# yjzxkxdn/HubertFA

Measured on NVIDIA B200. Metric: dp_cells_per_s, higher is better.
Workload: dtype f32

## Files before the change

hubertfa_b200/csrc/hfa_api.cu:

```cuda
#include <algorithm>
#include <atomic>
#include <climits>
#include <cstdarg>
#include <cstdio>
#include <cstdlib>
#include <cstring>
#include <mutex>
#include <new>
#include <numeric>
#include <unordered_map>
#include <vector>

#include <cuda.h>

#include "../../include/hfa_align.h"
#include "hfa_common.cuh"

#define HFA_EMIS_ROWS 64

cudaError_t hfa_launch_unpack_emissions(const HfaLaunchCtx &c, int total_row_blocks, float *out);
cudaError_t hfa_launch_dp_warp_any(const HfaLaunchCtx &c, int max_k, int max_pair_k, const int32_t *order, int n,
                                   float *dp_dump);
cudaError_t hfa_launch_dp_cta(const HfaLaunchCtx &c, const int32_t *order, int n, int max_sp, float *dp_dump);
cudaError_t hfa_launch_dp_band(const HfaLaunchCtx &c, int k, int item_begin, int n_items, int32_t *ticket,
                               bool keep_dp, int64_t fused_row_stride, float *dp_dump);
cudaError_t hfa_launch_dp_skew(const HfaLaunchCtx &c, int d, int item_begin, int n_items, int32_t *ticket,
                               bool keep_dp, float *dp_dump);
cudaError_t hfa_launch_emission(const HfaLaunchCtx &c, int total_row_blocks, int max_sp, int dtype,
                                int64_t max_row_stride, int *n_launched);
cudaError_t hfa_launch_edge(const HfaLaunchCtx &c, int total_row_blocks, int dtype);
cudaError_t hfa_launch_pack(const HfaLaunchCtx &c, int total_row_blocks, const float *prob_log,
                            const float *edge_log, const float *not_edge_log,
                            const float *edge_pred);
cudaError_t hfa_launch_backtrace(const HfaLaunchCtx &c, const int32_t *order, int n,
                                 const HfaResultPtrs &res, float *frame_conf, float *dp_path);
cudaError_t hfa_launch_unpack_bp(const HfaLaunchCtx &c, int utt, int8_t *out);
cudaError_t hfa_launch_unpack_dp(const HfaLaunchCtx &c, int utt, float *out);
cudaError_t hfa_launch_ctc_greedy(const void *logits, int dtype, int T, int V, int64_t st_t, int64_t st_v,
                                  int32_t *arg, int32_t *out_ids, int32_t *out_len, cudaStream_t stream);
cudaError_t hfa_launch_jump_tables(const HfaLaunchCtx &c, int n_blocks);
cudaError_t hfa_launch_backtrace_tables(const HfaLaunchCtx &c, const int32_t *order, int n,
                                        const HfaResultPtrs &res, float *frame_conf, float *dp_path);

namespace {

thread_local char g_err[512] = "";
std::atomic<int64_t> g_launches{0};

int fail(int code, const char *fmt, ...)
{
    va_list ap;
    va_start(ap, fmt);
    vsnprintf(g_err, sizeof(g_err), fmt, ap);
    va_end(ap);
    return code;
}
int cuda_fail(cudaError_t e, const char *what)
{
    return fail(HFA_ERR_CUDA, "%s: %s", what, cudaGetErrorString(e));
}

inline int64_t align_up(int64_t v, int64_t a) { return (v + a - 1) / a * a; }

typedef CUresult (*HfaEncodeTiled)(CUtensorMap *, CUtensorMapDataType, cuuint32_t, void *, const cuuint64_t *,
                                   const cuuint64_t *, const cuuint32_t *, const cuuint32_t *, CUtensorMapInterleave,
                                   CUtensorMapSwizzle, CUtensorMapL2promotion, CUtensorMapFloatOOBfill);
HfaEncodeTiled tensor_map_encoder()
{
    if (const char *e = std::getenv("HFA_NO_TENSORMAP"))
        if (e[0] == '1') return nullptr;
    static const HfaEncodeTiled fn = [] {
        void *f = nullptr;
        cudaDriverEntryPointQueryResult q;
        if (cudaGetDriverEntryPoint("cuTensorMapEncodeTiled", &f, cudaEnableDefault, &q) != cudaSuccess ||
            q != cudaDriverEntryPointSuccess)
            return (HfaEncodeTiled) nullptr;
        return reinterpret_cast<HfaEncodeTiled>(f);
    }();
    return fn;
}

struct HfaSideStreams {
    int device = -1;
    cudaStream_t stream[HFA_NUM_CLASSES] = {};
    cudaEvent_t fork = nullptr, join[HFA_NUM_CLASSES] = {};
};
std::vector<HfaSideStreams *> &side_pool()
{
    thread_local std::vector<HfaSideStreams *> pool;
    return pool;
}
HfaSideStreams *side_streams()
{
    std::vector<HfaSideStreams *> &pool = side_pool();
    int dev = 0;
    if (cudaGetDevice(&dev) != cudaSuccess) return nullptr;
    for (HfaSideStreams *s : pool)
        if (s->device == dev) return s;
    HfaSideStreams *s = new (std::nothrow) HfaSideStreams();
    if (!s) return nullptr;
    s->device = dev;
    bool ok = cudaEventCreateWithFlags(&s->fork, cudaEventDisableTiming) == cudaSuccess;
    for (int i = 0; ok && i < HFA_NUM_CLASSES; ++i) {
        ok = cudaStreamCreateWithFlags(&s->stream[i], cudaStreamNonBlocking) == cudaSuccess &&
             cudaEventCreateWithFlags(&s->join[i], cudaEventDisableTiming) == cudaSuccess;
    }
    if (!ok) { delete s; return nullptr; }
    try {
        pool.push_back(s);
    } catch (const std::bad_alloc &) {
        delete s;
        return nullptr;
    }
    return s;
}

int sm_count()
{
    int dev = 0, n = 0;
    if (cudaGetDevice(&dev) != cudaSuccess ||
        cudaDeviceGetAttribute(&n, cudaDevAttrMultiProcessorCount, dev) != cudaSuccess || n < 1)
        return 148;
    return n;
}

}

struct hfa_plan {
    int32_t n_utt = 0, vocab = 0;
    double frame_length = 0.0;
    std::vector<HfaUtt> utt;
    std::vector<int32_t> ids;
    std::vector<int32_t> col_ids;
    std::vector<uint8_t> colmap;
    int32_t n_compact = 0;
    int64_t stored_emis = 0;
    std::vector<int64_t> frame_off, seg_off;
    std::vector<int32_t> order;
    int32_t class_begin[HFA_NUM_CLASSES + 2] = {0};
    int32_t class_count[HFA_NUM_CLASSES + 1] = {0};
    int32_t cta_max_sp = 0, max_sp = 4;
    int32_t warp_all_begin = 0, warp_all_count = 0, warp_max_k = 0;
    int32_t warp_max_pair_k = 0, pair_count = 0;
    std::vector<HfaBandItem> band_items;
    int32_t band_begin[2] = {0, 0}, band_count[2] = {0, 0}, band_k[2] = {2, 4};
    int32_t band_skew[2] = {0, 0};
    int64_t band_xchg_elems = 0, dp_store_elems = 0;
    std::vector<int32_t> jblk_utt, jblk_first;
    int32_t n_valid = 0, n_kept = 0;
    int32_t bt_begin = 0;
    std::vector<int32_t> row_blocks;
    std::vector<int32_t> block_utt;
    int64_t total_frames = 0, total_states = 0, total_cells = 0, padded_cells = 0;
    int64_t total_words = 0, total_edge = 0;
    int64_t o_colids = 0, o_colmap = 0, o_emode = 0;
    int64_t o_utt = 0, o_ids = 0, o_order = 0, o_rowblk = 0, o_blkutt = 0, o_inputs = 0, head_bytes = 0;
    int64_t o_emis = 0, o_edge2 = 0, o_edgep = 0, o_bp = 0, o_path = 0, o_revi = 0, o_revt = 0,
            o_last = 0, o_dpst = 0, o_jump = 0, o_moves = 0, o_rowent = 0, o_band_items = 0, o_jblk_utt = 0, o_jblk_first = 0, o_band_ticket = 0, o_band_xchg = 0, band_bytes = 0, o_tmaps = 0, ws_bytes = 0;
    int32_t n_tmaps = 0;
    std::vector<unsigned char> head;
    HfaResultLayout res{};
    mutable std::mutex layout_mu;
    mutable std::unordered_map<const void *, int64_t> layout_of;
    int64_t row_stride_of(const void *workspace) const
    {
        std::lock_guard<std::mutex> g(layout_mu);
        auto it = layout_of.find(workspace);
        return it == layout_of.end() ? 0 : it->second;
    }
    void set_row_stride(const void *workspace, int64_t v) const
    {
        std::lock_guard<std::mutex> g(layout_mu);
        layout_of[workspace] = v;
    }
};

namespace {

HfaWs make_ws(const hfa_plan *p, void *workspace)
{
    unsigned char *b = static_cast<unsigned char *>(workspace);
    HfaWs w;
    w.utt = reinterpret_cast<const HfaUtt *>(b + p->o_utt);
    w.ids = reinterpret_cast<const int32_t *>(b + p->o_ids);
    w.order = reinterpret_cast<const int32_t *>(b + p->o_order);
    w.row_blocks = reinterpret_cast<const int32_t *>(b + p->o_rowblk);
    w.block_utt = reinterpret_cast<const int32_t *>(b + p->o_blkutt);
    w.inputs = reinterpret_cast<HfaInput *>(b + p->o_inputs);
    w.emis = reinterpret_cast<float *>(b + p->o_emis);
    w.edge2 = reinterpret_cast<float2 *>(b + p->o_edge2);
    w.edge_p = reinterpret_cast<float *>(b + p->o_edgep);
    w.bp = reinterpret_cast<uint32_t *>(b + p->o_bp);
    w.path_state = reinterpret_cast<int32_t *>(b + p->o_path);
    w.rev_idx = reinterpret_cast<int32_t *>(b + p->o_revi);
    w.rev_t = reinterpret_cast<int32_t *>(b + p->o_revt);
    w.dp_last = reinterpret_cast<float *>(b + p->o_last);
    w.dp_store = reinterpret_cast<float *>(b + p->o_dpst);
    w.jump = reinterpret_cast<uint8_t *>(b + p->o_jump);
    w.moves = reinterpret_cast<uint8_t *>(b + p->o_moves);
    w.row_entry = reinterpret_cast<int32_t *>(b + p->o_rowent);
    w.jblk_utt = reinterpret_cast<const int32_t *>(b + p->o_jblk_utt);
    w.jblk_first = reinterpret_cast<const int32_t *>(b + p->o_jblk_first);
    w.tmaps = (p->n_tmaps > 0 && tensor_map_encoder() != nullptr) ? b + p->o_tmaps : nullptr;
    w.col_ids = reinterpret_cast<const int32_t *>(b + p->o_colids);
    w.colmap = reinterpret_cast<const uint8_t *>(b + p->o_colmap);
    w.emis_mode = reinterpret_cast<int32_t *>(b + p->o_emode);
    w.band_items = reinterpret_cast<const HfaBandItem *>(b + p->o_band_items);
    w.band_ticket = reinterpret_cast<int32_t *>(b + p->o_band_ticket);
    w.band_xchg = reinterpret_cast<uint4 *>(b + p->o_band_xchg);
    return w;
}

HfaLaunchCtx make_ctx(const hfa_plan *p, void *workspace, void *stream)
{
    HfaLaunchCtx c;
    c.ws = make_ws(p, workspace);
    c.n_utt = p->n_utt;
    c.vocab = p->vocab;
    c.frame_length = p->frame_length;
    c.stream = static_cast<cudaStream_t>(stream);
    return c;
}

HfaResultPtrs make_res(const hfa_plan *p, void *result)
{
    unsigned char *b = static_cast<unsigned char *>(result);
    HfaResultPtrs r;
    r.status = reinterpret_cast<int32_t *>(b + p->res.status);
    r.n_seg = reinterpret_cast<int32_t *>(b + p->res.n_seg);
    r.end_state = reinterpret_cast<int32_t *>(b + p->res.end_state);
    r.final_score = reinterpret_cast<float *>(b + p->res.final_score);
    r.total_conf = reinterpret_cast<float *>(b + p->res.total_conf);
    r.ph_idx_seq = reinterpret_cast<int32_t *>(b + p->res.ph_idx_seq);
    r.ph_time_int = reinterpret_cast<int32_t *>(b + p->res.ph_time_int);
    r.intervals = reinterpret_cast<double *>(b + p->res.intervals);
    return r;
}

}

extern "C" {

int hfa_abi_version(void) { return HFA_ABI_VERSION; }
const char *hfa_last_error(void) { return g_err; }
int64_t hfa_launch_count(void) { return g_launches.load(); }

int hfa_plan_create(int32_t n_utt, int32_t vocab_size, const int32_t *T, const int32_t *S,
                    const int32_t *ph_ids, double frame_length, hfa_plan **out)
{
    if (out == nullptr) return fail(HFA_ERR_ARG, "hfa_plan_create: out is NULL");
    *out = nullptr;
    if (n_utt < 0 || vocab_size < 1 || (n_utt > 0 && (!T || !S || !ph_ids)))
        return fail(HFA_ERR_ARG, "hfa_plan_create: bad arguments (n_utt=%d, V=%d)", n_utt,
                    vocab_size);
    hfa_plan *p = new (std::nothrow) hfa_plan();
    if (!p) return fail(HFA_ERR_NOMEM, "hfa_plan_create: out of host memory");
    try {
        p->n_utt = n_utt;
        p->vocab = vocab_size;
        p->frame_length = frame_length;
        p->utt.resize((size_t)n_utt);
        p->frame_off.assign((size_t)n_utt + 1, 0);
        p->seg_off.assign((size_t)n_utt + 1, 0);
        p->row_blocks.assign((size_t)n_utt + 1, 0);
        for (int32_t b = 0; b < n_utt; ++b)
            p->seg_off[b + 1] = p->seg_off[b] + std::max<int32_t>(S[b], 0);
        p->total_states = p->seg_off[n_utt];
        p->ids.assign(ph_ids, ph_ids + p->total_states);

        std::vector<int32_t> lists[HFA_NUM_CLASSES + 1], invalid, giant;
        int64_t emis = 0, edge = 0, words = 0, cells = 0, frames = 0;
        for (int32_t b = 0; b < n_utt; ++b) {
            HfaUtt &m = p->utt[b];
            std::memset(&m, 0, sizeof(m));
            const int32_t t = T[b], s = S[b];
            int32_t st = HFA_UTT_OK;
            if (s < 1) st = HFA_UTT_NO_STATES;
            else if (t < 1) st = HFA_UTT_EMPTY;
            else if (s > HFA_MAX_STATES) st = HFA_UTT_TOO_MANY_STATES;
            else {
                const int32_t *id = ph_ids + p->seg_off[b];
                for (int32_t i = 0; i < s; ++i)
                    if (id[i] < 0 || id[i] >= vocab_size) { st = HFA_UTT_BAD_ID; break; }
            }
            m.status = st;
            m.seg_off = p->seg_off[b];
            m.frame_off = frames;
            m.cell_off = cells;
            m.emis_off = emis;
            m.edge_off = edge;
            m.bp_off = words;
            m.dp_off = -1;
            m.tmap = -1;
            p->frame_off[b] = frames;
            if (st == HFA_UTT_OK) {
                m.T = t;
                m.S = s;
                m.Sp = (s + 3) & ~3;
                frames += t;
                cells += (int64_t)t * s;
                emis += (int64_t)t * m.Sp;
                edge += align_up(t, HFA_TILE_T);
                words += (int64_t)((t + 15) / 16) * m.Sp;
                p->row_blocks[b + 1] = p->row_blocks[b] + (t + HFA_EMIS_ROWS - 1) / HFA_EMIS_ROWS;
                p->max_sp = std::max(p->max_sp, m.Sp);
                if (m.Sp <= HFA_WARP_MAX_S) lists[(m.Sp + 31) / 32 - 1].push_back(b);
                else if (s > HFA_CTA_MAX_S) giant.push_back(b);
                else {
                    lists[HFA_NUM_CLASSES].push_back(b);
                    p->cta_max_sp = std::max(p->cta_max_sp, m.Sp);
                }
            } else {
                p->row_blocks[b + 1] = p->row_blocks[b];
                invalid.push_back(b);
            }
        }
        p->frame_off[n_utt] = frames;
        p->total_frames = frames;
        p->total_cells = cells;
        p->padded_cells = emis;
        p->total_words = words;
        p->total_edge = edge;

        auto by_len = [&](int32_t a, int32_t b) {
            return p->utt[a].T != p->utt[b].T ? p->utt[a].T > p->utt[b].T : a < b;
        };
        std::vector<int32_t> all;
        for (int c = 0; c <= HFA_NUM_CLASSES; ++c) {
            std::sort(lists[c].begin(), lists[c].end(), by_len);
            p->class_begin[c] = (int32_t)p->order.size();
            p->class_count[c] = (int32_t)lists[c].size();
            p->order.insert(p->order.end(), lists[c].begin(), lists[c].end());
            all.insert(all.end(), lists[c].begin(), lists[c].end());
        }
        all.insert(all.end(), giant.begin(), giant.end());
        int skew_d = 2;
        if (const char *e = std::getenv("HFA_SKEW_D")) skew_d = (std::atoi(e) == 3) ? 3 : 2;
        if (const char *e = std::getenv("HFA_LAT_KERNEL")) { if (e[0] == 'b') skew_d = 0; }
        if (tensor_map_encoder() == nullptr) skew_d = 0;
        auto n_bands = [&](int32_t b, int k) {
            if (k == 1) return hfa_skew_strips(p->utt[b].Sp);
            const int w = 32 * k, own = w - 32, sp = p->utt[b].Sp;
            return sp <= w ? 1 : (sp - 32 + own - 1) / own;
        };
        int64_t band_max = 3072;
        if (const char *e = std::getenv("HFA_BAND_MAX")) band_max = std::atoll(e);
        int lat_mode = -1;
        if (const char *e = std::getenv("HFA_LATENCY_MODE")) lat_mode = e[0] - '0';
        std::vector<int32_t> lat_band;
        bool hybrid = false;
        if (lat_mode != 0) {
            int64_t nb = 0;
            for (int c = 0; c < HFA_NUM_CLASSES; ++c)
                for (int32_t b : lists[c]) nb += n_bands(b, skew_d > 0 ? 1 : 2);
            if (skew_d > 0) {
                p->band_k[0] = 1;
                p->band_skew[0] = skew_d;
            }
            if (lat_mode == 2 || (nb > 0 && nb <= band_max)) {
                for (int c = 0; c < HFA_NUM_CLASSES; ++c) {
                    lat_band.insert(lat_band.end(), lists[c].begin(), lists[c].end());
                    lists[c].clear();
                    p->class_count[c] = 0;
                }
                std::sort(lat_band.begin(), lat_band.end(), by_len);
            } else if (skew_d > 0 && nb > 0) {
                double alpha = 0.0;
                if (const char *e = std::getenv("HFA_HYBRID")) alpha = std::atof(e);
                auto ucost = [&](int32_t b) { return (int64_t)p->utt[b].T * ((p->utt[b].Sp + 31) / 32); };
                int64_t sum_cost = 0;
                for (int c = 0; c < HFA_NUM_CLASSES; ++c)
                    for (int32_t b : lists[c]) sum_cost += ucost(b);
                const double thresh = alpha * (double)sum_cost / (4.0 * sm_count());
                if (alpha > 0.0) {
                    int64_t strips = 0;
                    for (int c = 1; c < HFA_NUM_CLASSES; ++c) {
                        std::vector<int32_t> keep;
                        for (int32_t b : lists[c]) {
                            if ((double)ucost(b) >= thresh && strips + n_bands(b, 1) <= 8 * band_max) {
                                lat_band.push_back(b);
                                strips += n_bands(b, 1);
                            } else {
                                keep.push_back(b);
                            }
                        }
                        lists[c].swap(keep);
                        p->class_count[c] = (int32_t)lists[c].size();
                    }
                    std::sort(lat_band.begin(), lat_band.end(), by_len);
                    hybrid = !lat_band.empty();
                }
            }
        }
        std::vector<int32_t> big_band;
        {
            int big_mode = -1;
            if (const char *e = std::getenv("HFA_BIG_KERNEL")) big_mode = (e[0] == 'b');
            auto count = [&](int k) {
                int64_t nb = 0;
                for (int32_t b : lists[HFA_NUM_CLASSES]) nb += n_bands(b, k);
                return nb;
            };
            int big_k = 0;
            if (const char *e = std::getenv("HFA_BIG_K")) big_k = std::atoi(e);
            if (big_k != 2 && big_k != 4 && big_k != 8) {
                big_k = 8;
                for (int k : {2, 4, 8})
                    if (count(k) <= band_max) { big_k = k; break; }
                if (skew_d > 0 && count(1) <= band_max) big_k = 1;
            }
            p->band_k[1] = big_k;
            if (big_k == 1) p->band_skew[1] = skew_d;
            if (big_mode == 1 || (big_mode == -1 && count(big_k) <= band_max)) {
                big_band = lists[HFA_NUM_CLASSES];
                lists[HFA_NUM_CLASSES].clear();
                p->class_count[HFA_NUM_CLASSES] = 0;
            }
            if (!giant.empty()) {
                if (big_band.empty()) {
                    p->band_k[1] = skew_d > 0 ? 1 : 2;
                    p->band_skew[1] = skew_d;
                }
                big_band.insert(big_band.end(), giant.begin(), giant.end());
                std::sort(big_band.begin(), big_band.end(), by_len);
            }
        }
        bool keep_dp = true;
        if (const char *e = std::getenv("HFA_KEEP_DP")) keep_dp = (e[0] != '0');
        auto add_bands = [&](const std::vector<int32_t> &utts, int which) {
            const int k = p->band_k[which];
            const int sd = p->band_skew[which];
            p->band_begin[which] = (int32_t)p->band_items.size();
            for (int32_t b : utts) {
                const int nb = n_bands(b, k);
                const int64_t tiles = (p->utt[b].T + 15) / 16;
                p->utt[b].skew_d = sd;
                p->utt[b].band_k = k;
                p->utt[b].tmap = p->n_tmaps++;
                if (keep_dp && !(hybrid && which == 0)) {
                    p->utt[b].dp_off = p->dp_store_elems;
                    p->dp_store_elems += sd > 0 ? (int64_t)nb * hfa_skew_blocks(sd, p->utt[b].T) * HFA_SKEW_BLK * 32
                                                : (int64_t)nb * p->utt[b].T * 32 * k;
                }
                for (int j = 0; j < nb; ++j) {
                    const bool has_right = j + 1 < nb;
                    p->band_items.push_back(HfaBandItem{b, j, has_right ? p->band_xchg_elems : 0});
                    if (has_right) p->band_xchg_elems += sd > 0 ? (tiles + 1) / 2 * 32 : tiles * 64;
                }
            }
            p->band_count[which] = (int32_t)p->band_items.size() - p->band_begin[which];
        };
        add_bands(lat_band, 0);
        add_bands(big_band, 1);
        p->n_valid = (int32_t)all.size();
        for (const HfaUtt &m : p->utt) p->n_kept += (m.status == 0 && m.dp_off >= 0);
        p->jblk_first.assign((size_t)n_utt + 1, 0);
        for (int32_t b = 0; b < n_utt; ++b) {
            const HfaUtt &m = p->utt[b];
            const int64_t w = (m.status == 0 && m.dp_off >= 0) ? (int64_t)((m.T + 15) / 16) * m.Sp : 0;
            const int32_t nblk = (int32_t)((w + 255) / 256);
            p->jblk_first[b + 1] = p->jblk_first[b] + nblk;
            p->jblk_utt.insert(p->jblk_utt.end(), (size_t)nblk, b);
        }
        int pair_mode = 1;
        if (const char *e = std::getenv("HFA_PAIR")) pair_mode = std::atoi(e);
        std::vector<int32_t> warp_all;
        std::vector<std::pair<int32_t, int>> pairable;
        int64_t sum_pair = 0, sum_plain = 0;
        for (int c = 0; c < HFA_NUM_CLASSES; ++c) {
            warp_all.insert(warp_all.end(), lists[c].begin(), lists[c].end());
            for (int32_t b : lists[c]) {
                const HfaUtt &m = p->utt[b];
                const int32_t *id = ph_ids + m.seg_off;
                int phon = 0;
                bool ok = pair_mode > 0;
                for (int32_t i = 0; i < m.S && ok; ++i) {
                    phon += id[i] != 0;
                    if (i > 0 && id[i] == 0 && id[i - 1] == 0) ok = false;
                }
                const int kp = (phon + (id[m.S - 1] == 0) + 31) / 32;
                if (ok && kp <= HFA_PAIR_MAX_K) {
                    pairable.push_back({b, kp});
                    sum_pair += (int64_t)m.T * (17 + 25 * kp);
                    sum_plain += (int64_t)m.T * (16 + 21 * (c + 1));
                }
                p->warp_max_k = std::max(p->warp_max_k, c + 1);
            }
        }
        bool compact = vocab_size <= 255;
        if (const char *e = std::getenv("HFA_COMPACT")) compact = compact && e[0] != '0';
        p->col_ids.assign((size_t)(p->total_states + 4 * (int64_t)n_utt), vocab_size);
        p->colmap.assign((size_t)p->total_states, 0);
        if (pair_mode >= 2 || sum_pair < sum_plain)
            for (const auto &bk : pairable) {
                HfaUtt &m = p->utt[bk.first];
                m.pair_k = bk.second;
                p->warp_max_pair_k = std::max(p->warp_max_pair_k, bk.second);
                p->pair_count += 1;
                if (!compact) continue;
                const int32_t *id = ph_ids + m.seg_off;
                int col_of[256];
                std::fill(col_of, col_of + 256, -1);
                for (int32_t i = 0; i < m.S; ++i) col_of[id[i]] = 0;
                int d = 0;
                for (int v = 0; v < vocab_size; ++v)
                    if (col_of[v] == 0) col_of[v] = d++;
                const int dp = (d + 3) & ~3;
                if (dp >= m.Sp) continue;
                m.Dp = dp;
                p->n_compact += 1;
                int32_t *ci = p->col_ids.data() + m.seg_off + 4 * (int64_t)bk.first;
                for (int v = 0; v < vocab_size; ++v)
                    if (col_of[v] >= 0) ci[col_of[v]] = v;
                for (int32_t i = 0; i < m.S; ++i) p->colmap[(size_t)(m.seg_off + i)] = (uint8_t)col_of[id[i]];
            }
        for (const HfaUtt &m : p->utt)
            if (m.status == 0) p->stored_emis += (int64_t)m.T * (m.Dp > 0 ? m.Dp : m.Sp);
        const bool old_order = p->pair_count == 0;
        auto cost = [&](int32_t b) {
            const HfaUtt &m = p->utt[b];
            if (old_order) return (int64_t)m.T * (2 + (m.Sp + 31) / 32);
            return (int64_t)m.T * (m.pair_k > 0 ? 17 + 25 * m.pair_k : 16 + 21 * ((m.Sp + 31) / 32));
        };
        std::sort(warp_all.begin(), warp_all.end(),
                  [&](int32_t a, int32_t b) { return cost(a) != cost(b) ? cost(a) > cost(b) : a < b; });
        p->warp_all_begin = (int32_t)p->order.size();
        p->warp_all_count = (int32_t)warp_all.size();
        p->order.insert(p->order.end(), warp_all.begin(), warp_all.end());
        std::sort(all.begin(), all.end(), by_len);
        p->bt_begin = (int32_t)p->order.size();
        p->order.insert(p->order.end(), all.begin(), all.end());
        p->order.insert(p->order.end(), invalid.begin(), invalid.end());

        int64_t o = 0;
        auto region = [&](int64_t bytes) { const int64_t at = o; o = align_up(o + bytes, 256); return at; };
        p->o_utt = region((int64_t)n_utt * sizeof(HfaUtt));
        p->o_ids = region(p->total_states * 4);
        p->o_order = region((int64_t)p->order.size() * 4);
        p->o_rowblk = region((int64_t)(n_utt + 1) * 4);
        p->block_utt.reserve((size_t)p->row_blocks[n_utt]);
        for (int32_t b = 0; b < n_utt; ++b)
            p->block_utt.insert(p->block_utt.end(), (size_t)(p->row_blocks[b + 1] - p->row_blocks[b]), b);
        p->o_blkutt = region((int64_t)p->block_utt.size() * 4);
        p->o_band_items = region((int64_t)p->band_items.size() * sizeof(HfaBandItem));
        p->o_jblk_utt = region((int64_t)p->jblk_utt.size() * 4);
        p->o_jblk_first = region((int64_t)p->jblk_first.size() * 4);
        p->o_colids = region(p->n_compact > 0 ? (int64_t)p->col_ids.size() * 4 : 0);
        p->o_colmap = region(p->n_compact > 0 ? (int64_t)p->colmap.size() : 0);
        p->head_bytes = o;
        p->o_inputs = region((int64_t)n_utt * sizeof(HfaInput));
        p->o_emis = region(emis * 4);
        p->o_edge2 = region(edge * 8);
        p->o_edgep = region(edge * 4 + 4);
        p->o_bp = region(words * 4);
        p->o_path = region(frames * 4);
        p->o_revi = region(p->total_states * 4);
        p->o_revt = region(p->total_states * 4);
        p->o_last = region((int64_t)n_utt * 8);
        p->o_emode = region(p->n_compact > 0 ? (int64_t)n_utt * 4 : 0);
        p->o_dpst = region(p->dp_store_elems * 4);
        const bool jump_tables = p->dp_store_elems > 0;
        p->o_jump = region(jump_tables ? words : 0);
        p->o_moves = region(jump_tables ? words : 0);
        p->o_rowent = region(jump_tables ? edge / 16 * 4 : 0);

        p->o_tmaps = region((int64_t)p->n_tmaps * 128);
        p->o_band_ticket = region(p->band_items.empty() ? 0 : 8);
        p->o_band_xchg = region(p->band_xchg_elems * 16);
        p->band_bytes = o - p->o_band_ticket;
        p->ws_bytes = std::max<int64_t>(o, 256);

        p->head.assign((size_t)p->head_bytes, 0);
        if (n_utt > 0) {
            std::memcpy(p->head.data() + p->o_utt, p->utt.data(), (size_t)n_utt * sizeof(HfaUtt));
            if (p->total_states)
                std::memcpy(p->head.data() + p->o_ids, p->ids.data(), (size_t)p->total_states * 4);
            std::memcpy(p->head.data() + p->o_order, p->order.data(), p->order.size() * 4);
        }
        if (!p->band_items.empty())
            std::memcpy(p->head.data() + p->o_band_items, p->band_items.data(),
                        p->band_items.size() * sizeof(HfaBandItem));
        if (!p->jblk_utt.empty())
            std::memcpy(p->head.data() + p->o_jblk_utt, p->jblk_utt.data(), p->jblk_utt.size() * 4);
        std::memcpy(p->head.data() + p->o_jblk_first, p->jblk_first.data(), p->jblk_first.size() * 4);
        if (p->n_compact > 0) {
            std::memcpy(p->head.data() + p->o_colids, p->col_ids.data(), p->col_ids.size() * 4);
            if (!p->colmap.empty()) std::memcpy(p->head.data() + p->o_colmap, p->colmap.data(), p->colmap.size());
        }
        std::memcpy(p->head.data() + p->o_rowblk, p->row_blocks.data(), (size_t)(n_utt + 1) * 4);
        if (!p->block_utt.empty())
            std::memcpy(p->head.data() + p->o_blkutt, p->block_utt.data(), p->block_utt.size() * 4);

        int64_t r = 0;
        auto rreg = [&](int64_t bytes) { const int64_t at = r; r = align_up(r + bytes, 16); return at; };
        p->res.status = rreg((int64_t)n_utt * 4);
        p->res.n_seg = rreg((int64_t)n_utt * 4);
        p->res.end_state = rreg((int64_t)n_utt * 4);
        p->res.final_score = rreg((int64_t)n_utt * 4);
        p->res.total_conf = rreg((int64_t)n_utt * 4);
        p->res.ph_idx_seq = rreg(p->total_states * 4);
        p->res.ph_time_int = rreg(p->total_states * 4);
        p->res.intervals = rreg(p->total_states * 16);
        p->res.total_bytes = std::max<int64_t>(r, 16);
    } catch (const std::bad_alloc &) {
        delete p;
        return fail(HFA_ERR_NOMEM, "hfa_plan_create: out of host memory");
    }
    *out = p;
    return HFA_OK;
}

void hfa_plan_destroy(hfa_plan *plan) { delete plan; }

int64_t hfa_plan_workspace_bytes(const hfa_plan *p) { return p ? p->ws_bytes : 0; }
int64_t hfa_plan_total_frames(const hfa_plan *p) { return p ? p->total_frames : 0; }
int64_t hfa_plan_total_states(const hfa_plan *p) { return p ? p->total_states : 0; }
int64_t hfa_plan_total_cells(const hfa_plan *p) { return p ? p->total_cells : 0; }
const int64_t *hfa_plan_frame_offsets(const hfa_plan *p) { return p ? p->frame_off.data() : nullptr; }
const int64_t *hfa_plan_seg_offsets(const hfa_plan *p) { return p ? p->seg_off.data() : nullptr; }

int hfa_plan_result_layout(const hfa_plan *p, HfaResultLayout *out)
{
    if (!p || !out) return fail(HFA_ERR_ARG, "hfa_plan_result_layout: NULL argument");
    *out = p->res;
    return HFA_OK;
}

int hfa_plan_algorithmic_bytes(const hfa_plan *p, int32_t dtype, int64_t out[3])
{
    if (!p || !out) return fail(HFA_ERR_ARG, "hfa_plan_algorithmic_bytes: NULL argument");
    const int64_t in_b = (dtype == HFA_DTYPE_F32) ? 4 : 2;
    int64_t words = 0, kept_cells = 0, kept_frames = 0;
    for (const HfaUtt &m : p->utt)
        if (m.status == 0) {
            words += (int64_t)((m.T + 15) / 16) * m.S;
            if (m.dp_off >= 0) {
                kept_cells += (int64_t)m.T * m.S;
                kept_frames += m.T;
            }
        }
    out[0] = p->total_frames * ((int64_t)p->vocab * in_b + in_b) + p->total_cells * 4 +
             p->total_frames * 12;
    out[1] = p->total_cells * 4 + p->total_frames * 8 + words * 4 + kept_cells * 4;
    out[2] = (p->total_frames - kept_frames) * (8 + 8) + kept_frames * (8 + 4) + p->total_states * 24;
    return HFA_OK;
}

int hfa_plan_routing(const hfa_plan *p, int32_t out[8])
{
    if (!p || !out) return fail(HFA_ERR_ARG, "hfa_plan_routing: NULL argument");
    out[0] = p->warp_all_count;
    out[1] = p->band_count[0];
    out[2] = p->band_k[0];
    out[3] = p->band_count[1];
    out[4] = p->band_k[1];
    out[5] = p->class_count[HFA_NUM_CLASSES];
    out[6] = p->dp_store_elems > 0;
    out[7] = std::max(p->band_skew[0], p->band_skew[1]);
    return HFA_OK;
}

int32_t hfa_plan_pair_utterances(const hfa_plan *p) { return p ? p->pair_count : 0; }
int64_t hfa_plan_stored_emission_bytes(const hfa_plan *p) { return p ? p->stored_emis * 4 : 0; }

int64_t hfa_plan_debug_region(const hfa_plan *p, int32_t which, int64_t *n_bytes)
{
    if (!p) return -1;
    int64_t off = -1, n = 0;
    switch (which) {
        case 0: off = p->o_emis; n = p->padded_cells * 4; break;
        case 1: off = p->o_edge2; n = p->total_edge * 8; break;
        case 2: off = p->o_edgep; n = p->total_edge * 4; break;
        case 3: off = p->o_bp; n = p->total_words * 4; break;
        default: break;
    }
    if (n_bytes) *n_bytes = n;
    return off;
}

int hfa_plan_upload(const hfa_plan *p, void *workspace, void *stream)
{
    if (!p || !workspace) return fail(HFA_ERR_ARG, "hfa_plan_upload: NULL argument");
    if (p->head_bytes == 0) return HFA_OK;
    cudaError_t e = cudaMemcpyAsync(workspace, p->head.data(), (size_t)p->head_bytes,
                                    cudaMemcpyHostToDevice, static_cast<cudaStream_t>(stream));
    if (e != cudaSuccess) return cuda_fail(e, "hfa_plan_upload");
    if (p->n_tmaps > 0 && tensor_map_encoder() != nullptr) try {
        std::vector<CUtensorMap> maps((size_t)p->n_tmaps);
        for (const HfaUtt &m : p->utt) {
            if (m.status != 0 || m.tmap < 0) continue;
            const cuuint64_t dims[2] = {(cuuint64_t)m.Sp, (cuuint64_t)m.T};
            const cuuint64_t pitch[1] = {(cuuint64_t)m.Sp * 4};
            const cuuint32_t box[2] = {(cuuint32_t)(m.skew_d > 0 ? HFA_SKEW_BOX : 32 * m.band_k),
                                       (cuuint32_t)(m.skew_d > 0 ? HFA_SKEW_BLK : HFA_TILE_T)};
            const cuuint32_t estr[2] = {1, 1};
            void *base = static_cast<unsigned char *>(workspace) + p->o_emis + m.emis_off * 4;
            const CUresult r = tensor_map_encoder()(&maps[(size_t)m.tmap], CU_TENSOR_MAP_DATA_TYPE_FLOAT32, 2, base,
                                                    dims, pitch, box, estr, CU_TENSOR_MAP_INTERLEAVE_NONE,
                                                    CU_TENSOR_MAP_SWIZZLE_NONE, CU_TENSOR_MAP_L2_PROMOTION_NONE,
                                                    CU_TENSOR_MAP_FLOAT_OOB_FILL_NONE);
            if (r != CUDA_SUCCESS) return fail(HFA_ERR_CUDA, "hfa_plan_upload: cuTensorMapEncodeTiled failed (%d)", (int)r);
        }
        e = cudaMemcpyAsync(static_cast<unsigned char *>(workspace) + p->o_tmaps, maps.data(), maps.size() * 128,
                            cudaMemcpyHostToDevice, static_cast<cudaStream_t>(stream));
        if (e != cudaSuccess) return cuda_fail(e, "hfa_plan_upload: tensor maps");
    } catch (const std::bad_alloc &) {
        return fail(HFA_ERR_NOMEM, "hfa_plan_upload: out of host memory");
    }
    if (p->n_compact > 0) {
        e = cudaMemsetAsync(static_cast<unsigned char *>(workspace) + p->o_emode, 0, (size_t)p->n_utt * 4,
                            static_cast<cudaStream_t>(stream));
        if (e != cudaSuccess) return cuda_fail(e, "hfa_plan_upload: emission mode reset");
    }
    if (p->band_bytes > 0) {
        e = cudaMemsetAsync(static_cast<unsigned char *>(workspace) + p->o_band_ticket, 0,
                            (size_t)p->band_bytes, static_cast<cudaStream_t>(stream));
        if (e != cudaSuccess) return cuda_fail(e, "hfa_plan_upload: band table reset");
    }
    return HFA_OK;
}

int hfa_set_inputs(const hfa_plan *p, void *workspace, const void *const *frame_ptrs,
                   const int64_t *frame_stride_t, const int64_t *frame_stride_v,
                   const void *const *edge_ptrs, const int64_t *edge_stride, void *stream)
{
    if (!p || !workspace) return fail(HFA_ERR_ARG, "hfa_set_inputs: NULL plan/workspace");
    if (p->n_utt == 0) return HFA_OK;
    if (!frame_ptrs || !frame_stride_t || !frame_stride_v || !edge_ptrs || !edge_stride)
        return fail(HFA_ERR_ARG, "hfa_set_inputs: NULL input table");
    try {
        std::vector<HfaInput> in((size_t)p->n_utt);
        int64_t row_stride = 0;
        bool contiguous = true;
        for (int32_t b = 0; b < p->n_utt; ++b) {
            if (p->utt[b].status == 0 && (!frame_ptrs[b] || !edge_ptrs[b]))
                return fail(HFA_ERR_ARG, "hfa_set_inputs: NULL logits pointer for utterance %d", b);
            if (p->utt[b].status == 0) {
                if (frame_stride_v[b] != 1 || frame_stride_t[b] < p->vocab ||
                    (reinterpret_cast<uintptr_t>(frame_ptrs[b]) & 3u))
                    contiguous = false;
                row_stride = std::max(row_stride, frame_stride_t[b]);
            }
            in[b].frame = frame_ptrs[b];
            in[b].edge = edge_ptrs[b];
            in[b].frame_st = frame_stride_t[b];
            in[b].frame_sv = frame_stride_v[b];
            in[b].edge_st = edge_stride[b];
        }
        HfaLaunchCtx c = make_ctx(p, workspace, stream);
        cudaError_t e = cudaMemcpyAsync(c.ws.inputs, in.data(), in.size() * sizeof(HfaInput),
                                        cudaMemcpyHostToDevice, c.stream);
        if (e != cudaSuccess) return cuda_fail(e, "hfa_set_inputs: input table upload");
        p->set_row_stride(workspace, contiguous ? row_stride : 0);
    } catch (const std::bad_alloc &) {
        return fail(HFA_ERR_NOMEM, "hfa_set_inputs: out of host memory");
    }
    return HFA_OK;
}

static_assert(sizeof(HfaInputDesc) == sizeof(HfaInput), "the public descriptor is the kernels' own");

int hfa_set_inputs_device(const hfa_plan *p, void *workspace, const HfaInputDesc *table, int64_t max_row_stride,
                          void *stream)
{
    if (!p || !workspace) return fail(HFA_ERR_ARG, "hfa_set_inputs_device: NULL plan/workspace");
    if (p->n_utt == 0) return HFA_OK;
    if (!table) return fail(HFA_ERR_ARG, "hfa_set_inputs_device: NULL table");
    if (max_row_stride < 0) return fail(HFA_ERR_ARG, "hfa_set_inputs_device: negative row stride");
    HfaLaunchCtx c = make_ctx(p, workspace, stream);
    cudaError_t e = cudaMemcpyAsync(c.ws.inputs, table, (size_t)p->n_utt * sizeof(HfaInput),
                                    cudaMemcpyDeviceToDevice, c.stream);
    if (e != cudaSuccess) return cuda_fail(e, "hfa_set_inputs_device: table copy");
    try {
        p->set_row_stride(workspace, max_row_stride);
    } catch (const std::bad_alloc &) {
        return fail(HFA_ERR_NOMEM, "hfa_set_inputs_device: out of host memory");
    }
    return HFA_OK;
}

void hfa_release_thread_resources(void)
{
    for (HfaSideStreams *s : side_pool()) {
        for (int i = 0; i < HFA_NUM_CLASSES; ++i) {
            if (s->stream[i]) cudaStreamDestroy(s->stream[i]);
            if (s->join[i]) cudaEventDestroy(s->join[i]);
        }
        if (s->fork) cudaEventDestroy(s->fork);
        delete s;
    }
    side_pool().clear();
}

int hfa_emission(const hfa_plan *p, void *workspace, int32_t dtype, void *stream)
{
    if (!p || !workspace) return fail(HFA_ERR_ARG, "hfa_emission: NULL plan/workspace");
    if (p->n_utt == 0 || p->total_frames == 0) return HFA_OK;
    if (dtype < 0 || dtype > 2) return fail(HFA_ERR_ARG, "hfa_emission: bad dtype %d", dtype);
    HfaLaunchCtx c = make_ctx(p, workspace, stream);
    static const bool no_tma = [] { const char *v = std::getenv("HFA_EMISSION_NO_TMA"); return v && v[0] == '1'; }();
    const int64_t row_stride = no_tma ? 0 : p->row_stride_of(workspace);
    HfaSideStreams *ss = nullptr;
    cudaError_t e = cudaSuccess;
    if (row_stride > 0) {
        ss = side_streams();
        if (!ss) return fail(HFA_ERR_CUDA, "hfa_emission: cannot create side streams");
        e = cudaEventRecord(ss->fork, c.stream);
        if (e != cudaSuccess) return cuda_fail(e, "hfa_emission: fork");
    }
    int n_launched = 0;
    e = hfa_launch_emission(c, p->row_blocks[p->n_utt], p->max_sp, dtype, row_stride, &n_launched);
    if (e != cudaSuccess) return cuda_fail(e, "hfa_emission: launch");
    if (n_launched == 2) {
        HfaLaunchCtx cs = c;
        cs.stream = ss->stream[HFA_NUM_CLASSES - 1];
        e = cudaStreamWaitEvent(cs.stream, ss->fork, 0);
        if (e == cudaSuccess) e = hfa_launch_edge(cs, p->row_blocks[p->n_utt], dtype);
        if (e == cudaSuccess) e = cudaEventRecord(ss->join[HFA_NUM_CLASSES - 1], cs.stream);
        if (e == cudaSuccess) e = cudaStreamWaitEvent(c.stream, ss->join[HFA_NUM_CLASSES - 1], 0);
        if (e != cudaSuccess) return cuda_fail(e, "hfa_emission: edge kernel");
    }
    g_launches += n_launched;
    return HFA_OK;
}

int hfa_pack_emissions(const hfa_plan *p, void *workspace, const float *prob_log,
                       const float *edge_log, const float *not_edge_log, const float *edge_pred,
                       void *stream)
{
    if (!p || !workspace) return fail(HFA_ERR_ARG, "hfa_pack_emissions: NULL plan/workspace");
    if (p->n_utt == 0 || p->total_frames == 0) return HFA_OK;
    if (!prob_log || !edge_log || !not_edge_log)
        return fail(HFA_ERR_ARG, "hfa_pack_emissions: NULL input");
    HfaLaunchCtx c = make_ctx(p, workspace, stream);
    cudaError_t e = hfa_launch_pack(c, p->row_blocks[p->n_utt], prob_log, edge_log, not_edge_log,
                                    edge_pred);
    if (e != cudaSuccess) return cuda_fail(e, "hfa_pack_emissions: launch");
    g_launches += 1;
    return HFA_OK;
}

static int viterbi_forward_impl(const hfa_plan *p, void *workspace, float *dp_dump, void *stream,
                                int64_t fused_row_stride)
{
    if (!p || !workspace) return fail(HFA_ERR_ARG, "hfa_viterbi_forward: NULL plan/workspace");
    HfaLaunchCtx c = make_ctx(p, workspace, stream);
    const int n_cta = p->class_count[HFA_NUM_CLASSES];
    struct Item { int k; const int32_t *order; int n; };
    Item items[4];
    int n_items = 0;
    if (p->warp_all_count > 0) items[n_items++] = {0, c.ws.order + p->warp_all_begin, p->warp_all_count};
    if (p->band_count[0] > 0) items[n_items++] = {-3, nullptr, 0};
    if (p->band_count[1] > 0) items[n_items++] = {-4, nullptr, 1};
    if (n_cta > 0) items[n_items++] = {-1, c.ws.order + p->class_begin[HFA_NUM_CLASSES], n_cta};
    if (n_items == 0) return HFA_OK;

    const bool fork = n_items > 1;
    HfaSideStreams *ss = nullptr;
    if (fork) {
        ss = side_streams();
        if (!ss) return fail(HFA_ERR_CUDA, "hfa_viterbi_forward: cannot create side streams");
        cudaError_t e = cudaEventRecord(ss->fork, c.stream);
        if (e != cudaSuccess) return cuda_fail(e, "hfa_viterbi_forward: fork record");
    }
    const cudaStream_t user = c.stream;
    for (int it = 0; it < n_items; ++it) {
        cudaError_t e;
        const bool side = fork && it > 0;
        c.stream = side ? ss->stream[it - 1] : user;
        if (side) {
            e = cudaStreamWaitEvent(c.stream, ss->fork, 0);
            if (e != cudaSuccess) return cuda_fail(e, "hfa_viterbi_forward: fork wait");
        }
        if (items[it].k == 0)
            e = hfa_launch_dp_warp_any(c, p->warp_max_k, p->warp_max_pair_k, items[it].order, items[it].n, dp_dump);
        else if (items[it].k == -3 || items[it].k == -4) {
            const int wh = items[it].k == -3 ? 0 : 1;
            if (p->band_skew[wh] > 0)
                e = hfa_launch_dp_skew(c, p->band_skew[wh], p->band_begin[wh], p->band_count[wh],
                                       c.ws.band_ticket + wh, p->dp_store_elems > 0, dp_dump);
            else
                e = hfa_launch_dp_band(c, p->band_k[wh], p->band_begin[wh], p->band_count[wh],
                                       c.ws.band_ticket + wh, p->dp_store_elems > 0, fused_row_stride, dp_dump);
        }
        else
            e = hfa_launch_dp_cta(c, items[it].order, items[it].n, p->cta_max_sp, dp_dump);
        if (e != cudaSuccess) return cuda_fail(e, "hfa_viterbi_forward: kernel launch");
        g_launches += 1;
        if (side) {
            e = cudaEventRecord(ss->join[it - 1], c.stream);
            if (e == cudaSuccess) e = cudaStreamWaitEvent(user, ss->join[it - 1], 0);
            if (e != cudaSuccess) return cuda_fail(e, "hfa_viterbi_forward: join");
        }
    }
    return HFA_OK;
}

int hfa_viterbi_forward(const hfa_plan *p, void *workspace, float *dp_dump, void *stream)
{
    return viterbi_forward_impl(p, workspace, dp_dump, stream, 0);
}

int hfa_backtrace(const hfa_plan *p, void *workspace, void *result, float *frame_conf,
                  float *dp_path, void *stream)
{
    if (!p || !workspace || !result) return fail(HFA_ERR_ARG, "hfa_backtrace: NULL argument");
    if (p->n_utt == 0) return HFA_OK;
    HfaLaunchCtx c = make_ctx(p, workspace, stream);
    const HfaResultPtrs r = make_res(p, result);
    if (!p->jblk_utt.empty()) {
        cudaError_t ej = hfa_launch_jump_tables(c, (int)p->jblk_utt.size());
        if (ej == cudaSuccess)
            ej = hfa_launch_backtrace_tables(c, c.ws.order + p->bt_begin, p->n_valid, r, frame_conf, dp_path);
        if (ej != cudaSuccess) return cuda_fail(ej, "hfa_backtrace: table kernels");
        g_launches += 2;
        if (p->n_kept == p->n_utt) return HFA_OK;
    }
    cudaError_t e = hfa_launch_backtrace(c, c.ws.order + p->bt_begin, p->n_utt, r, frame_conf,
                                         dp_path);
    if (e != cudaSuccess) return cuda_fail(e, "hfa_backtrace: launch");
    g_launches += 1;
    return HFA_OK;
}

static bool fused_ok(const hfa_plan *p, const void *workspace, int32_t dtype)
{
    const int64_t max_row_stride = p->row_stride_of(workspace);
    const bool all_banded = p->warp_all_count == 0 &&
                            p->class_count[HFA_NUM_CLASSES] == 0 && !p->band_items.empty();
    const bool skewed = p->band_skew[0] > 0 || p->band_skew[1] > 0;
    return all_banded && !skewed && p->max_sp <= HFA_CTA_MAX_S && p->dp_store_elems > 0 && dtype == HFA_DTYPE_F32 &&
           max_row_stride > 0 &&
           p->vocab <= 256 && max_row_stride * 4 * HFA_TILE_T <= 48 * 1024;
}

int hfa_forward_fused(const hfa_plan *p, void *workspace, int32_t dtype, void *stream)
{
    if (!p || !workspace) return fail(HFA_ERR_ARG, "hfa_forward_fused: NULL plan/workspace");
    if (!fused_ok(p, workspace, dtype))
        return fail(HFA_ERR_UNSUPPORTED, "hfa_forward_fused: needs an all-banded plan that keeps dp, f32 logits "
                                         "with contiguous rows (set by hfa_set_inputs) and V <= 256");
    HfaLaunchCtx c = make_ctx(p, workspace, stream);
    cudaError_t e = hfa_launch_edge(c, p->row_blocks[p->n_utt], dtype);
    if (e != cudaSuccess) return cuda_fail(e, "hfa_forward_fused: edge kernel");
    g_launches += 1;
    return viterbi_forward_impl(p, workspace, nullptr, stream, p->row_stride_of(workspace));
}

int64_t hfa_plan_algorithmic_bytes_fused(const hfa_plan *p, int32_t dtype)
{
    if (!p) return 0;
    const int64_t in_b = (dtype == HFA_DTYPE_F32) ? 4 : 2;
    int64_t words = 0;
    for (const HfaUtt &m : p->utt)
        if (m.status == 0) words += (int64_t)((m.T + 15) / 16) * m.S;
    return p->total_frames * ((int64_t)p->vocab * in_b + in_b) + p->total_frames * 12 + words * 4 +
           p->total_cells * 4;
}

int hfa_align_batch(const hfa_plan *p, void *workspace, int32_t dtype, void *result,
                    float *frame_conf, void *stream)
{
    if (!p || !workspace) return fail(HFA_ERR_ARG, "hfa_align_batch: NULL plan/workspace");
    static const int fused_mode = [] { const char *v = std::getenv("HFA_FUSED"); return v ? (v[0] == '1' ? 1 : 0) : -1; }();
    int64_t n_valid = 0;
    for (const HfaUtt &m : p->utt) n_valid += (m.status == 0);
    const bool unsplit = (int64_t)p->band_items.size() == n_valid;
    int rc;
    if ((fused_mode == 1 || (fused_mode == -1 && unsplit)) && fused_ok(p, workspace, dtype)) {
        rc = hfa_forward_fused(p, workspace, dtype, stream);
    } else {
        rc = hfa_emission(p, workspace, dtype, stream);
        if (rc != HFA_OK) return rc;
        rc = viterbi_forward_impl(p, workspace, nullptr, stream, 0);
    }
    if (rc != HFA_OK) return rc;
    return hfa_backtrace(p, workspace, result, frame_conf, nullptr, stream);
}

int hfa_ctc_greedy(const void *logits, int32_t dtype, int64_t T, int64_t V, int64_t stride_t,
                   int64_t stride_v, int32_t *scratch, int32_t *out_ids, int32_t *out_len, void *stream)
{
    if (!logits || !scratch || !out_ids || !out_len) return fail(HFA_ERR_ARG, "hfa_ctc_greedy: NULL argument");
    if (T < 0 || V < 1 || T > INT32_MAX || V > INT32_MAX || dtype < 0 || dtype > 2)
        return fail(HFA_ERR_ARG, "hfa_ctc_greedy: bad shape / dtype (T=%lld, V=%lld)", (long long)T, (long long)V);
    cudaError_t e = hfa_launch_ctc_greedy(logits, dtype, (int)T, (int)V, stride_t, stride_v, scratch, out_ids,
                                          out_len, static_cast<cudaStream_t>(stream));
    if (e != cudaSuccess) return cuda_fail(e, "hfa_ctc_greedy: launch");
    g_launches += 1;
    return HFA_OK;
}

int hfa_debug_unpack_backptr(const hfa_plan *p, const void *workspace, int32_t utt, int8_t *out,
                             void *stream)
{
    if (!p || !workspace || !out) return fail(HFA_ERR_ARG, "hfa_debug_unpack_backptr: NULL argument");
    if (utt < 0 || utt >= p->n_utt || p->utt[utt].status != 0)
        return fail(HFA_ERR_ARG, "hfa_debug_unpack_backptr: bad utterance %d", utt);
    HfaLaunchCtx c = make_ctx(p, const_cast<void *>(workspace), stream);
    cudaError_t e = hfa_launch_unpack_bp(c, utt, out);
    if (e != cudaSuccess) return cuda_fail(e, "hfa_debug_unpack_backptr: launch");
    g_launches += 1;
    return HFA_OK;
}

int hfa_debug_unpack_dp(const hfa_plan *p, const void *workspace, int32_t utt, float *out, void *stream)
{
    if (!p || !workspace || !out) return fail(HFA_ERR_ARG, "hfa_debug_unpack_dp: NULL argument");
    if (utt < 0 || utt >= p->n_utt || p->utt[utt].status != 0)
        return fail(HFA_ERR_ARG, "hfa_debug_unpack_dp: bad utterance %d", utt);
    if (p->utt[utt].dp_off < 0)
        return fail(HFA_ERR_UNSUPPORTED, "hfa_debug_unpack_dp: the forward pass keeps no dp for utterance %d", utt);
    HfaLaunchCtx c = make_ctx(p, const_cast<void *>(workspace), stream);
    cudaError_t e = hfa_launch_unpack_dp(c, utt, out);
    if (e != cudaSuccess) return cuda_fail(e, "hfa_debug_unpack_dp: launch");
    g_launches += 1;
    return HFA_OK;
}

int hfa_debug_unpack_emissions(const hfa_plan *p, const void *workspace, float *out, void *stream)
{
    if (!p || !workspace || !out) return fail(HFA_ERR_ARG, "hfa_debug_unpack_emissions: NULL argument");
    HfaLaunchCtx c = make_ctx(p, const_cast<void *>(workspace), stream);
    cudaError_t e = hfa_launch_unpack_emissions(c, p->n_utt > 0 ? p->row_blocks[p->n_utt] : 0, out);
    if (e != cudaSuccess) return cuda_fail(e, "hfa_debug_unpack_emissions: launch");
    g_launches += 1;
    return HFA_OK;
}

}
```

hubertfa_b200/csrc/hfa_backtrace.cu:

```cuda
#include "hfa_common.cuh"

#define HFA_BT_WARPS 4

namespace {

__device__ __forceinline__ double seg_time(const float *p, int t, int T, double frame_length)
{
    double d = (t + 1 < T) ? (double)__fsub_rn(p[t + 1], p[t]) : 0.0;
    d = fmin(fmax(__dmul_rn(d, 0.5), -0.5), 0.5);
    return __dmul_rn(frame_length, __dadd_rn((double)(float)t, d));
}

template <typename FMove, typename FSpan>
__device__ __forceinline__ int hfa_walk_row(const uint32_t *__restrict__ row_words, int cur, int tt, bool row0,
                                            FMove on_move, FSpan on_span)
{
    while (tt >= 0) {
        const uint32_t wc = row_words[cur];
        uint32_t nz = (wc | (wc >> 16)) & 0xffffu & ((2u << tt) - 1u);
        if (row0) nz |= 1u;
        if (nz == 0u) {
            on_span(cur, 0, tt);
            break;
        }
        const int tp = 31 - __clz(nz);
        on_span(cur, tp, tt);
        on_move(cur, tp);
        if (row0 && tp == 0) break;
        cur -= ((wc >> (16 + tp)) & 1u) ? 2 : 1;
        tt = tp - 1;
    }
    return cur;
}

__global__ void __launch_bounds__(256)
hfa_jump_table_kernel(HfaWs ws)
{
    const int u = ws.jblk_utt[blockIdx.x];
    const HfaUtt m = ws.utt[u];
    const int n_rows = (m.T + 15) >> 4;
    const int64_t idx = (int64_t)(blockIdx.x - ws.jblk_first[u]) * blockDim.x + threadIdx.x;
    if (idx >= (int64_t)n_rows * m.Sp) return;
    const int w = (int)(idx / m.Sp), s = (int)(idx - (int64_t)w * m.Sp);
    const int tt = (w == n_rows - 1) ? ((m.T - 1) & 15) : 15;
    int n_moves = 0;
    const int from = hfa_walk_row(ws.bp + m.bp_off + (int64_t)w * m.Sp, s, tt, false,
                                  [&](int, int) { ++n_moves; }, [](int, int, int) {});
    ws.jump[m.bp_off + idx] = (uint8_t)(s - from);
    ws.moves[m.bp_off + idx] = (uint8_t)n_moves;
}

__global__ void __launch_bounds__(HFA_BT_WARPS * 32)
hfa_backtrace_kernel(HfaWs ws, const int32_t *__restrict__ order, int n, HfaResultPtrs res,
                     float *__restrict__ frame_conf, float *__restrict__ dp_path,
                     double frame_length)
{
    __shared__ float4 stage_sm[HFA_BT_WARPS][32];
    __shared__ float dpath_sm[HFA_BT_WARPS][32];
    const int lane = threadIdx.x & 31, warp = threadIdx.x >> 5;
    const int item = blockIdx.x * HFA_BT_WARPS + warp;
    if (item >= n) return;
    const int u = order[item];
    const HfaUtt m = ws.utt[u];
    if (m.status != 0) {
        if (lane == 0) {
            res.status[u] = m.status;
            res.n_seg[u] = 0;
            res.end_state[u] = -1;
            res.final_score[u] = HFA_NEG_INF;
            res.total_conf[u] = __uint_as_float(0x7fc00000u);
        }
        return;
    }
    if (m.dp_off >= 0) return;
    const int T = m.T, S = m.S, Sp = m.Sp;
    const int32_t *ids = ws.ids + m.seg_off;
    const uint32_t *bp = ws.bp + m.bp_off;
    int32_t *rev_idx = ws.rev_idx + m.seg_off;
    int32_t *rev_t = ws.rev_t + m.seg_off;
    int32_t *path_state = ws.path_state + m.frame_off;

    const float last1 = ws.dp_last[2 * u];
    const float last2 = (S >= 2) ? ws.dp_last[2 * u + 1] : HFA_NEG_INF;
    int s = S - 1;
    float final_score = last1;
    if (S >= 2 && last2 > last1 && ids[S - 1] == 0) {
        s = S - 2;
        final_score = last2;
    }
    const int s_end = s;

    constexpr int LEAD = 4;
    const int n_rows = (T + 15) >> 4;
    int n_seg = 0;
    int s_hi = s;
    uint32_t q[LEAD][2];
    int qref[LEAD];
    auto fetch = [&](int row, int ref, uint32_t (&w2)[2]) {
        w2[0] = w2[1] = 0u;
        if (row >= 0) {
            const uint32_t *r = bp + (int64_t)row * Sp;
            if (ref - lane >= 0) w2[0] = r[ref - lane];
            if (ref - lane - 32 >= 0) w2[1] = r[ref - lane - 32];
        }
    };
    uint32_t W = (s_hi - lane >= 0) ? bp[(int64_t)(n_rows - 1) * Sp + (s_hi - lane)] : 0u;
#pragma unroll
    for (int dd = 0; dd < LEAD; ++dd) {
        fetch(n_rows - 2 - dd, s_hi, q[dd]);
        qref[dd] = s_hi;
    }
    for (int w = n_rows - 1; w >= 0; --w) {
        uint32_t f[2];
        fetch(w - 1 - LEAD, s_hi, f);
        const int fref = s_hi;
        int tt = (w == n_rows - 1) ? ((T - 1) & 15) : 15;
        int my_state = 0;
        while (tt >= 0) {
            const uint32_t wc = __shfl_sync(0xffffffffu, W, (s_hi - s) & 31);
            uint32_t nz = (wc | (wc >> 16)) & 0xffffu & ((2u << tt) - 1u);
            if (w == 0) nz |= 1u;
            if (nz == 0u) {
                if (lane <= tt) my_state = s;
                break;
            }
            const int tp = 31 - __clz(nz);
            if (lane <= tt && lane >= tp) my_state = s;
            if (lane == 0 && n_seg < S) {
                rev_idx[n_seg] = s;
                rev_t[n_seg] = 16 * w + tp;
            }
            ++n_seg;
            if (w == 0 && tp == 0) break;
            s -= ((wc >> (16 + tp)) & 1u) ? 2 : 1;
            tt = tp - 1;
        }
        if (lane < 16 && 16 * w + lane < T) path_state[16 * w + lane] = my_state;
        if (w > 0) {
            const int o = (qref[0] - s) + lane;
            if (qref[0] - s + 31 < 64) {
                const uint32_t x0 = __shfl_sync(0xffffffffu, q[0][0], o & 31);
                const uint32_t x1 = __shfl_sync(0xffffffffu, q[0][1], o & 31);
                W = (o < 32) ? x0 : x1;
            } else {
                W = (s - lane >= 0) ? bp[(int64_t)(w - 1) * Sp + (s - lane)] : 0u;
            }
            s_hi = s;
#pragma unroll
            for (int dd = 0; dd + 1 < LEAD; ++dd) {
                q[dd][0] = q[dd + 1][0];
                q[dd][1] = q[dd + 1][1];
                qref[dd] = qref[dd + 1];
            }
            q[LEAD - 1][0] = f[0];
            q[LEAD - 1][1] = f[1];
            qref[LEAD - 1] = fref;
        }
    }
    if (n_seg > S) n_seg = S;
    __syncwarp();

    double log_sum = 0.0;
    {
    const float *emis = ws.emis + m.emis_off;
    const float2 *edge2 = ws.edge2 + m.edge_off;
    const double ratio = __ddiv_rn((double)T, (double)S);
    const bool lead_sp = (ids[0] == 0) && (S > 1);
    const bool compact = m.Dp > 0 && ws.emis_mode[u] != 0;
    const int Ep = compact ? m.Dp : Sp;
    const uint8_t *cmap = ws.colmap + m.seg_off;
    float4 *stage = stage_sm[warp];
    float *dpath = dpath_sm[warp];
    float d = 0.0f, cu = 0.0f, carry_d = 0.0f;
    const int n_rounds = (T + 31) >> 5;
    auto load_state = [&](int round) {
        const int t = round * 32 + lane;
        return (round < n_rounds && t < T) ? path_state[t] : 0;
    };
    struct Raw { float x, y; float2 ed; int id, st, sprev; };
    auto gather = [&](int round, int st, int sprev) {
        const int t = min(round * 32 + lane, T - 1);
        const float *row = emis + (int64_t)t * Ep;
        Raw g;
        g.x = hfa_ldg_f32_64B(row + (compact ? (int)cmap[st] : st));
        g.y = hfa_ldg_f32_64B(row + (compact ? (int)cmap[sprev] : sprev));
        g.ed = edge2[t];
        g.id = ids[st];
        g.st = st;
        g.sprev = sprev;
        return g;
    };
    auto finish = [&](int round, const Raw &g) {
        const int t = round * 32 + lane;
        float4 v = make_float4(0.f, 0.f, 0.f, __int_as_float(4));
        if (t < T) {
            const bool moved = (t > 0) && (g.sprev != g.st);
            v.x = g.x;
            v.y = g.y;
            v.z = moved ? g.ed.x : g.ed.y;
            int fl = (moved ? 1 : 0) | ((g.id == 0) ? 2 : 0);
            if (t == 0) {
                const bool seeded = (g.st == 0) || (g.st == 1 && lead_sp);
                v.x = seeded ? v.x : HFA_NEG_INF;
                fl = 8;
            }
            v.w = __int_as_float(fl);
        }
        return v;
    };
    int st_a = load_state(0), st_b = load_state(1), st_c = load_state(2);
    Raw g_cur = gather(0, st_a, __shfl_up_sync(0xffffffffu, st_a, 1));
    Raw g_nxt;
    {
        int sp1 = __shfl_up_sync(0xffffffffu, st_b, 1);
        const int last0 = __shfl_sync(0xffffffffu, st_a, 31);
        if (lane == 0) sp1 = last0;
        g_nxt = gather(1, st_b, sp1);
    }
    for (int r = 0; r < n_rounds; ++r) {
        const int st_d = load_state(r + 3);
        int sp2 = __shfl_up_sync(0xffffffffu, st_c, 1);
        const int last1 = __shfl_sync(0xffffffffu, st_b, 31);
        if (lane == 0) sp2 = last1;
        const Raw g_nn = gather(r + 2, st_c, sp2);
        const float4 v_cur = finish(r, g_cur);

        stage[lane] = v_cur;
        const uint32_t special = __ballot_sync(0xffffffffu, (__float_as_int(v_cur.w) & 13) != 0);
        __syncwarp();
        int j = 0;
        while (j < 32) {
            if ((special >> j) & 1u) {
                const float4 q = stage[j];
                const int fl = __float_as_int(q.w);
                if (fl & 1) {
                    d = hfa_advance(__fadd_rn(__fadd_rn(d, q.y), q.z), cu, ratio);
                    cu = (fl & 2) ? 0.0f : q.x;
                } else if (fl & 8) {
                    d = q.x;
                    cu = d;
                }
                if (lane == 0) dpath[j] = d;
                ++j;
                continue;
            }
            const uint32_t rest = special >> j;
            const int run = rest ? (__ffs(rest) - 1) : (32 - j);
            const bool sp_state = (__float_as_int(stage[j].w) & 2) != 0;
            int k = 0;
            for (; k + 4 <= run; k += 4) {
                const float4 q0 = stage[j + k], q1 = stage[j + k + 1], q2 = stage[j + k + 2],
                             q3 = stage[j + k + 3];
                const float d0 = __fadd_rn(__fadd_rn(d, q0.x), q0.z);
                const float d1 = __fadd_rn(__fadd_rn(d0, q1.x), q1.z);
                const float d2 = __fadd_rn(__fadd_rn(d1, q2.x), q2.z);
                d = __fadd_rn(__fadd_rn(d2, q3.x), q3.z);
                cu = fmaxf(fmaxf(cu, q0.x), fmaxf(fmaxf(q1.x, q2.x), q3.x));
                if (lane == 0) {
                    dpath[j + k] = d0; dpath[j + k + 1] = d1; dpath[j + k + 2] = d2; dpath[j + k + 3] = d;
                }
            }
            for (; k < run; ++k) {
                const float4 q = stage[j + k];
                d = __fadd_rn(__fadd_rn(d, q.x), q.z);
                cu = fmaxf(cu, q.x);
                if (lane == 0) dpath[j + k] = d;
            }
            if (sp_state) cu = 0.0f;
            j += run;
        }
        __syncwarp();
        const int t = r * 32 + lane;
        if (t < T) {
            const float cur = dpath[lane];
            const float prev = (lane == 0) ? carry_d : dpath[lane - 1];
            const float fc = expf(__fsub_rn(cur, prev));
            if (frame_conf != nullptr) frame_conf[m.frame_off + t] = fc;
            if (dp_path != nullptr) dp_path[m.frame_off + t] = cur;
            log_sum += (double)logf(__fadd_rn(fc, 1e-6f));
        }
        carry_d = d;
        __syncwarp();
        st_b = st_c;
        st_c = st_d;
        g_cur = g_nxt;
        g_nxt = g_nn;
    }
    }
#pragma unroll
    for (int o = 16; o > 0; o >>= 1) log_sum += __shfl_xor_sync(0xffffffffu, log_sum, o);
    const float mean = (float)(log_sum / (double)T);
    const float total = expf(__fdiv_rn(mean, 3.0f));

    const float *p = ws.edge_p + m.edge_off;
    int32_t *out_idx = res.ph_idx_seq + m.seg_off;
    int32_t *out_t = res.ph_time_int + m.seg_off;
    double *out_iv = res.intervals + 2 * m.seg_off;
    for (int k = lane; k < n_seg; k += 32) {
        const int tk = rev_t[n_seg - 1 - k];
        out_idx[k] = rev_idx[n_seg - 1 - k];
        out_t[k] = tk;
        out_iv[2 * k] = seg_time(p, tk, T, frame_length);
        out_iv[2 * k + 1] = (k + 1 < n_seg) ? seg_time(p, rev_t[n_seg - 2 - k], T, frame_length)
                                            : __dmul_rn(frame_length, (double)T);
    }
    if (lane == 0) {
        res.status[u] = (final_score == HFA_NEG_INF) ? 4 : 0;
        res.n_seg[u] = n_seg;
        res.end_state[u] = s_end;
        res.final_score[u] = final_score;
        res.total_conf[u] = total;
    }
}

#define HFA_BTT_THREADS 256

__global__ void __launch_bounds__(HFA_BTT_THREADS)
hfa_backtrace_tables_kernel(HfaWs ws, const int32_t *__restrict__ order, int n, HfaResultPtrs res,
                            float *__restrict__ frame_conf, float *__restrict__ dp_path, double frame_length)
{
    constexpr int NW = HFA_BTT_THREADS / 32;
    __shared__ int warp_sum[NW];
    __shared__ double warp_log[NW];
    __shared__ int carry_sm;
    const int tid = threadIdx.x, lane = tid & 31, warp = tid >> 5;
    const int u = order[blockIdx.x];
    const HfaUtt m = ws.utt[u];
    if (m.status != 0 || m.dp_off < 0) return;
    const int T = m.T, S = m.S, Sp = m.Sp;
    const int32_t *ids = ws.ids + m.seg_off;
    const uint32_t *bp = ws.bp + m.bp_off;
    int32_t *path_state = ws.path_state + m.frame_off;
    int32_t *out_idx = res.ph_idx_seq + m.seg_off;
    int32_t *out_t = res.ph_time_int + m.seg_off;
    const int n_rows = (T + 15) >> 4;
    int32_t *entry = ws.row_entry + m.edge_off / HFA_TILE_T;

    const float last1 = ws.dp_last[2 * u];
    const float last2 = (S >= 2) ? ws.dp_last[2 * u + 1] : HFA_NEG_INF;
    int s_end = S - 1;
    float final_score = last1;
    if (S >= 2 && last2 > last1 && ids[S - 1] == 0) {
        s_end = S - 2;
        final_score = last2;
    }

    if (warp == 0) {
        const uint8_t *J = ws.jump + m.bp_off;
        int sr = s_end;
        int w = n_rows - 1;
        while (w >= 0) {
            uint32_t c0[16], c1[16];
#pragma unroll
            for (int r = 0; r < 16; ++r) {
                const bool row_ok = w - r >= 1;
                c0[r] = (row_ok && sr - lane >= 0) ? J[(int64_t)(w - r) * Sp + (sr - lane)] : 0u;
                c1[r] = (row_ok && sr - lane - 32 >= 0) ? J[(int64_t)(w - r) * Sp + (sr - lane - 32)] : 0u;
            }
            const int s_ref = sr;
            int done = 0;
#pragma unroll
            for (int r = 0; r < 16; ++r) {
                const int d = s_ref - sr;
                if (w - r < 0 || d >= 64) break;
                if (lane == 0) entry[w - r] = sr;
                const uint32_t x0 = __shfl_sync(0xffffffffu, c0[r], d & 31);
                const uint32_t x1 = __shfl_sync(0xffffffffu, c1[r], d & 31);
                sr -= (int)(d < 32 ? x0 : x1);
                ++done;
            }
            w -= done;
        }
    }
    if (tid == 0) carry_sm = 0;
    __syncthreads();

    const uint8_t *M = ws.moves + m.bp_off;
    const float *dps = ws.dp_store + m.dp_off;
    for (int base = 0; base < n_rows; base += HFA_BTT_THREADS) {
        const int wr = base + tid;
        int e = 0, c = 0;
        if (wr < n_rows) {
            e = entry[wr];
            c = (int)M[(int64_t)wr * Sp + e] + (wr == 0 ? 1 : 0);
        }
        int incl = c;
#pragma unroll
        for (int o = 1; o < 32; o <<= 1) {
            const int v = __shfl_up_sync(0xffffffffu, incl, o);
            if (lane >= o) incl += v;
        }
        if (lane == 31) warp_sum[warp] = incl;
        __syncthreads();
        int pos = carry_sm + incl;
        for (int q = 0; q < warp; ++q) pos += warp_sum[q];
        __syncthreads();
        if (tid == HFA_BTT_THREADS - 1) carry_sm = pos;
        if (wr < n_rows) {
            const int tt = (wr == n_rows - 1) ? ((T - 1) & 15) : 15;
            hfa_walk_row(bp + (int64_t)wr * Sp, e, tt, wr == 0,
                         [&](int st, int f) {
                             --pos;
                             if (pos < S) {
                                 out_idx[pos] = st;
                                 out_t[pos] = 16 * wr + f;
                             }
                         },
                         [&](int st, int f_lo, int f_hi) {
                             for (int f = f_lo; f <= f_hi; ++f) path_state[16 * wr + f] = st;
                         });
            float dv[16];
#pragma unroll
            for (int f = 0; f < 16; ++f) {
                const int t = min(16 * wr + f, T - 1);
                dv[f] = hfa_ldg_f32_64B(dps + (m.skew_d > 0 ? hfa_skew_dp_index(m.skew_d, T, t, path_state[t])
                                                            : hfa_dp_store_index(m.band_k, T, t, path_state[t])));
            }
#pragma unroll
            for (int f = 0; f < 16; ++f)
                if (16 * wr + f < T) path_state[16 * wr + f] = __float_as_int(dv[f]);
        }
        __syncthreads();
    }
    const int n_seg = min(carry_sm, S);

    double log_sum = 0.0;
    for (int t = tid; t < T; t += HFA_BTT_THREADS) {
        const float cur = __int_as_float(path_state[t]);
        const float prev = (t > 0) ? __int_as_float(path_state[t - 1]) : 0.0f;
        const float fc = expf(__fsub_rn(cur, prev));
        if (frame_conf != nullptr) frame_conf[m.frame_off + t] = fc;
        if (dp_path != nullptr) dp_path[m.frame_off + t] = cur;
        log_sum += (double)logf(__fadd_rn(fc, 1e-6f));
    }
#pragma unroll
    for (int o = 16; o > 0; o >>= 1) log_sum += __shfl_xor_sync(0xffffffffu, log_sum, o);
    if (lane == 0) warp_log[warp] = log_sum;

    const float *p = ws.edge_p + m.edge_off;
    double *out_iv = res.intervals + 2 * m.seg_off;
    for (int k = tid; k < n_seg; k += HFA_BTT_THREADS) {
        out_iv[2 * k] = seg_time(p, out_t[k], T, frame_length);
        out_iv[2 * k + 1] = (k + 1 < n_seg) ? seg_time(p, out_t[k + 1], T, frame_length)
                                            : __dmul_rn(frame_length, (double)T);
    }
    __syncthreads();
    if (tid == 0) {
        double tot = 0.0;
        for (int q = 0; q < NW; ++q) tot += warp_log[q];
        const float mean = (float)(tot / (double)T);
        res.status[u] = (final_score == HFA_NEG_INF) ? 4 : 0;
        res.n_seg[u] = n_seg;
        res.end_state[u] = s_end;
        res.final_score[u] = final_score;
        res.total_conf[u] = expf(__fdiv_rn(mean, 3.0f));
    }
}

__global__ void hfa_unpack_bp_kernel(HfaWs ws, int u, int8_t *__restrict__ out)
{
    const HfaUtt m = ws.utt[u];
    const int64_t n = (int64_t)m.T * m.S;
    for (int64_t i = blockIdx.x * (int64_t)blockDim.x + threadIdx.x; i < n;
         i += (int64_t)gridDim.x * blockDim.x) {
        const int t = (int)(i / m.S), s = (int)(i - (int64_t)t * m.S);
        const uint32_t w = ws.bp[m.bp_off + (int64_t)(t >> 4) * m.Sp + s];
        const int b = t & 15;
        const int code = ((w >> (16 + b)) & 1u) ? 2 : (int)((w >> b) & 1u);
        out[i] = (int8_t)((t == 0) ? -1 : code);
    }
}

__global__ void hfa_unpack_dp_kernel(HfaWs ws, int u, float *__restrict__ out)
{
    const HfaUtt m = ws.utt[u];
    const float *dps = ws.dp_store + m.dp_off;
    const int64_t n = (int64_t)m.T * m.S;
    for (int64_t i = blockIdx.x * (int64_t)blockDim.x + threadIdx.x; i < n;
         i += (int64_t)gridDim.x * blockDim.x) {
        const int t = (int)(i / m.S), s = (int)(i - (int64_t)t * m.S);
        out[i] = dps[m.skew_d > 0 ? hfa_skew_dp_index(m.skew_d, m.T, t, s) : hfa_dp_store_index(m.band_k, m.T, t, s)];
    }
}

}

cudaError_t hfa_launch_unpack_dp(const HfaLaunchCtx &c, int utt, float *out)
{
    hfa_unpack_dp_kernel<<<148, 256, 0, c.stream>>>(c.ws, utt, out);
    return cudaGetLastError();
}

cudaError_t hfa_launch_backtrace(const HfaLaunchCtx &c, const int32_t *order, int n,
                                 const HfaResultPtrs &res, float *frame_conf, float *dp_path)
{
    if (n <= 0) return cudaSuccess;
    const int blocks = (n + HFA_BT_WARPS - 1) / HFA_BT_WARPS;
    hfa_backtrace_kernel<<<blocks, HFA_BT_WARPS * 32, 0, c.stream>>>(c.ws, order, n, res, frame_conf,
                                                                    dp_path, c.frame_length);
    return cudaGetLastError();
}

cudaError_t hfa_launch_jump_tables(const HfaLaunchCtx &c, int n_blocks)
{
    if (n_blocks <= 0) return cudaSuccess;
    hfa_jump_table_kernel<<<n_blocks, 256, 0, c.stream>>>(c.ws);
    return cudaGetLastError();
}

cudaError_t hfa_launch_backtrace_tables(const HfaLaunchCtx &c, const int32_t *order, int n,
                                        const HfaResultPtrs &res, float *frame_conf, float *dp_path)
{
    if (n <= 0) return cudaSuccess;
    hfa_backtrace_tables_kernel<<<n, HFA_BTT_THREADS, 0, c.stream>>>(c.ws, order, n, res, frame_conf, dp_path,
                                                                    c.frame_length);
    return cudaGetLastError();
}

cudaError_t hfa_launch_unpack_bp(const HfaLaunchCtx &c, int utt, int8_t *out)
{
    hfa_unpack_bp_kernel<<<148, 256, 0, c.stream>>>(c.ws, utt, out);
    return cudaGetLastError();
}
```

hubertfa_b200/csrc/hfa_common.cuh:

```cuda
#pragma once
#include <cuda_runtime.h>
#include <cuda_fp16.h>
#include <cuda_bf16.h>
#include <stdint.h>

#define HFA_TILE_T 16
#define HFA_WARP_MAX_K 8
#define HFA_WARP_MAX_S (32 * HFA_WARP_MAX_K)
#define HFA_CTA_K 8
#define HFA_PAIR_MAX_K 4
#define HFA_NUM_CLASSES 8

struct HfaUtt {
    int32_t T, S, Sp, status;
    int64_t seg_off;
    int64_t emis_off;
    int64_t edge_off;
    int64_t bp_off;
    int64_t frame_off;
    int64_t cell_off;
    int64_t dp_off;
    int32_t band_k;
    int32_t tmap;
    int32_t skew_d;
    int32_t pair_k;
    int32_t Dp;
    int32_t pad_;
};
static_assert(sizeof(HfaUtt) == 96, "HfaUtt is 96 bytes (16-byte multiple)");

struct HfaInput {
    const void *frame;
    const void *edge;
    int64_t frame_st, frame_sv, edge_st;
};

struct HfaBandItem {
    int32_t utt, band;
    int64_t xoff;
};

struct HfaWs {
    const HfaUtt *utt;
    const int32_t *ids;
    const int32_t *order;
    const int32_t *row_blocks;
    const int32_t *block_utt;
    HfaInput *inputs;
    float *emis;
    float2 *edge2;
    float *edge_p;
    uint32_t *bp;
    int32_t *path_state;
    int32_t *rev_idx;
    int32_t *rev_t;
    float *dp_last;
    float *dp_store;
    uint8_t *jump;
    uint8_t *moves;
    int32_t *row_entry;
    const int32_t *jblk_utt;
    const int32_t *jblk_first;
    const void *tmaps;
    const int32_t *col_ids;
    const uint8_t *colmap;
    int32_t *emis_mode;
    const HfaBandItem *band_items;
    int32_t *band_ticket;
    uint4 *band_xchg;
};

#define HFA_NEG_INF __uint_as_float(0xff800000u)

__host__ __device__ __forceinline__ int64_t hfa_dp_store_index(int K, int T, int t, int s)
{
    const int W = 32 * K, OWN = W - 32;
    const int b = (s < W) ? 0 : 1 + (s - W) / OWN;
    return ((int64_t)b * T + t) * W + (s - b * OWN);
}

#define HFA_SKEW_OWN 30
#define HFA_SKEW_BOX 36
#define HFA_SKEW_BLK 32
__host__ __device__ __forceinline__ int hfa_skew_strips(int Sp)
{
    return Sp <= 32 ? 1 : 1 + (Sp - 32 + HFA_SKEW_OWN - 1) / HFA_SKEW_OWN;
}
__host__ __device__ __forceinline__ int hfa_skew_blocks(int D, int T)
{
    return (T + 31 * D + HFA_SKEW_BLK - 1) / HFA_SKEW_BLK;
}
__host__ __device__ __forceinline__ int64_t hfa_skew_dp_index(int D, int T, int t, int s)
{
    const int w = (s < 32) ? 0 : 1 + (s - 32) / HFA_SKEW_OWN;
    const int p = s - HFA_SKEW_OWN * w;
    return ((int64_t)w * hfa_skew_blocks(D, T) * HFA_SKEW_BLK + t + p * D) * 32 + p;
}

__device__ __forceinline__ uint32_t hfa_smem_u32(const void *p)
{
    return static_cast<uint32_t>(__cvta_generic_to_shared(p));
}
__device__ __forceinline__ void hfa_mbar_init(uint64_t *bar, uint32_t count)
{
    asm volatile("mbarrier.init.shared::cta.b64 [%0], %1;" ::"r"(hfa_smem_u32(bar)), "r"(count)
                 : "memory");
}
__device__ __forceinline__ void hfa_fence_mbar_init()
{
    asm volatile("fence.mbarrier_init.release.cluster;" ::: "memory");
    asm volatile("fence.proxy.async.shared::cta;" ::: "memory");
}
__device__ __forceinline__ void hfa_mbar_expect_tx(uint64_t *bar, uint32_t bytes)
{
    asm volatile("mbarrier.arrive.expect_tx.shared::cta.b64 _, [%0], %1;" ::"r"(hfa_smem_u32(bar)),
                 "r"(bytes)
                 : "memory");
}
__device__ __forceinline__ void hfa_bulk_load(void *dst_smem, const void *src_gmem, uint32_t bytes,
                                              uint64_t *bar)
{
    asm volatile(
        "cp.async.bulk.shared::cluster.global.mbarrier::complete_tx::bytes [%0], [%1], %2, [%3];" ::
            "r"(hfa_smem_u32(dst_smem)),
        "l"(src_gmem), "r"(bytes), "r"(hfa_smem_u32(bar))
        : "memory");
}
__device__ __forceinline__ void hfa_bulk_store(void *dst_gmem, const void *src_smem, uint32_t bytes)
{
    asm volatile("cp.async.bulk.global.shared::cta.bulk_group [%0], [%1], %2;" ::"l"(dst_gmem),
                 "r"(hfa_smem_u32(src_smem)), "r"(bytes)
                 : "memory");
}
__device__ __forceinline__ void hfa_bulk_commit() { asm volatile("cp.async.bulk.commit_group;" ::: "memory"); }
__device__ __forceinline__ void hfa_bulk_wait_read() { asm volatile("cp.async.bulk.wait_group.read 0;" ::: "memory"); }
__device__ __forceinline__ void hfa_bulk_wait_all() { asm volatile("cp.async.bulk.wait_group 0;" ::: "memory"); }
__device__ __forceinline__ void hfa_fence_async_smem() { asm volatile("fence.proxy.async.shared::cta;" ::: "memory"); }
__device__ __forceinline__ void hfa_tensor_load_2d(void *dst_smem, const void *tmap, int x, int y, uint64_t *bar)
{
    asm volatile(
        "cp.async.bulk.tensor.2d.shared::cluster.global.tile.mbarrier::complete_tx::bytes [%0], [%1, {%2, %3}], [%4];"
        ::"r"(hfa_smem_u32(dst_smem)), "l"(tmap), "r"(x), "r"(y), "r"(hfa_smem_u32(bar))
        : "memory");
}
__device__ __forceinline__ bool hfa_elect_one()
{
    uint32_t pred;
    asm volatile(
        "{\n"
        ".reg .pred p;\n"
        "elect.sync _|p, 0xffffffff;\n"
        "selp.u32 %0, 1, 0, p;\n"
        "}\n"
        : "=r"(pred));
    return pred != 0;
}
__device__ __forceinline__ bool hfa_mbar_try_wait(uint64_t *bar, uint32_t parity)
{
    uint32_t ok;
    asm volatile(
        "{\n"
        ".reg .pred p;\n"
        "mbarrier.try_wait.parity.shared::cta.b64 p, [%1], %2;\n"
        "selp.u32 %0, 1, 0, p;\n"
        "}\n"
        : "=r"(ok)
        : "r"(hfa_smem_u32(bar)), "r"(parity)
        : "memory");
    return ok != 0;
}
__device__ __forceinline__ bool hfa_mbar_test_wait(uint64_t *bar, uint32_t parity)
{
    uint32_t ok;
    asm volatile(
        "{\n"
        ".reg .pred p;\n"
        "mbarrier.test_wait.parity.shared::cta.b64 p, [%1], %2;\n"
        "selp.u32 %0, 1, 0, p;\n"
        "}\n"
        : "=r"(ok)
        : "r"(hfa_smem_u32(bar)), "r"(parity)
        : "memory");
    return ok != 0;
}
__device__ __forceinline__ void hfa_mbar_arrive(uint64_t *bar)
{
    asm volatile("mbarrier.arrive.shared::cta.b64 _, [%0];" ::"r"(hfa_smem_u32(bar)) : "memory");
}
__device__ __forceinline__ void hfa_mbar_wait(uint64_t *bar, uint32_t parity)
{
    uint32_t spins = 0;
    while (!hfa_mbar_try_wait(bar, parity)) {
        if (++spins > (1u << 24)) __trap();
    }
}

__device__ __forceinline__ float hfa_ldg_f32_64B(const float *p)
{
    float v;
    asm volatile("ld.global.L2::64B.f32 %0, [%1];" : "=f"(v) : "l"(p));
    return v;
}

__device__ __forceinline__ float hfa_advance(float a, float curr, double ratio)
{
    return __double2float_rn(__dadd_rn((double)a, __dmul_rn((double)curr, ratio)));
}

__device__ __forceinline__ float hfa_exp_neg(float x)
{
#ifndef HFA_FAST_EXP
    return expf(x);
#else
    float y;
    asm("ex2.approx.ftz.f32 %0, %1;" : "=f"(y) : "f"(__fmul_rn(x, 1.4426950408889634f)));
    return y;
#endif
}

template <typename T> __device__ __forceinline__ float hfa_to_float(T v);
template <> __device__ __forceinline__ float hfa_to_float<float>(float v) { return v; }
template <> __device__ __forceinline__ float hfa_to_float<__half>(__half v) { return __half2float(v); }
template <> __device__ __forceinline__ float hfa_to_float<__nv_bfloat16>(__nv_bfloat16 v)
{
    return __bfloat162float(v);
}

struct HfaResultPtrs {
    int32_t *status, *n_seg, *end_state;
    float *final_score, *total_conf;
    int32_t *ph_idx_seq, *ph_time_int;
    double *intervals;
};

struct HfaLaunchCtx {
    HfaWs ws;
    int32_t n_utt;
    int32_t vocab;
    double frame_length;
    cudaStream_t stream;
};
```

hubertfa_b200/csrc/hfa_dp_skew.cu:

```cuda
#include <cstdlib>

#include "hfa_common.cuh"

namespace {

__device__ __forceinline__ float sk_lds_f32(uint32_t addr)
{
    float v;
    asm volatile("ld.shared.f32 %0, [%1];" : "=f"(v) : "r"(addr));
    return v;
}
__device__ __forceinline__ float2 sk_lds_f2(uint32_t addr)
{
    float2 v;
    asm volatile("ld.shared.v2.f32 {%0, %1}, [%2];" : "=f"(v.x), "=f"(v.y) : "r"(addr));
    return v;
}
__device__ __forceinline__ void sk_sts_f32(uint32_t addr, float v)
{
    asm volatile("st.shared.f32 [%0], %1;" ::"r"(addr), "f"(v) : "memory");
}
__device__ __forceinline__ int sk_lds_i32(uint32_t addr)
{
    int v;
    asm volatile("ld.shared.s32 %0, [%1];" : "=r"(v) : "r"(addr) : "memory");
    return v;
}
__device__ __forceinline__ void sk_sts_i32(uint32_t addr, int v)
{
    asm volatile("st.shared.s32 [%0], %1;" ::"r"(addr), "r"(v) : "memory");
}
__device__ __forceinline__ void sk_mbar_init(uint32_t bar, uint32_t count)
{
    asm volatile("mbarrier.init.shared::cta.b64 [%0], %1;" ::"r"(bar), "r"(count) : "memory");
}
__device__ __forceinline__ void sk_mbar_expect_tx(uint32_t bar, uint32_t bytes)
{
    asm volatile("mbarrier.arrive.expect_tx.shared::cta.b64 _, [%0], %1;" ::"r"(bar), "r"(bytes) : "memory");
}
__device__ __forceinline__ void sk_mbar_arrive(uint32_t bar)
{
    asm volatile("mbarrier.arrive.shared::cta.b64 _, [%0];" ::"r"(bar) : "memory");
}
__device__ __forceinline__ void sk_mbar_wait(uint32_t bar, uint32_t parity, uint32_t limit)
{
    uint32_t spins = 0;
    for (;;) {
        uint32_t ok;
        asm volatile(
            "{\n"
            ".reg .pred p;\n"
            "mbarrier.try_wait.parity.shared::cta.b64 p, [%1], %2;\n"
            "selp.u32 %0, 1, 0, p;\n"
            "}\n"
            : "=r"(ok)
            : "r"(bar), "r"(parity)
            : "memory");
        if (ok) return;
        if (++spins > limit) __trap();
    }
}
__device__ __forceinline__ bool sk_mbar_test(uint32_t bar, uint32_t parity)
{
    uint32_t ok;
    asm volatile(
        "{\n"
        ".reg .pred p;\n"
        "mbarrier.test_wait.parity.shared::cta.b64 p, [%1], %2;\n"
        "selp.u32 %0, 1, 0, p;\n"
        "}\n"
        : "=r"(ok)
        : "r"(bar), "r"(parity)
        : "memory");
    return ok != 0;
}
__device__ __forceinline__ void sk_bulk_load(uint32_t dst, const void *src, uint32_t bytes, uint32_t bar)
{
    asm volatile("cp.async.bulk.shared::cta.global.mbarrier::complete_tx::bytes [%0], [%1], %2, [%3];" ::"r"(dst),
                 "l"(src), "r"(bytes), "r"(bar)
                 : "memory");
}
__device__ __forceinline__ void sk_tensor_load_2d(uint32_t dst, const void *tmap, int x, int y, uint32_t bar)
{
    asm volatile(
        "cp.async.bulk.tensor.2d.shared::cta.global.tile.mbarrier::complete_tx::bytes [%0], [%1, {%2, %3}], [%4];" ::"r"(dst),
        "l"(tmap), "r"(x), "r"(y), "r"(bar)
        : "memory");
}
__device__ __forceinline__ void sk_bulk_store(void *dst, uint32_t src, uint32_t bytes)
{
    asm volatile("cp.async.bulk.global.shared::cta.bulk_group [%0], [%1], %2;" ::"l"(dst), "r"(src), "r"(bytes) : "memory");
}
__device__ __forceinline__ bool sk_elect_one()
{
    uint32_t pred;
    asm volatile(
        "{\n"
        ".reg .pred p;\n"
        "elect.sync _|p, 0xffffffff;\n"
        "selp.u32 %0, 1, 0, p;\n"
        "}\n"
        : "=r"(pred));
    return pred != 0;
}
__device__ __forceinline__ void sk_bulk_wait_read_1() { asm volatile("cp.async.bulk.wait_group.read 1;" ::: "memory"); }
__device__ __forceinline__ void sk_bulk_wait_read_0() { asm volatile("cp.async.bulk.wait_group.read 0;" ::: "memory"); }

__device__ __forceinline__ ulonglong2 sk_ld_slot(const ulonglong2 *p)
{
    ulonglong2 v;
    asm volatile("ld.relaxed.gpu.global.v2.u64 {%0, %1}, [%2];" : "=l"(v.x), "=l"(v.y) : "l"(p) : "memory");
    return v;
}
__device__ __forceinline__ void sk_st_slot(ulonglong2 *p, unsigned long long a, unsigned long long b)
{
    asm volatile("st.relaxed.gpu.global.v2.u64 [%0], {%1, %2};" ::"l"(p), "l"(a), "l"(b) : "memory");
}
__device__ __forceinline__ void sk_st_word(unsigned long long *p, unsigned long long a)
{
    asm volatile("st.relaxed.gpu.global.u64 [%0], %1;" ::"l"(p), "l"(a) : "memory");
}
__device__ __forceinline__ unsigned long long sk_pack(float v, uint32_t tag)
{
    return (unsigned long long)__float_as_uint(v) | ((unsigned long long)tag << 32);
}

__device__ __forceinline__ void sk_select(float up1, float stay, float up2, double pe, uint32_t sp_hi, uint32_t mr,
                                          float &dp, double &P, uint32_t &acc)
{
    asm("{\n\t"
        ".reg .pred q1, q2, q3;\n\t"
        ".reg .f32 m;\n\t"
        ".reg .f64 pn;\n\t"
        ".reg .b32 lo, hi;\n\t"
        "setp.gt.f32 q1, %3, %4;\n\t"
        "max.f32 m, %4, %3;\n\t"
        "setp.gt.f32 q2, %5, m;\n\t"
        "max.f32 %0, m, %5;\n\t"
        "@q1 lop3.b32 %2, %2, %8, 0x0000ffff, 0xf8;\n\t"
        "@q2 lop3.b32 %2, %2, %8, 0xffff0000, 0xf8;\n\t"
        "or.pred q3, q1, q2;\n\t"
        "setp.gt.or.f64 q3, %6, %1, q3;\n\t"
        "selp.f64 pn, %6, %1, q3;\n\t"
        "mov.b64 {lo, hi}, pn;\n\t"
        "and.b32 hi, hi, %7;\n\t"
        "mov.b64 %1, {lo, hi};\n\t"
        "}"
        : "=&f"(dp), "+d"(P), "+r"(acc)
        : "f"(up1), "f"(stay), "f"(up2), "d"(pe), "r"(sp_hi), "r"(mr));
}
__device__ __forceinline__ void sk_select_guarded(float up1, float stay, float up2, double pe, uint32_t sp_hi,
                                                  uint32_t mr, int live, float &dp, double &P, uint32_t &acc)
{
    asm("{\n\t"
        ".reg .pred pl, q1, q2, q3;\n\t"
        ".reg .f32 m, dn;\n\t"
        ".reg .f64 pn;\n\t"
        ".reg .b32 lo, hi, msk;\n\t"
        "setp.ne.b32 pl, %9, 0;\n\t"
        "setp.gt.and.f32 q1, %3, %4, pl;\n\t"
        "max.f32 m, %4, %3;\n\t"
        "setp.gt.and.f32 q2, %5, m, pl;\n\t"
        "max.f32 dn, m, %5;\n\t"
        "selp.f32 %0, dn, %0, pl;\n\t"
        "@q1 lop3.b32 %2, %2, %8, 0x0000ffff, 0xf8;\n\t"
        "@q2 lop3.b32 %2, %2, %8, 0xffff0000, 0xf8;\n\t"
        "or.pred q3, q1, q2;\n\t"
        "setp.gt.or.f64 q3, %6, %1, q3;\n\t"
        "and.pred q3, q3, pl;\n\t"
        "selp.f64 pn, %6, %1, q3;\n\t"
        "mov.b64 {lo, hi}, pn;\n\t"
        "selp.b32 msk, %7, 0xffffffff, pl;\n\t"
        "and.b32 hi, hi, msk;\n\t"
        "mov.b64 %1, {lo, hi};\n\t"
        "}"
        : "+f"(dp), "+d"(P), "+r"(acc)
        : "f"(up1), "f"(stay), "f"(up2), "d"(pe), "r"(sp_hi), "r"(mr), "r"(live));
}

constexpr int SK_BOXW = HFA_SKEW_BOX;
constexpr int BLK = HFA_SKEW_BLK;
constexpr uint32_t SK_ROW_B = SK_BOXW * 4u;
constexpr uint32_t SK_STG_B = BLK * SK_ROW_B;
constexpr uint32_t SK_EDGE_B = BLK * 8u;
constexpr uint32_t SK_DPST_B = BLK * 128u;
constexpr uint32_t SK_PUB_B = (2 * BLK + BLK + 32) * 4u;
constexpr int SK_LOOK = 3;
constexpr int SK_NBUF = 3;
static_assert(BLK == 16 || BLK == 32, "a block is one or two backpointer words long");

template <int NSTG> struct SkSmem {
    static constexpr uint32_t TILE = 0;
    static constexpr uint32_t EDGE = TILE + (NSTG + 1) * SK_STG_B;
    static constexpr uint32_t DPST = EDGE + (NSTG + 1) * SK_EDGE_B;
    static constexpr uint32_t PUB = DPST + SK_NBUF * SK_DPST_B;
    static constexpr uint32_t FULL = PUB + SK_NBUF * SK_PUB_B;
    static constexpr uint32_t READY = FULL + NSTG * 8;
    static constexpr uint32_t DONE = READY + NSTG * 8;
    static constexpr uint32_t SLOT = DONE + NSTG * 8;
    static constexpr uint32_t BYTES = SLOT + 16;
};

template <int D, int NSTG, bool KEEP, bool DUMP>
__global__ void __launch_bounds__(64)
hfa_dp_skew_kernel(HfaWs ws, int item_begin, int32_t *ticket, float *__restrict__ dp_dump, int force_slow)
{
    using SM = SkSmem<NSTG>;
    constexpr int R = NSTG * BLK;
    constexpr int Q = (31 * D + BLK - 1) / BLK;
    constexpr int PF = NSTG - 1 - Q;
    static_assert(D >= 2, "advance scores must be at least two iterations old when they are consumed");
    static_assert(PF >= 1, "ring too small for this skew");
    extern __shared__ __align__(128) unsigned char smem_raw[];
    uint32_t sm0;
    {
        const uint32_t a = hfa_smem_u32(smem_raw);
        asm volatile("mov.u32 %0, %1;" : "=r"(sm0) : "r"(a));
    }

    if (threadIdx.x == 0) {
        unsigned hw_slot;
        asm volatile("mov.u32 %0, %%warpid;" : "=r"(hw_slot));
        sk_sts_i32(sm0 + SM::SLOT + 4u, (int)((hw_slot >> 2) & 1u));
        sk_sts_i32(sm0 + SM::SLOT, (int)atomicInc(reinterpret_cast<unsigned int *>(ticket), gridDim.x - 1));
#pragma unroll
        for (int s = 0; s < NSTG; ++s) {
            sk_mbar_init(sm0 + SM::FULL + 8u * s, 1);
            sk_mbar_init(sm0 + SM::READY + 8u * s, 32);
            sk_mbar_init(sm0 + SM::DONE + 8u * s, 32);
        }
        hfa_fence_mbar_init();
    }
    __syncthreads();
    const int lane = threadIdx.x & 31;
    const bool producer =
        __shfl_sync(0xffffffffu, (threadIdx.x >> 5) ^ (unsigned)sk_lds_i32(sm0 + SM::SLOT + 4u), 0) != 0;
    const int item = item_begin + sk_lds_i32(sm0 + SM::SLOT);
    const HfaBandItem bi = ws.band_items[item];
    const int u = bi.utt, w = bi.band;
    const HfaUtt m = ws.utt[u];
    const int T = m.T, S = m.S, Sp = m.Sp;
    const bool has_left = w > 0, has_right = w + 1 < hfa_skew_strips(Sp);
    const int c0 = HFA_SKEW_OWN * w;
    const int NB = hfa_skew_blocks(D, T);

    if (producer) {
        const float2 *g_edge = ws.edge2 + m.edge_off;
        const unsigned char *tmap = static_cast<const unsigned char *>(ws.tmaps) + (size_t)m.tmap * 128;
        float *g_dp = (KEEP && m.dp_off >= 0) ? ws.dp_store + m.dp_off + (int64_t)w * NB * (BLK * 32) : nullptr;
        const int edge_len = (T + 15) & ~15;
        auto issue = [&](int i, int st) {
            const int t0 = i * BLK;
            const uint32_t bar = sm0 + SM::FULL + 8u * (uint32_t)st;
            if (t0 >= T) {
                sk_mbar_arrive(bar);
                return;
            }
            const uint32_t ebytes = (uint32_t)min(BLK, edge_len - t0) * 8u;
            const uint32_t bytes = SK_STG_B + ebytes;
            sk_mbar_expect_tx(bar, st == 0 ? 2u * bytes : bytes);
            sk_tensor_load_2d(sm0 + SM::TILE + (uint32_t)st * SK_STG_B, tmap, c0 & ~3, t0, bar);
            sk_bulk_load(sm0 + SM::EDGE + (uint32_t)st * SK_EDGE_B, g_edge + t0, ebytes, bar);
            if (st == 0) {
                sk_tensor_load_2d(sm0 + SM::TILE + (uint32_t)NSTG * SK_STG_B, tmap, c0 & ~3, t0, bar);
                sk_bulk_load(sm0 + SM::EDGE + (uint32_t)NSTG * SK_EDGE_B, g_edge + t0, ebytes, bar);
            }
        };
        static_assert(PF + 1 <= NSTG, "prologue fills distinct stages");
        if (sk_elect_one())
            for (int i = 0; i <= PF && i < NB; ++i) issue(i, i);

        const ulonglong2 *left_x = reinterpret_cast<const ulonglong2 *>(ws.band_xchg) +
                                   (has_left ? ws.band_items[item - 1].xoff : 0);
        ulonglong2 *my_x = reinterpret_cast<ulonglong2 *>(ws.band_xchg) + bi.xoff;
        auto slot_needed = [&](int jj) { const int t = BLK * jj + lane; return has_left && lane < BLK && t >= 1 && t < T; };
        ulonglong2 xv = make_ulonglong2(0ull, 0ull);
        if (slot_needed(0)) xv = sk_ld_slot(left_x + lane);

        int a = 0, st_a = 0, buf_b = 0;
        uint32_t par_a = 0;
        int b = 0, st_b = 0;
        uint32_t par_b = 0;
        int st_issue = (PF + 1) % NSTG;
        uint32_t spins = 0;
        while (b < NB) {
            if (b < a && __all_sync(0xffffffffu, sk_mbar_test(sm0 + SM::DONE + 8u * (uint32_t)st_b, par_b))) {
                if (has_right) {
#pragma unroll
                    for (int q = lane; q < 2 * BLK; q += 32) {
                        const int half = q / BLK, i = q % BLK;
                        const int t = BLK * b + i - (31 - half) * D;
                        if (t >= 1 && t < T)
                            sk_st_word(reinterpret_cast<unsigned long long *>(my_x + t) + half,
                                       sk_pack(sk_lds_f32(sm0 + SM::PUB + (uint32_t)buf_b * SK_PUB_B + 4u * (uint32_t)q),
                                               (uint32_t)t + 1u));
                    }
                }
                if (sk_elect_one()) {
                    if (KEEP && g_dp != nullptr) {
                        sk_bulk_store(g_dp + (int64_t)b * (BLK * 32), sm0 + SM::DPST + (uint32_t)buf_b * SK_DPST_B,
                                      SK_DPST_B);
                        hfa_bulk_commit();
                    }
                    if (b + PF + 1 < NB) issue(b + PF + 1, st_issue);
                }
                if (++st_issue == NSTG) st_issue = 0;
                if (++st_b == NSTG) {
                    st_b = 0;
                    par_b ^= 1u;
                }
                if (++buf_b == SK_NBUF) buf_b = 0;
                ++b;
                spins = 0;
                continue;
            }
            if (a < NB && a <= b + SK_NBUF - 1 &&
                __all_sync(0xffffffffu, sk_mbar_test(sm0 + SM::FULL + 8u * (uint32_t)st_a, par_a))) {
                bool go = true;
                if (has_left) {
                    const int t = BLK * a + lane;
                    const bool need = slot_needed(a);
                    ulonglong2 *src = const_cast<ulonglong2 *>(left_x) + t;
                    const uint32_t tag = (uint32_t)t + 1u;
                    const bool ok = !need || ((uint32_t)(xv.x >> 32) == tag && (uint32_t)(xv.y >> 32) == tag);
                    go = __all_sync(0xffffffffu, ok);
                    if (!go) {
                        if (!ok) xv = sk_ld_slot(src);
                    } else {
                        const ulonglong2 v = xv;
                        xv = slot_needed(a + 1) ? sk_ld_slot(src + BLK) : make_ulonglong2(0ull, 0ull);
                        if (lane < BLK) {
                            const float a30 = need ? __uint_as_float((uint32_t)v.y) : 0.0f;
                            const float a31 = need ? __uint_as_float((uint32_t)v.x) : 0.0f;
                            const uint32_t row_sa = sm0 + SM::TILE + (uint32_t)st_a * SK_STG_B + (uint32_t)lane * SK_ROW_B +
                                                    4u * (uint32_t)(c0 & 3);
                            sk_sts_f32(row_sa, a30);
                            sk_sts_f32(row_sa + 4u, a31);
                            if (st_a == 0) {
                                sk_sts_f32(row_sa + (uint32_t)NSTG * SK_STG_B, a30);
                                sk_sts_f32(row_sa + (uint32_t)NSTG * SK_STG_B + 4u, a31);
                            }
                            if (need) sk_st_slot(src, 0ull, 0ull);
                        }
                        hfa_fence_async_smem();
                    }
                }
                if (go) {
                    if (KEEP && a >= SK_NBUF && sk_elect_one()) {
                        if (a == b + SK_NBUF - 1) sk_bulk_wait_read_0();
                        else sk_bulk_wait_read_1();
                    }
                    sk_mbar_arrive(sm0 + SM::READY + 8u * (uint32_t)st_a);
                    if (++st_a == NSTG) {
                        st_a = 0;
                        par_a ^= 1u;
                    }
                    ++a;
                    spins = 0;
                    continue;
                }
            }
            if (++spins > (1u << 26)) __trap();
        }
        if (KEEP && sk_elect_one()) hfa_bulk_wait_all();
        return;
    }

    const int s = c0 + lane;
    const bool ghost = has_left && lane < 2;
    const bool real = !ghost && s < Sp;
    const int n_rows = (T + 15) >> 4;
    uint32_t *g_bp = ws.bp + m.bp_off;
    const double ratio = __ddiv_rn((double)T, (double)S);
    const float NEG = HFA_NEG_INF, POS = __uint_as_float(0x7f800000u);

    const int32_t *ids = ws.ids + m.seg_off;
    uint32_t sp_hi = 0xffffffffu;
    float jcap = NEG;
    if (s < S) {
        if (ids[s] == 0) sp_hi = 0u;
        if (s >= 2 && ids[s - 1] == 0) jcap = POS;
    }
    const bool lead_sp = (ids[0] == 0) && (S > 1);
    const bool seeded = !ghost && (s == 0 || (s == 1 && lead_sp));
    const float cap1 = (s == 0) ? NEG : POS;

    int st_wait = 0;
    uint32_t par_wait = 0;
    int buf = 0;

    float dp = NEG;
    double P = __longlong_as_double(0xfff0000000000000ll);
    uint32_t bits = 0;
    float q1[D], q2[2 * D];
#pragma unroll
    for (int i = 0; i < D; ++i) q1[i] = NEG;
#pragma unroll
    for (int i = 0; i < 2 * D; ++i) q2[i] = NEG;

    int u_row = ((-lane * D) % R + R) % R;
    const uint32_t tile_sa = sm0 + SM::TILE + 4u * (uint32_t)(lane + (c0 & 3));
    const uint32_t edge_sa = sm0 + SM::EDGE;
    const uint32_t dpst_sa = sm0 + SM::DPST + 4u * (uint32_t)lane;
    const int o_res = (lane * D) & 15;
    const int q_rows = (lane * D + 15) >> 4;
    const uint32_t m16 = o_res ? ((0xffffu << (16 - o_res)) & 0xffffu) : 0xffffu;
    const uint32_t hi_mask = m16 | (m16 << 16);
    const uint32_t mrot0 = 0x00010001u << ((16 - o_res) & 15);
    const uint32_t pub_sa = sm0 + SM::PUB +
                            ((has_right && lane == 31) ? 0u : (has_right && lane == 30) ? 4u * BLK
                                                                                        : 8u * BLK + 4u * (uint32_t)lane);
    uint32_t *bp_ptr = g_bp + (int64_t)(-q_rows) * Sp + s;
    int bp_row = -q_rows;

    auto flush_bits = [&](uint32_t acc, bool all_valid) {
        if (real && (all_valid || (bp_row >= 0 && bp_row < n_rows))) *bp_ptr = bits | (acc & hi_mask);
        bits = acc & ~hi_mask;
        bp_ptr += Sp;
        ++bp_row;
    };

    for (int j = 0; j < NB; ++j) {
        sk_mbar_wait(sm0 + SM::READY + 8u * (uint32_t)st_wait, par_wait, 1u << 26);
        const int st_cur = st_wait;
        if (++st_wait == NSTG) {
            st_wait = 0;
            par_wait ^= 1u;
        }

        const uint32_t e_sa = tile_sa + (uint32_t)u_row * SK_ROW_B;
        const uint32_t d_sa = edge_sa + (uint32_t)u_row * 8u;
        const uint32_t k_sa = dpst_sa + (uint32_t)buf * SK_DPST_B;
        const uint32_t p_sa = pub_sa + (uint32_t)buf * SK_PUB_B;
        const bool steady = (BLK * j - 31 * D >= 1) && (BLK * j + BLK - 1 <= T - 1);

        if ((j == 0 && !has_left) || force_slow) {
            uint32_t acc = 0;
#pragma unroll 1
            for (int k = 0; k < BLK; ++k) {
                const int t = BLK * j + k - lane * D;
                const bool live = (t >= 1) && (t < T);
                const float e = sk_lds_f32(e_sa + SK_ROW_B * k);
                const float2 ed = sk_lds_f2(d_sa + 8u * k);
                const float base = __fadd_rn(dp, e);
                const float stay = __fadd_rn(base, ed.y);
                const float adv = __double2float_rn(__dadd_rn((double)__fadd_rn(base, ed.x), P));
                const float advx = ghost ? e : adv;
                const float n1 = fminf(__shfl_up_sync(0xffffffffu, advx, 1), cap1);
                const float n2 = fminf(__shfl_up_sync(0xffffffffu, advx, 2), jcap);
                const float up1 = q1[0], up2 = q2[0];
#pragma unroll
                for (int i = 0; i + 1 < D; ++i) q1[i] = q1[i + 1];
                q1[D - 1] = n1;
#pragma unroll
                for (int i = 0; i + 1 < 2 * D; ++i) q2[i] = q2[i + 1];
                q2[2 * D - 1] = n2;
                sk_sts_f32(p_sa + 4u * k, advx);
                const float mm = fmaxf(stay, up1);
                const bool b1 = up1 > stay, b2 = up2 > mm;
                const double pe = __dmul_rn((double)e, ratio);
                if (live) {
                    dp = fmaxf(mm, up2);
                    if (b1) acc |= 1u << (t & 15);
                    if (b2) acc |= 0x10000u << (t & 15);
                    const double pn = (b1 || b2 || pe > P) ? pe : P;
                    P = __hiloint2double(__double2hiint(pn) & (int)sp_hi, __double2loint(pn));
                }
                if (t == 0 && seeded) {
                    dp = e;
                    P = pe;
                }
                if (KEEP) sk_sts_f32(k_sa + 128u * k, dp);
                if (DUMP) {
                    if (!ghost && s < S && t >= 0 && t < T) dp_dump[m.cell_off + (int64_t)t * S + s] = dp;
                }
                if ((k & 15) == 15) {
                    flush_bits(acc, false);
                    acc = 0;
                }
            }
        } else {
            float ev[BLK];
            float2 dv[BLK];
#pragma unroll
            for (int k = 0; k < SK_LOOK; ++k) {
                ev[k] = sk_lds_f32(e_sa + SK_ROW_B * k);
                dv[k] = sk_lds_f2(d_sa + 8u * k);
            }
            float r1[BLK + D], r2[BLK + 2 * D];
#pragma unroll
            for (int i = 0; i < D; ++i) r1[i] = q1[i];
#pragma unroll
            for (int i = 0; i < 2 * D; ++i) r2[i] = q2[i];
            uint32_t mr = mrot0, acc = 0;
            if (!DUMP && steady) {
#pragma unroll
                for (int k = 0; k < BLK; ++k) {
                    if (k + SK_LOOK < BLK) {
                        ev[k + SK_LOOK] = sk_lds_f32(e_sa + SK_ROW_B * (k + SK_LOOK));
                        dv[k + SK_LOOK] = sk_lds_f2(d_sa + 8u * (k + SK_LOOK));
                    }
                    const float e = ev[k];
                    const float base = __fadd_rn(dp, e);
                    const float stay = __fadd_rn(base, dv[k].y);
                    const float adv = __double2float_rn(__dadd_rn((double)__fadd_rn(base, dv[k].x), P));
                    const float advx = ghost ? e : adv;
                    r1[k + D] = fminf(__shfl_up_sync(0xffffffffu, advx, 1), cap1);
                    r2[k + 2 * D] = fminf(__shfl_up_sync(0xffffffffu, advx, 2), jcap);
                    sk_sts_f32(p_sa + 4u * k, advx);
                    const double pe = __dmul_rn((double)e, ratio);
                    sk_select(r1[k], stay, r2[k], pe, sp_hi, mr, dp, P, acc);
                    mr = __funnelshift_l(mr, mr, 1);
                    if (KEEP) sk_sts_f32(k_sa + 128u * k, dp);
                    if ((k & 15) == 15) {
                        flush_bits(acc, true);
                        acc = 0;
                    }
                }
            } else {
                const int tb = BLK * j - lane * D - 1;
#pragma unroll
                for (int k = 0; k < BLK; ++k) {
                    if (k + SK_LOOK < BLK) {
                        ev[k + SK_LOOK] = sk_lds_f32(e_sa + SK_ROW_B * (k + SK_LOOK));
                        dv[k + SK_LOOK] = sk_lds_f2(d_sa + 8u * (k + SK_LOOK));
                    }
                    const int live = (unsigned)(tb + k) < (unsigned)(T - 1);
                    const float e = ev[k];
                    const float base = __fadd_rn(dp, e);
                    const float stay = __fadd_rn(base, dv[k].y);
                    const float adv = __double2float_rn(__dadd_rn((double)__fadd_rn(base, dv[k].x), P));
                    const float advx = ghost ? e : adv;
                    r1[k + D] = fminf(__shfl_up_sync(0xffffffffu, advx, 1), cap1);
                    r2[k + 2 * D] = fminf(__shfl_up_sync(0xffffffffu, advx, 2), jcap);
                    sk_sts_f32(p_sa + 4u * k, advx);
                    const double pe = __dmul_rn((double)e, ratio);
                    sk_select_guarded(r1[k], stay, r2[k], pe, sp_hi, mr, live, dp, P, acc);
                    mr = __funnelshift_l(mr, mr, 1);
                    if (KEEP) sk_sts_f32(k_sa + 128u * k, dp);
                    if (DUMP) {
                        const int t = tb + 1 + k;
                        if (!ghost && s < S && t >= 0 && t < T) dp_dump[m.cell_off + (int64_t)t * S + s] = dp;
                    }
                    if ((k & 15) == 15) {
                        flush_bits(acc, false);
                        acc = 0;
                    }
                }
            }
#pragma unroll
            for (int i = 0; i < D; ++i) q1[i] = r1[BLK + i];
#pragma unroll
            for (int i = 0; i < 2 * D; ++i) q2[i] = r2[BLK + i];
        }
        if (KEEP) hfa_fence_async_smem();
        sk_mbar_arrive(sm0 + SM::DONE + 8u * (uint32_t)st_cur);
        if (++buf == SK_NBUF) buf = 0;
        u_row += BLK;
        if (u_row >= R) u_row -= R;
    }
    if (real && o_res != 0 && bp_row >= 0 && bp_row < n_rows) *bp_ptr = bits;
    if (!ghost) {
        if (s == S - 1) ws.dp_last[2 * u] = dp;
        if (s == S - 2) ws.dp_last[2 * u + 1] = dp;
    }
}

template <int D, int NSTG, bool KEEP, bool DUMP>
cudaError_t launch_skew(const HfaLaunchCtx &c, int item_begin, int n_items, int32_t *ticket, float *dp_dump,
                        int force_slow)
{
    const size_t smem = SkSmem<NSTG>::BYTES;
    cudaError_t e = cudaFuncSetAttribute(hfa_dp_skew_kernel<D, NSTG, KEEP, DUMP>,
                                         cudaFuncAttributeMaxDynamicSharedMemorySize, (int)smem);
    if (e != cudaSuccess) return e;
    hfa_dp_skew_kernel<D, NSTG, KEEP, DUMP><<<n_items, 64, smem, c.stream>>>(c.ws, item_begin, ticket, dp_dump,
                                                                            force_slow);
    return cudaGetLastError();
}

template <int D, int NSTG>
cudaError_t launch_skew_d(const HfaLaunchCtx &c, int item_begin, int n_items, int32_t *ticket, bool keep_dp,
                          float *dp_dump, int force_slow)
{
    if (dp_dump != nullptr)
        return keep_dp ? launch_skew<D, NSTG, true, true>(c, item_begin, n_items, ticket, dp_dump, force_slow)
                       : launch_skew<D, NSTG, false, true>(c, item_begin, n_items, ticket, dp_dump, force_slow);
    return keep_dp ? launch_skew<D, NSTG, true, false>(c, item_begin, n_items, ticket, dp_dump, force_slow)
                   : launch_skew<D, NSTG, false, false>(c, item_begin, n_items, ticket, dp_dump, force_slow);
}

}

cudaError_t hfa_launch_dp_skew(const HfaLaunchCtx &c, int d, int item_begin, int n_items, int32_t *ticket,
                               bool keep_dp, float *dp_dump)
{
    if (n_items <= 0) return cudaSuccess;
    if (c.ws.tmaps == nullptr) return cudaErrorNotSupported;
    const char *sl = getenv("HFA_SKEW_SLOW");
    const int force_slow = (sl && sl[0] == '1') ? 1 : 0;
    constexpr int NS = HFA_SKEW_BLK == 32 ? 5 : 12;
    if (d == 2) return launch_skew_d<2, NS>(c, item_begin, n_items, ticket, keep_dp, dp_dump, force_slow);
    if (d == 3) return launch_skew_d<3, NS>(c, item_begin, n_items, ticket, keep_dp, dp_dump, force_slow);
    return cudaErrorInvalidValue;
}
```

hubertfa_b200/csrc/hfa_emission.cu:

```cuda
#include "hfa_common.cuh"

#define HFA_EMIS_ROWS 64
#define HFA_EMIS_WARPS 8

namespace {

__device__ __forceinline__ float warp_max(float v)
{
#pragma unroll
    for (int o = 16; o > 0; o >>= 1) v = fmaxf(v, __shfl_xor_sync(0xffffffffu, v, o));
    return v;
}
__device__ __forceinline__ float warp_sum(float v)
{
#pragma unroll
    for (int o = 16; o > 0; o >>= 1) v = __fadd_rn(v, __shfl_xor_sync(0xffffffffu, v, o));
    return v;
}

__device__ __forceinline__ float edge_pred(float x)
{
    const float sg = __fdiv_rn(1.0f, __fadd_rn(1.0f, expf(-x)));
    const float v = __fdiv_rn(__fsub_rn(sg, 0.1f), 0.8f);
    return fminf(fmaxf(v, 0.0f), 1.0f);
}

__device__ __forceinline__ void edge_logs(float p, float p_prev, float2 &out)
{
    double ep = __dadd_rn((double)p, (double)p_prev);
    ep = fmin(fmax(ep, 0.0), 1.0);
    out.x = (float)log(__dadd_rn(ep, 1e-6));
    out.y = (float)log(__dadd_rn(__dsub_rn(1.0, ep), 1e-6));
}

__device__ __forceinline__ float lds_f32(uint32_t addr)
{
    float v;
    asm volatile("ld.shared.f32 %0, [%1];" : "=f"(v) : "r"(addr));
    return v;
}

#define HFA_EMIS_ID_CAP 8192

__device__ __forceinline__ int4 hfa_ids4(const int32_t *ids, int S, int V, int s4)
{
    return make_int4(s4 < S ? __ldg(ids + s4) : V, s4 + 1 < S ? __ldg(ids + s4 + 1) : V,
                     s4 + 2 < S ? __ldg(ids + s4 + 2) : V, s4 + 3 < S ? __ldg(ids + s4 + 3) : V);
}

template <typename TIn> __device__ __forceinline__ float hfa_ld_edge(const TIn *p);
template <> __device__ __forceinline__ float hfa_ld_edge<float>(const float *p)
{
    float v;
    asm volatile("ld.global.L2::64B.f32 %0, [%1];" : "=f"(v) : "l"(p));
    return v;
}
template <> __device__ __forceinline__ float hfa_ld_edge<__half>(const __half *p)
{
    unsigned short v;
    asm volatile("ld.global.L2::64B.u16 %0, [%1];" : "=h"(v) : "l"(p));
    return __half2float(__ushort_as_half(v));
}
template <> __device__ __forceinline__ float hfa_ld_edge<__nv_bfloat16>(const __nv_bfloat16 *p)
{
    unsigned short v;
    asm volatile("ld.global.L2::64B.u16 %0, [%1];" : "=h"(v) : "l"(p));
    return __bfloat162float(__ushort_as_bfloat16(v));
}

template <typename TIn>
__device__ __forceinline__ void edge_block(const HfaWs &ws, const HfaUtt &m, const HfaInput &in,
                                           int t_base, int tid)
{
    if (tid < HFA_EMIS_ROWS) {
        const int t = t_base + tid;
        if (t < m.T) {
            const TIn *edge = reinterpret_cast<const TIn *>(in.edge);
            const float p = edge_pred(hfa_ld_edge<TIn>(edge + (int64_t)t * in.edge_st));
            const float pp = (t > 0) ? edge_pred(hfa_ld_edge<TIn>(edge + (int64_t)(t - 1) * in.edge_st)) : 0.0f;
            float2 lg;
            edge_logs(p, pp, lg);
            ws.edge2[m.edge_off + t] = lg;
            ws.edge_p[m.edge_off + t] = p;
        }
    }
}

#define HFA_EMIS_BLOCK_MAX_V 255

template <typename TIn>
__global__ void __launch_bounds__(HFA_EMIS_WARPS * 32, 5)
hfa_emission_block_kernel(HfaWs ws, int n_utt, int V, int sp_cap)
{
    constexpr int RPW = HFA_EMIS_ROWS / HFA_EMIS_WARPS;
    extern __shared__ __align__(16) unsigned char smem_raw[];
    const int VP = (V + 1) | 1;
    const int mask_words = (V + 31) >> 5;
    int32_t *ids_sm = reinterpret_cast<int32_t *>(smem_raw);
    uint32_t *mask_sm = reinterpret_cast<uint32_t *>(ids_sm + sp_cap);
    int32_t *kept_sm = reinterpret_cast<int32_t *>(mask_sm + 8);
    float2 *stat_sm = reinterpret_cast<float2 *>(kept_sm + 256);
    float *xs = reinterpret_cast<float *>(stat_sm + HFA_EMIS_ROWS);

    const int tid = threadIdx.x, lane = tid & 31, warp = tid >> 5;
    const int u = ws.block_utt[blockIdx.x];
    const HfaUtt m = ws.utt[u];
    const HfaInput in = ws.inputs[u];
    const bool compact = m.Dp > 0;
    const int T = m.T, S = compact ? m.Dp : m.S, Sp = compact ? m.Dp : m.Sp;
    const int t_base = (blockIdx.x - ws.row_blocks[u]) * HFA_EMIS_ROWS;
    const TIn *frame = reinterpret_cast<const TIn *>(in.frame);
    if (compact && t_base == 0 && threadIdx.x == 0) ws.emis_mode[u] = 1;

    {
        const TIn *rowp[RPW];
#pragma unroll
        for (int r = 0; r < RPW; ++r)
            rowp[r] = frame + (int64_t)min(t_base + warp + HFA_EMIS_WARPS * r, T - 1) * in.frame_st +
                      (int64_t)lane * in.frame_sv;
        const int64_t vstep = 32 * in.frame_sv;
        float *xw = xs + warp * VP + lane;
        for (int v = lane; v < V; v += 32) {
            float xv[RPW];
#pragma unroll
            for (int r = 0; r < RPW; ++r) {
                xv[r] = hfa_to_float<TIn>(*rowp[r]);
                rowp[r] += vstep;
            }
#pragma unroll
            for (int r = 0; r < RPW; ++r) xw[r * HFA_EMIS_WARPS * VP] = xv[r];
            xw += 32;
        }
    }
    if (lane < RPW) xs[(warp + HFA_EMIS_WARPS * lane) * VP + V] = HFA_NEG_INF;

    if (tid < 8) mask_sm[tid] = (tid == 0) ? 1u : 0u;
    __syncthreads();
    const int32_t *ids = compact ? ws.col_ids + m.seg_off + 4 * (int64_t)u : ws.ids + m.seg_off;
    for (int s = tid; s < Sp; s += blockDim.x) {
        const int id = (s < S) ? ids[s] : V;
        if (s < sp_cap) ids_sm[s] = id;
        if (id < V) atomicOr(&mask_sm[id >> 5], 1u << (id & 31));
    }
    __syncthreads();
    int n_kept = 0;
#pragma unroll
    for (int w = 0; w < 8; ++w) n_kept += (w < mask_words) ? __popc(mask_sm[w]) : 0;
    if (tid < V && ((mask_sm[tid >> 5] >> (tid & 31)) & 1u)) {
        int pos = __popc(mask_sm[tid >> 5] & ((1u << (tid & 31)) - 1u));
        for (int w = 0; w < (tid >> 5); ++w) pos += __popc(mask_sm[w]);
        kept_sm[pos] = tid;
    }
    __syncthreads();

    {
        const float *row = xs + (tid >> 2) * VP;
        const int part = tid & 3;
        float mx = HFA_NEG_INF;
        for (int k = part; k < n_kept; k += 4) mx = fmaxf(mx, row[kept_sm[k]]);
        mx = fmaxf(mx, __shfl_xor_sync(0xffffffffu, mx, 1));
        mx = fmaxf(mx, __shfl_xor_sync(0xffffffffu, mx, 2));
        float sum = 0.0f;
        for (int k = part; k < n_kept; k += 4) sum = __fadd_rn(sum, hfa_exp_neg(__fsub_rn(row[kept_sm[k]], mx)));
        sum = __fadd_rn(sum, __shfl_xor_sync(0xffffffffu, sum, 1));
        sum = __fadd_rn(sum, __shfl_xor_sync(0xffffffffu, sum, 2));
        if (part == 0) stat_sm[tid >> 2] = make_float2(mx, logf(sum));
    }
    __syncthreads();

    {
        uint32_t goff[2][4];
#pragma unroll
        for (int it = 0; it < 2; ++it) {
            const int s4 = min(lane * 4 + 128 * it, Sp - 4);
            const int4 id4 = *reinterpret_cast<const int4 *>(ids_sm + s4);
            goff[it][0] = (uint32_t)id4.x * 4u; goff[it][1] = (uint32_t)id4.y * 4u;
            goff[it][2] = (uint32_t)id4.z * 4u; goff[it][3] = (uint32_t)id4.w * 4u;
        }
        const uint32_t xs_sa = hfa_smem_u32(xs);
        const int rows_here = min(RPW, (T - t_base - warp + HFA_EMIS_WARPS - 1) / HFA_EMIS_WARPS);
        float *dst = ws.emis + m.emis_off + (int64_t)(t_base + warp) * Sp + lane * 4;
        const int dst_step = HFA_EMIS_WARPS * Sp;
        const bool st0 = lane * 4 < Sp, st1 = lane * 4 + 128 < Sp;
#pragma unroll
        for (int r = 0; r < RPW; ++r) {
            if (r >= rows_here) break;
            const int rr = warp + HFA_EMIS_WARPS * r;
            const float2 st = stat_sm[rr];
            const uint32_t rb = xs_sa + (uint32_t)(rr * VP) * 4u;
            float4 o;
            o.x = __fsub_rn(__fsub_rn(lds_f32(rb + goff[0][0]), st.x), st.y);
            o.y = __fsub_rn(__fsub_rn(lds_f32(rb + goff[0][1]), st.x), st.y);
            o.z = __fsub_rn(__fsub_rn(lds_f32(rb + goff[0][2]), st.x), st.y);
            o.w = __fsub_rn(__fsub_rn(lds_f32(rb + goff[0][3]), st.x), st.y);
            if (st0) *reinterpret_cast<float4 *>(dst + r * dst_step) = o;
            if (Sp > 128) {
                o.x = __fsub_rn(__fsub_rn(lds_f32(rb + goff[1][0]), st.x), st.y);
                o.y = __fsub_rn(__fsub_rn(lds_f32(rb + goff[1][1]), st.x), st.y);
                o.z = __fsub_rn(__fsub_rn(lds_f32(rb + goff[1][2]), st.x), st.y);
                o.w = __fsub_rn(__fsub_rn(lds_f32(rb + goff[1][3]), st.x), st.y);
                if (st1) *reinterpret_cast<float4 *>(dst + r * dst_step + 128) = o;
            }
        }
        if (Sp > 256) {
            const int s_sm = min(Sp, sp_cap);
            for (int r = 0; r < rows_here; ++r) {
                const int rr = warp + HFA_EMIS_WARPS * r;
                const float2 st = stat_sm[rr];
                for (int s4 = lane * 4 + 256; s4 < s_sm; s4 += 128) {
                    const int4 id4 = *reinterpret_cast<const int4 *>(ids_sm + s4);
                    float4 o;
                    o.x = __fsub_rn(__fsub_rn(xs[rr * VP + id4.x], st.x), st.y);
                    o.y = __fsub_rn(__fsub_rn(xs[rr * VP + id4.y], st.x), st.y);
                    o.z = __fsub_rn(__fsub_rn(xs[rr * VP + id4.z], st.x), st.y);
                    o.w = __fsub_rn(__fsub_rn(xs[rr * VP + id4.w], st.x), st.y);
                    *reinterpret_cast<float4 *>(dst + r * dst_step + (s4 - lane * 4)) = o;
                }
                for (int s4 = lane * 4 + s_sm; s4 < Sp; s4 += 128) {
                    const int4 id4 = hfa_ids4(ids, S, V, s4);
                    float4 o;
                    o.x = __fsub_rn(__fsub_rn(xs[rr * VP + id4.x], st.x), st.y);
                    o.y = __fsub_rn(__fsub_rn(xs[rr * VP + id4.y], st.x), st.y);
                    o.z = __fsub_rn(__fsub_rn(xs[rr * VP + id4.z], st.x), st.y);
                    o.w = __fsub_rn(__fsub_rn(xs[rr * VP + id4.w], st.x), st.y);
                    *reinterpret_cast<float4 *>(dst + r * dst_step + (s4 - lane * 4)) = o;
                }
            }
        }
    }
    edge_block<TIn>(ws, m, in, t_base, tid);
}

template <typename TIn>
__global__ void __launch_bounds__(HFA_EMIS_ROWS)
hfa_edge_kernel(HfaWs ws)
{
    const int u = ws.block_utt[blockIdx.x];
    const HfaUtt m = ws.utt[u];
    const HfaInput in = ws.inputs[u];
    edge_block<TIn>(ws, m, in, (blockIdx.x - ws.row_blocks[u]) * HFA_EMIS_ROWS, threadIdx.x);
}

template <int NJ, typename TIn>
__device__ __forceinline__ void hfa_row_stats(const TIn *row, const int (&kreg)[16], int part, int n_kept,
                                              float &mx, float &sum)
{
    float xv[NJ];
#pragma unroll
    for (int j = 0; j < NJ; ++j) {
        const float x = hfa_to_float<TIn>(row[kreg[j]]);
        xv[j] = (part + 4 * j < n_kept) ? x : HFA_NEG_INF;
    }
#pragma unroll
    for (int j = 0; j < NJ; ++j) mx = fmaxf(mx, xv[j]);
    mx = fmaxf(mx, __shfl_xor_sync(0xffffffffu, mx, 1));
    mx = fmaxf(mx, __shfl_xor_sync(0xffffffffu, mx, 2));
#pragma unroll
    for (int j = 0; j < NJ; ++j)
        sum = __fadd_rn(sum, hfa_exp_neg(__fsub_rn(xv[j], mx)));
}

template <typename TIn>
__global__ void __launch_bounds__(HFA_EMIS_WARPS * 32)
hfa_emission_stream_kernel(HfaWs ws, int n_blocks, int V, int sp_cap, int stage_bytes)
{
    constexpr int RPW = HFA_EMIS_ROWS / HFA_EMIS_WARPS;
    extern __shared__ __align__(128) unsigned char smem_raw[];
    unsigned char *stage0 = smem_raw;
    int32_t *ids_sm = reinterpret_cast<int32_t *>(smem_raw + 2 * stage_bytes);
    uint32_t *mask_sm = reinterpret_cast<uint32_t *>(ids_sm + sp_cap);
    int32_t *kept_sm = reinterpret_cast<int32_t *>(mask_sm + 8);
    float2 *stat_sm = reinterpret_cast<float2 *>(kept_sm + 256);
    uint64_t *bar = reinterpret_cast<uint64_t *>(stat_sm + HFA_EMIS_ROWS);
    int32_t *shift_sm = reinterpret_cast<int32_t *>(bar + 2);

    const int tid = threadIdx.x, lane = tid & 31, warp = tid >> 5;
    const int blk0 = (int)(((int64_t)blockIdx.x * n_blocks) / gridDim.x);
    const int blk1 = (int)(((int64_t)(blockIdx.x + 1) * n_blocks) / gridDim.x);
    if (blk0 >= blk1) return;

    auto issue = [&](int blk, int s) {
        const int u = ws.block_utt[blk];
        const HfaUtt m = ws.utt[u];
        const HfaInput in = ws.inputs[u];
        const int t_base = (blk - ws.row_blocks[u]) * HFA_EMIS_ROWS;
        const int rows = min(HFA_EMIS_ROWS, m.T - t_base);
        const unsigned char *src = reinterpret_cast<const unsigned char *>(in.frame) +
                                   (int64_t)t_base * in.frame_st * (int64_t)sizeof(TIn);
        const uint32_t shift = (uint32_t)(reinterpret_cast<uintptr_t>(src) & 15u);
        const uint32_t bytes =
            (shift + (uint32_t)(((int64_t)(rows - 1) * in.frame_st + V) * (int64_t)sizeof(TIn)) + 15u) & ~15u;
        shift_sm[s] = (int32_t)shift;
        hfa_mbar_expect_tx(&bar[s], bytes);
        hfa_bulk_load(stage0 + (size_t)s * stage_bytes, src - shift, bytes, &bar[s]);
    };
    if (tid == 0) {
        hfa_mbar_init(&bar[0], 1);
        hfa_mbar_init(&bar[1], 1);
        hfa_fence_mbar_init();
        issue(blk0, 0);
    }
    __syncthreads();

    int cur_u = -1;
    int S = 0, Sp = 4, T = 0, n_kept = 0;
    uint32_t goff[2][4] = {{0, 0, 0, 0}, {0, 0, 0, 0}};
    int lpr = 32;
    int kreg[16];
#pragma unroll
    for (int j = 0; j < 16; ++j) kreg[j] = 0;
    HfaUtt m;
    HfaInput in;
    for (int blk = blk0; blk < blk1; ++blk) {
        const int s = (blk - blk0) & 1;
        if (tid == 0 && blk + 1 < blk1) issue(blk + 1, s ^ 1);
        const int u = ws.block_utt[blk];
        if (u != cur_u) {
            cur_u = u;
            m = ws.utt[u];
            in = ws.inputs[u];
            const bool compact = m.Dp > 0;
            S = compact ? m.Dp : m.S; Sp = compact ? m.Dp : m.Sp; T = m.T;
            const int mask_words = (V + 31) >> 5;
            if (tid < 8) mask_sm[tid] = (tid == 0) ? 1u : 0u;
            __syncthreads();
            const int32_t *ids = compact ? ws.col_ids + m.seg_off + 4 * (int64_t)u : ws.ids + m.seg_off;
            for (int q = tid; q < Sp; q += blockDim.x) {
                const int id = (q < S) ? ids[q] : V;
                if (q < sp_cap) ids_sm[q] = id;
                if (id < V) atomicOr(&mask_sm[id >> 5], 1u << (id & 31));
            }
            if (compact && tid == 0 && blk == ws.row_blocks[u]) ws.emis_mode[u] = 1;
            __syncthreads();
            n_kept = 0;
#pragma unroll
            for (int w = 0; w < 8; ++w) n_kept += (w < mask_words) ? __popc(mask_sm[w]) : 0;
            if (tid < V && ((mask_sm[tid >> 5] >> (tid & 31)) & 1u)) {
                int pos = __popc(mask_sm[tid >> 5] & ((1u << (tid & 31)) - 1u));
                for (int w = 0; w < (tid >> 5); ++w) pos += __popc(mask_sm[w]);
                kept_sm[pos] = tid;
            }
            lpr = (Sp <= 32) ? 8 : (Sp <= 64) ? 16 : 32;
#pragma unroll
            for (int it = 0; it < 2; ++it) {
                const int s4 = min((lane & (lpr - 1)) * 4 + 128 * it, Sp - 4);
                const int4 id4 = *reinterpret_cast<const int4 *>(ids_sm + s4);
                goff[it][0] = (uint32_t)id4.x; goff[it][1] = (uint32_t)id4.y;
                goff[it][2] = (uint32_t)id4.z; goff[it][3] = (uint32_t)id4.w;
            }
            __syncthreads();
#pragma unroll
            for (int j = 0; j < 16; ++j) {
                const int k = (lane & 3) + 4 * j;
                kreg[j] = (k < n_kept && k < 256) ? kept_sm[k] : 0;
            }
        }
        const int t_base = (blk - ws.row_blocks[u]) * HFA_EMIS_ROWS;
        const int row_st = (int)in.frame_st;

        hfa_mbar_wait(&bar[s], (uint32_t)(((blk - blk0) >> 1) & 1));
        const TIn *xs = reinterpret_cast<const TIn *>(stage0 + (size_t)s * stage_bytes + shift_sm[s]);

        {
            const int rr = RPW * warp + (lane >> 2);
            const TIn *row = xs + rr * row_st;
            const int part = lane & 3;
            float mx = HFA_NEG_INF, sum = 0.0f;
            if (n_kept <= 64) {
                const int nj = (n_kept + 3) >> 2;
                if (nj <= 8) hfa_row_stats<8, TIn>(row, kreg, part, n_kept, mx, sum);
                else if (nj <= 10) hfa_row_stats<10, TIn>(row, kreg, part, n_kept, mx, sum);
                else if (nj <= 12) hfa_row_stats<12, TIn>(row, kreg, part, n_kept, mx, sum);
                else if (nj <= 14) hfa_row_stats<14, TIn>(row, kreg, part, n_kept, mx, sum);
                else hfa_row_stats<16, TIn>(row, kreg, part, n_kept, mx, sum);
            } else {
                for (int k = part; k < n_kept; k += 4) mx = fmaxf(mx, hfa_to_float<TIn>(row[kept_sm[k]]));
                mx = fmaxf(mx, __shfl_xor_sync(0xffffffffu, mx, 1));
                mx = fmaxf(mx, __shfl_xor_sync(0xffffffffu, mx, 2));
                for (int k = part; k < n_kept; k += 4)
                    sum = __fadd_rn(sum, hfa_exp_neg(__fsub_rn(hfa_to_float<TIn>(row[kept_sm[k]]), mx)));
            }
            sum = __fadd_rn(sum, __shfl_xor_sync(0xffffffffu, sum, 1));
            sum = __fadd_rn(sum, __shfl_xor_sync(0xffffffffu, sum, 2));
            if (part == 0) stat_sm[rr] = make_float2(mx, logf(sum));
        }
        __syncwarp();

        {
            const int rows_here = max(0, min(RPW, T - t_base - RPW * warp));
            float *dst = ws.emis + m.emis_off + (int64_t)(t_base + RPW * warp) * Sp + lane * 4;
            const int dst_step = Sp;
            const bool st0 = lane * 4 < Sp, st1 = lane * 4 + 128 < Sp;
            auto val = [&](const TIn *row, uint32_t id, const float2 st) {
                const float x = (id < (uint32_t)V) ? hfa_to_float<TIn>(row[id]) : HFA_NEG_INF;
                return __fsub_rn(__fsub_rn(x, st.x), st.y);
            };
            if (lpr < 32) {
                const int sub = (lpr == 8) ? (lane >> 3) : (lane >> 4);
                const int col = (lane & (lpr - 1)) * 4;
                const int rpp = 32 / lpr;
                const bool stc = col < Sp;
                float *dst_n = ws.emis + m.emis_off + (int64_t)(t_base + RPW * warp) * Sp + col;
#pragma unroll
                for (int r0 = 0; r0 < RPW; r0 += 2) {
                    if (r0 >= rows_here) break;
                    if (rpp == 4 && (r0 & 2)) continue;
                    const int r = r0 + sub;
                    const int rr = RPW * warp + r;
                    const float2 st = stat_sm[rr];
                    const TIn *row = xs + rr * row_st;
                    float4 o;
                    o.x = val(row, goff[0][0], st); o.y = val(row, goff[0][1], st);
                    o.z = val(row, goff[0][2], st); o.w = val(row, goff[0][3], st);
                    if (stc && r < rows_here) *reinterpret_cast<float4 *>(dst_n + r * dst_step) = o;
                }
            } else {
#pragma unroll
            for (int r = 0; r < RPW; ++r) {
                if (r >= rows_here) break;
                const int rr = RPW * warp + r;
                const float2 st = stat_sm[rr];
                const TIn *row = xs + rr * row_st;
                float4 o;
                o.x = val(row, goff[0][0], st); o.y = val(row, goff[0][1], st);
                o.z = val(row, goff[0][2], st); o.w = val(row, goff[0][3], st);
                if (st0) *reinterpret_cast<float4 *>(dst + r * dst_step) = o;
                if (Sp > 128) {
                    o.x = val(row, goff[1][0], st); o.y = val(row, goff[1][1], st);
                    o.z = val(row, goff[1][2], st); o.w = val(row, goff[1][3], st);
                    if (st1) *reinterpret_cast<float4 *>(dst + r * dst_step + 128) = o;
                }
            }
            }
            if (Sp > 256) {
                const int s_sm = min(Sp, sp_cap);
                for (int r = 0; r < rows_here; ++r) {
                    const int rr = RPW * warp + r;
                    const float2 st = stat_sm[rr];
                    const TIn *row = xs + rr * row_st;
                    for (int s4 = lane * 4 + 256; s4 < s_sm; s4 += 128) {
                        const int4 id4 = *reinterpret_cast<const int4 *>(ids_sm + s4);
                        float4 o;
                        o.x = val(row, (uint32_t)id4.x, st); o.y = val(row, (uint32_t)id4.y, st);
                        o.z = val(row, (uint32_t)id4.z, st); o.w = val(row, (uint32_t)id4.w, st);
                        *reinterpret_cast<float4 *>(dst + r * dst_step + (s4 - lane * 4)) = o;
                    }
                    if (Sp > s_sm) {
                        const int32_t *ids = m.Dp > 0 ? ws.col_ids + m.seg_off + 4 * (int64_t)cur_u
                                                      : ws.ids + m.seg_off;
                        for (int s4 = lane * 4 + s_sm; s4 < Sp; s4 += 128) {
                            const int4 id4 = hfa_ids4(ids, S, V, s4);
                            float4 o;
                            o.x = val(row, (uint32_t)id4.x, st); o.y = val(row, (uint32_t)id4.y, st);
                            o.z = val(row, (uint32_t)id4.z, st); o.w = val(row, (uint32_t)id4.w, st);
                            *reinterpret_cast<float4 *>(dst + r * dst_step + (s4 - lane * 4)) = o;
                        }
                    }
                }
            }
        }
        __syncthreads();
    }
}

template <typename TIn>
__global__ void __launch_bounds__(HFA_EMIS_WARPS * 32)
hfa_emission_wide_kernel(HfaWs ws, int n_utt, int V, int sp_cap)
{
    constexpr int RPW = HFA_EMIS_ROWS / HFA_EMIS_WARPS;
    extern __shared__ __align__(16) unsigned char smem_raw[];
    int32_t *ids_sm = reinterpret_cast<int32_t *>(smem_raw);
    uint32_t *mask_sm = reinterpret_cast<uint32_t *>(ids_sm + sp_cap);
    const int mask_words = (V + 31) >> 5;
    float *rows_sm = reinterpret_cast<float *>(mask_sm + ((mask_words + 3) & ~3));
    const int VS = V + 1;

    const int tid = threadIdx.x, lane = tid & 31, warp = tid >> 5;
    const int u = ws.block_utt[blockIdx.x];
    const HfaUtt m = ws.utt[u];
    const HfaInput in = ws.inputs[u];
    const bool compact = m.Dp > 0;
    const int T = m.T, S = compact ? m.Dp : m.S, Sp = compact ? m.Dp : m.Sp;
    const int t_base = (blockIdx.x - ws.row_blocks[u]) * HFA_EMIS_ROWS;
    const TIn *frame = reinterpret_cast<const TIn *>(in.frame);
    float *g_out = ws.emis + m.emis_off;
    if (compact && t_base == 0 && threadIdx.x == 0) ws.emis_mode[u] = 1;

    for (int w = tid; w < mask_words; w += blockDim.x) mask_sm[w] = (w == 0) ? 1u : 0u;
    __syncthreads();
    const int32_t *ids = compact ? ws.col_ids + m.seg_off + 4 * (int64_t)u : ws.ids + m.seg_off;
    for (int s = tid; s < Sp; s += blockDim.x) {
        const int id = (s < S) ? ids[s] : V;
        if (s < sp_cap) ids_sm[s] = id;
        if (id < V) atomicOr(&mask_sm[id >> 5], 1u << (id & 31));
    }
    __syncthreads();

    float *rowbuf = rows_sm + (size_t)warp * VS;
    if (lane == 0) rowbuf[V] = HFA_NEG_INF;
    __syncwarp();
    for (int j = 0; j < RPW; ++j) {
        const int t = t_base + warp + HFA_EMIS_WARPS * j;
        if (t >= T) continue;
        const TIn *src = frame + (int64_t)t * in.frame_st;
        float mr = HFA_NEG_INF;
        for (int v = lane; v < V; v += 32) {
            float xv = hfa_to_float<TIn>(src[(int64_t)v * in.frame_sv]);
            if (!((mask_sm[v >> 5] >> (v & 31)) & 1u)) xv = __fsub_rn(xv, 1e9f);
            rowbuf[v] = xv;
            mr = fmaxf(mr, xv);
        }
        mr = warp_max(mr);
        float sum = 0.0f;
        for (int v = lane; v < V; v += 32) sum = __fadd_rn(sum, hfa_exp_neg(__fsub_rn(rowbuf[v], mr)));
        const float l = logf(warp_sum(sum));
        __syncwarp();
        float *dst = g_out + (int64_t)t * Sp;
        for (int s4 = lane * 4; s4 < Sp; s4 += 128) {
            const int4 id4 = s4 < sp_cap ? *reinterpret_cast<const int4 *>(ids_sm + s4)
                                         : hfa_ids4(ids, S, V, s4);
            float4 o;
            o.x = __fsub_rn(__fsub_rn(rowbuf[id4.x], mr), l);
            o.y = __fsub_rn(__fsub_rn(rowbuf[id4.y], mr), l);
            o.z = __fsub_rn(__fsub_rn(rowbuf[id4.z], mr), l);
            o.w = __fsub_rn(__fsub_rn(rowbuf[id4.w], mr), l);
            *reinterpret_cast<float4 *>(dst + s4) = o;
        }
        __syncwarp();
    }
    edge_block<TIn>(ws, m, in, t_base, tid);
}

__global__ void __launch_bounds__(256)
hfa_pack_kernel(HfaWs ws, int n_utt, const float *__restrict__ prob_log,
                const float *__restrict__ edge_log, const float *__restrict__ not_edge_log,
                const float *__restrict__ edge_pred_in)
{
    const int tid = threadIdx.x;
    const int u = ws.block_utt[blockIdx.x];
    const HfaUtt m = ws.utt[u];
    const int T = m.T, S = m.S, Sp = m.Sp;
    const int t_base = (blockIdx.x - ws.row_blocks[u]) * HFA_EMIS_ROWS;
    const int rows = min(HFA_EMIS_ROWS, T - t_base);
    const float *src = prob_log + m.cell_off + (int64_t)t_base * S;
    float *dst = ws.emis + m.emis_off + (int64_t)t_base * Sp;
    if (m.Dp > 0 && t_base == 0 && tid == 0) ws.emis_mode[u] = 0;
    for (int64_t i = tid; i < (int64_t)rows * Sp; i += blockDim.x) {
        const int r = (int)(i / Sp), s = (int)(i - (int64_t)r * Sp);
        dst[i] = (s < S) ? src[(int64_t)r * S + s] : HFA_NEG_INF;
    }
    if (tid < rows) {
        const int t = t_base + tid;
        ws.edge2[m.edge_off + t] = make_float2(edge_log[m.frame_off + t], not_edge_log[m.frame_off + t]);
        ws.edge_p[m.edge_off + t] = edge_pred_in ? edge_pred_in[m.frame_off + t] : 0.0f;
    }
}

__global__ void __launch_bounds__(256)
hfa_unpack_emis_kernel(HfaWs ws, float *__restrict__ out)
{
    const int u = ws.block_utt[blockIdx.x];
    const HfaUtt m = ws.utt[u];
    const bool compact = m.Dp > 0 && ws.emis_mode[u] != 0;
    const int Ep = compact ? m.Dp : m.Sp, S = m.S;
    const int t_base = (blockIdx.x - ws.row_blocks[u]) * HFA_EMIS_ROWS;
    const int rows = min(HFA_EMIS_ROWS, m.T - t_base);
    const uint8_t *cm = ws.colmap + m.seg_off;
    for (int64_t i = threadIdx.x; i < (int64_t)rows * S; i += blockDim.x) {
        const int r = (int)(i / S), s = (int)(i - (int64_t)r * S);
        out[m.cell_off + (int64_t)(t_base + r) * S + s] =
            ws.emis[m.emis_off + (int64_t)(t_base + r) * Ep + (compact ? cm[s] : s)];
    }
}

}

cudaError_t hfa_launch_unpack_emissions(const HfaLaunchCtx &c, int total_row_blocks, float *out)
{
    if (total_row_blocks <= 0) return cudaSuccess;
    hfa_unpack_emis_kernel<<<total_row_blocks, 256, 0, c.stream>>>(c.ws, out);
    return cudaGetLastError();
}

template <typename TIn>
static cudaError_t launch_emission_t(const HfaLaunchCtx &c, int blocks, int max_sp, int64_t max_row_stride,
                                     int *n_launched)
{
    *n_launched = 1;
    const int V = c.vocab;
    max_sp = max_sp < HFA_EMIS_ID_CAP ? max_sp : HFA_EMIS_ID_CAP;
    cudaError_t e;
    const int64_t stage = max_row_stride > 0
        ? ((HFA_EMIS_ROWS * max_row_stride * (int64_t)sizeof(TIn) + 32 + 127) & ~(int64_t)127) : 0;
    if (V <= HFA_EMIS_BLOCK_MAX_V && stage > 0 && stage <= 48 * 1024) {
        const size_t smem = 2 * (size_t)stage + (size_t)max_sp * 4 + 8 * 4 + 256 * 4 + HFA_EMIS_ROWS * 8 +
                            2 * 8 + 2 * 4 + 16;
        e = cudaFuncSetAttribute(hfa_emission_stream_kernel<TIn>,
                                 cudaFuncAttributeMaxDynamicSharedMemorySize, (int)smem);
        if (e != cudaSuccess) return e;
        int per_sm = 0;
        e = cudaOccupancyMaxActiveBlocksPerMultiprocessor(&per_sm, hfa_emission_stream_kernel<TIn>,
                                                          HFA_EMIS_WARPS * 32, smem);
        if (e != cudaSuccess) return e;
        per_sm = per_sm < 1 ? 1 : (per_sm > 4 ? 4 : per_sm);
        int dev = 0, n_sm = 148;
        if (cudaGetDevice(&dev) == cudaSuccess) cudaDeviceGetAttribute(&n_sm, cudaDevAttrMultiProcessorCount, dev);
        const int grid = blocks < n_sm * per_sm ? blocks : n_sm * per_sm;
        *n_launched = 2;
        hfa_emission_stream_kernel<TIn><<<grid, HFA_EMIS_WARPS * 32, smem, c.stream>>>(
            c.ws, blocks, V, max_sp, (int)stage);
        return cudaGetLastError();
    }
    if (V <= HFA_EMIS_BLOCK_MAX_V) {
        const int VP = (V + 1) | 1;
        const size_t smem = (size_t)max_sp * 4 + 8 * 4 + 256 * 4 + HFA_EMIS_ROWS * 8 +
                            (size_t)HFA_EMIS_ROWS * VP * 4;
        e = cudaFuncSetAttribute(hfa_emission_block_kernel<TIn>,
                                 cudaFuncAttributeMaxDynamicSharedMemorySize, (int)smem);
        if (e != cudaSuccess) return e;
        hfa_emission_block_kernel<TIn><<<blocks, HFA_EMIS_WARPS * 32, smem, c.stream>>>(c.ws, c.n_utt,
                                                                                    V, max_sp);
    } else {
        const int mask_words = (V + 31) >> 5;
        const size_t smem = (size_t)max_sp * 4 + (size_t)((mask_words + 3) & ~3) * 4 +
                            (size_t)HFA_EMIS_WARPS * (V + 1) * 4;
        e = cudaFuncSetAttribute(hfa_emission_wide_kernel<TIn>,
                                 cudaFuncAttributeMaxDynamicSharedMemorySize, (int)smem);
        if (e != cudaSuccess) return e;
        hfa_emission_wide_kernel<TIn><<<blocks, HFA_EMIS_WARPS * 32, smem, c.stream>>>(c.ws, c.n_utt,
                                                                                   V, max_sp);
    }
    return cudaGetLastError();
}

cudaError_t hfa_launch_emission(const HfaLaunchCtx &c, int total_row_blocks, int max_sp, int dtype,
                                int64_t max_row_stride, int *n_launched)
{
    *n_launched = 0;
    if (total_row_blocks <= 0) return cudaSuccess;
    if (dtype == 0) return launch_emission_t<float>(c, total_row_blocks, max_sp, max_row_stride, n_launched);
    if (dtype == 1) return launch_emission_t<__half>(c, total_row_blocks, max_sp, max_row_stride, n_launched);
    if (dtype == 2)
        return launch_emission_t<__nv_bfloat16>(c, total_row_blocks, max_sp, max_row_stride, n_launched);
    return cudaErrorInvalidValue;
}

cudaError_t hfa_launch_edge(const HfaLaunchCtx &c, int total_row_blocks, int dtype)
{
    if (total_row_blocks <= 0) return cudaSuccess;
    if (dtype == 0) hfa_edge_kernel<float><<<total_row_blocks, HFA_EMIS_ROWS, 0, c.stream>>>(c.ws);
    else if (dtype == 1) hfa_edge_kernel<__half><<<total_row_blocks, HFA_EMIS_ROWS, 0, c.stream>>>(c.ws);
    else if (dtype == 2) hfa_edge_kernel<__nv_bfloat16><<<total_row_blocks, HFA_EMIS_ROWS, 0, c.stream>>>(c.ws);
    else return cudaErrorInvalidValue;
    return cudaGetLastError();
}

cudaError_t hfa_launch_pack(const HfaLaunchCtx &c, int total_row_blocks, const float *prob_log,
                            const float *edge_log, const float *not_edge_log, const float *edge_pred)
{
    if (total_row_blocks <= 0) return cudaSuccess;
    hfa_pack_kernel<<<total_row_blocks, 256, 0, c.stream>>>(c.ws, c.n_utt, prob_log, edge_log,
                                                            not_edge_log, edge_pred);
    return cudaGetLastError();
}
```

hubertfa_b200/ops.py:

```python
from __future__ import annotations

import ctypes as C
from typing import Optional

import numpy as np
import torch

from . import _lib
from ._lib import HfaError, ResultLayout, check


def _stream_ptr() -> int:
    return int(torch.cuda.current_stream().cuda_stream)


def _require_cuda(t: torch.Tensor, what: str) -> None:
    if not t.is_cuda:
        raise HfaError(f"{what} must be a CUDA tensor: the aligner has no CPU path")


class AlignPlan:

    def __init__(self, T, S, ph_ids, vocab_size: int, frame_length: float):
        lib = _lib.load()
        self.T = np.ascontiguousarray(T, dtype=np.int32)
        self.S = np.ascontiguousarray(S, dtype=np.int32)
        self.ph_ids = np.ascontiguousarray(ph_ids, dtype=np.int32)
        if self.T.shape != self.S.shape or self.T.ndim != 1:
            raise ValueError("T and S must be 1-D arrays of the same length")
        if int(np.maximum(self.S, 0).sum()) != self.ph_ids.size:
            raise ValueError("ph_ids must hold sum(S) entries")
        self.n_utt = int(self.T.size)
        self.vocab_size = int(vocab_size)
        self.frame_length = float(frame_length)
        handle = C.c_void_p()
        check(lib.hfa_plan_create(self.n_utt, self.vocab_size, self.T.ctypes.data, self.S.ctypes.data,
                                  self.ph_ids.ctypes.data, self.frame_length, C.byref(handle)),
              "hfa_plan_create")
        self._h = handle
        self._lib = lib
        self.workspace_bytes = int(lib.hfa_plan_workspace_bytes(handle))
        self.total_frames = int(lib.hfa_plan_total_frames(handle))
        self.total_states = int(lib.hfa_plan_total_states(handle))
        self.total_cells = int(lib.hfa_plan_total_cells(handle))
        n1 = self.n_utt + 1
        self.frame_off = np.ctypeslib.as_array(lib.hfa_plan_frame_offsets(handle), shape=(n1,)).copy()
        self.seg_off = np.ctypeslib.as_array(lib.hfa_plan_seg_offsets(handle), shape=(n1,)).copy()
        self.layout = ResultLayout()
        check(lib.hfa_plan_result_layout(handle, C.byref(self.layout)), "hfa_plan_result_layout")
        self.result_bytes = int(self.layout.total_bytes)

    @property
    def handle(self) -> int:
        if self._h is None:
            raise HfaError("plan already destroyed")
        return int(self._h.value)

    def routing(self) -> dict:
        out = (C.c_int32 * 8)()
        check(self._lib.hfa_plan_routing(self._h, C.byref(out)))
        return dict(warp_utts=out[0], band_warps=out[1], band_k=out[2], big_band_warps=out[3],
                    big_band_k=out[4], cta_utts=out[5], keeps_dp=bool(out[6]), skew_d=out[7],
                    pair_utts=int(self._lib.hfa_plan_pair_utterances(self._h)),
                    stored_emission_bytes=int(self._lib.hfa_plan_stored_emission_bytes(self._h)))

    def algorithmic_bytes_fused(self, dtype: int = _lib.DTYPE_F32) -> int:
        return int(self._lib.hfa_plan_algorithmic_bytes_fused(self._h, dtype))

    def algorithmic_bytes(self, dtype: int = _lib.DTYPE_F32):
        out = (C.c_int64 * 3)()
        check(self._lib.hfa_plan_algorithmic_bytes(self._h, dtype, C.byref(out)))
        return {"emission": int(out[0]), "dp": int(out[1]), "backtrace": int(out[2])}

    def new_workspace(self, device) -> torch.Tensor:
        return torch.empty(max(self.workspace_bytes, 256), dtype=torch.uint8, device=device)

    def new_result(self, device) -> torch.Tensor:
        return torch.empty(self.result_bytes, dtype=torch.uint8, device=device)

    def upload(self, workspace: torch.Tensor) -> None:
        _require_cuda(workspace, "workspace")
        if workspace.numel() < self.workspace_bytes:
            raise HfaError("workspace too small for this plan")
        with torch.cuda.device(workspace.device):
            check(self._lib.hfa_plan_upload(self._h, workspace.data_ptr(), _stream_ptr()),
                  "hfa_plan_upload")

    def set_inputs(self, workspace: torch.Tensor, frame_ptrs, frame_st, frame_sv, edge_ptrs, edge_st):
        tabs = [np.ascontiguousarray(a, dtype=np.int64) for a in
                (frame_ptrs, frame_st, frame_sv, edge_ptrs, edge_st)]
        if any(a.shape != (self.n_utt,) for a in tabs):
            raise ValueError("input tables must have one entry per utterance")
        with torch.cuda.device(workspace.device):
            check(self._lib.hfa_set_inputs(self._h, workspace.data_ptr(), *[a.ctypes.data for a in tabs],
                                           _stream_ptr()), "hfa_set_inputs")

    INPUT_DESC = np.dtype([("frame", np.int64), ("edge", np.int64), ("frame_stride_t", np.int64),
                           ("frame_stride_v", np.int64), ("edge_stride", np.int64)])

    def input_table(self, frame_ptrs, frame_st, frame_sv, edge_ptrs, edge_st) -> np.ndarray:
        tab = np.zeros(self.n_utt, dtype=self.INPUT_DESC)
        for name, a in zip(self.INPUT_DESC.names, (frame_ptrs, edge_ptrs, frame_st, frame_sv, edge_st)):
            tab[name] = np.asarray(a, dtype=np.int64)
        ok = self.T > 0
        tma = bool(np.all(tab["frame_stride_v"][ok] == 1) and np.all(tab["frame_stride_t"][ok] >= self.vocab_size)
                   and np.all(tab["frame"][ok] % 4 == 0))
        stride = int(tab["frame_stride_t"][ok].max()) if ok.any() else 0
        return tab.view(np.uint8), (stride if tma else 0)

    def set_inputs_device(self, workspace: torch.Tensor, table: torch.Tensor, max_row_stride: int) -> None:
        _require_cuda(table, "input table")
        if table.numel() * table.element_size() < self.n_utt * self.INPUT_DESC.itemsize:
            raise HfaError("input table too small for this plan")
        with torch.cuda.device(workspace.device):
            check(self._lib.hfa_set_inputs_device(self._h, workspace.data_ptr(), table.data_ptr(),
                                                  int(max_row_stride), _stream_ptr()), "hfa_set_inputs_device")

    def views(self, blob: np.ndarray) -> dict:
        L, n, ns = self.layout, self.n_utt, self.total_states

        def v(off, dtype, count):
            return blob[off:off + count * np.dtype(dtype).itemsize].view(dtype)

        return dict(status=v(L.status, np.int32, n), n_seg=v(L.n_seg, np.int32, n),
                    end_state=v(L.end_state, np.int32, n), final_score=v(L.final_score, np.float32, n),
                    total_conf=v(L.total_conf, np.float32, n),
                    ph_idx_seq=v(L.ph_idx_seq, np.int32, ns), ph_time_int=v(L.ph_time_int, np.int32, ns),
                    intervals=v(L.intervals, np.float64, 2 * ns).reshape(ns, 2))

    def debug_region(self, workspace: torch.Tensor, which: str) -> torch.Tensor:
        code = {"emis": 0, "edge2": 1, "edge_p": 2, "bp": 3}[which]
        nb = C.c_int64()
        off = int(self._lib.hfa_plan_debug_region(self._h, code, C.byref(nb)))
        raw = workspace[off:off + int(nb.value)]
        if which == "bp":
            return raw.view(torch.int32)
        v = raw.view(torch.float32)
        return v.view(-1, 2) if which == "edge2" else v

    def close(self) -> None:
        if getattr(self, "_h", None) is not None:
            self._lib.hfa_plan_destroy(self._h)
            self._h = None

    def __del__(self):
        try:
            self.close()
        except Exception:
            pass


def _ptr(t: Optional[torch.Tensor]) -> Optional[int]:
    return None if t is None else t.data_ptr()


@torch.library.custom_op("hfa::emission", mutates_args=("workspace",), device_types="cuda")
def emission(workspace: torch.Tensor, plan: int, dtype: int) -> None:
    with torch.cuda.device(workspace.device):
        check(_lib.load().hfa_emission(plan, workspace.data_ptr(), dtype, _stream_ptr()), "hfa_emission")


@torch.library.custom_op("hfa::pack_emissions", mutates_args=("workspace",), device_types="cuda")
def pack_emissions(workspace: torch.Tensor, plan: int, prob_log: torch.Tensor, edge_log: torch.Tensor,
                   not_edge_log: torch.Tensor, edge_pred: Optional[torch.Tensor]) -> None:
    for t in (prob_log, edge_log, not_edge_log):
        if t.dtype != torch.float32 or not t.is_contiguous():
            raise HfaError("pack_emissions expects contiguous float32 tensors")
    with torch.cuda.device(workspace.device):
        check(_lib.load().hfa_pack_emissions(plan, workspace.data_ptr(), prob_log.data_ptr(),
                                             edge_log.data_ptr(), not_edge_log.data_ptr(),
                                             _ptr(edge_pred), _stream_ptr()), "hfa_pack_emissions")


@torch.library.custom_op("hfa::viterbi_forward", mutates_args=("workspace", "dp_dump"),
                         device_types="cuda")
def viterbi_forward(workspace: torch.Tensor, plan: int, dp_dump: Optional[torch.Tensor]) -> None:
    with torch.cuda.device(workspace.device):
        check(_lib.load().hfa_viterbi_forward(plan, workspace.data_ptr(), _ptr(dp_dump), _stream_ptr()),
              "hfa_viterbi_forward")


@torch.library.custom_op("hfa::backtrace", mutates_args=("workspace", "result", "frame_conf", "dp_path"),
                         device_types="cuda")
def backtrace(workspace: torch.Tensor, plan: int, result: torch.Tensor,
              frame_conf: Optional[torch.Tensor], dp_path: Optional[torch.Tensor]) -> None:
    with torch.cuda.device(workspace.device):
        check(_lib.load().hfa_backtrace(plan, workspace.data_ptr(), result.data_ptr(), _ptr(frame_conf),
                                        _ptr(dp_path), _stream_ptr()), "hfa_backtrace")


@torch.library.custom_op("hfa::align_batch", mutates_args=("workspace", "result", "frame_conf"),
                         device_types="cuda")
def align_batch(workspace: torch.Tensor, plan: int, dtype: int, result: torch.Tensor,
                frame_conf: Optional[torch.Tensor]) -> None:
    with torch.cuda.device(workspace.device):
        check(_lib.load().hfa_align_batch(plan, workspace.data_ptr(), dtype, result.data_ptr(),
                                          _ptr(frame_conf), _stream_ptr()), "hfa_align_batch")


@torch.library.custom_op("hfa::forward_fused", mutates_args=("workspace",), device_types="cuda")
def forward_fused(workspace: torch.Tensor, plan: int, dtype: int) -> None:
    with torch.cuda.device(workspace.device):
        check(_lib.load().hfa_forward_fused(plan, workspace.data_ptr(), dtype, _stream_ptr()), "hfa_forward_fused")


class GraphedStep:

    def __init__(self, plan: AlignPlan, workspace: torch.Tensor, result: torch.Tensor, host_result: torch.Tensor,
                 dtype: int, frame_conf: Optional[torch.Tensor] = None, table: Optional[torch.Tensor] = None,
                 max_row_stride: int = 0, warmup: int = 2):
        if not host_result.is_pinned():
            raise HfaError("host_result must be pinned memory")
        self.plan, self.host_result = plan, host_result
        dev = workspace.device

        def body():
            if table is not None:
                plan.set_inputs_device(workspace, table, max_row_stride)
            align_batch(workspace, plan.handle, dtype, result, frame_conf)
            host_result.copy_(result, non_blocking=True)

        with torch.cuda.device(dev):
            side = torch.cuda.Stream(device=dev)
            side.wait_stream(torch.cuda.current_stream())
            with torch.cuda.stream(side):
                for _ in range(max(warmup, 1)):
                    body()
            torch.cuda.current_stream().wait_stream(side)
            torch.cuda.synchronize(dev)
            self.graph = torch.cuda.CUDAGraph()
            with torch.cuda.graph(self.graph):
                body()

    def replay(self) -> None:
        self.graph.replay()


def unpack_backptr(plan: AlignPlan, workspace: torch.Tensor, utt: int) -> torch.Tensor:
    out = torch.empty((int(plan.T[utt]), int(plan.S[utt])), dtype=torch.int8, device=workspace.device)
    with torch.cuda.device(workspace.device):
        check(_lib.load().hfa_debug_unpack_backptr(plan.handle, workspace.data_ptr(), utt, out.data_ptr(),
                                                   _stream_ptr()), "hfa_debug_unpack_backptr")
    return out


def unpack_kept_dp(plan: AlignPlan, workspace: torch.Tensor, utt: int) -> torch.Tensor:
    out = torch.empty((int(plan.T[utt]), int(plan.S[utt])), dtype=torch.float32, device=workspace.device)
    with torch.cuda.device(workspace.device):
        check(_lib.load().hfa_debug_unpack_dp(plan.handle, workspace.data_ptr(), utt, out.data_ptr(),
                                              _stream_ptr()), "hfa_debug_unpack_dp")
    return out


def unpack_emissions(plan: AlignPlan, workspace: torch.Tensor) -> torch.Tensor:
    out = torch.empty(max(plan.total_cells, 1), dtype=torch.float32, device=workspace.device)
    with torch.cuda.device(workspace.device):
        check(_lib.load().hfa_debug_unpack_emissions(plan.handle, workspace.data_ptr(), out.data_ptr(),
                                                     _stream_ptr()), "hfa_debug_unpack_emissions")
    return out


def launch_count() -> int:
    return int(_lib.load().hfa_launch_count())


TORCH_TO_DTYPE = {torch.float32: _lib.DTYPE_F32, torch.float16: _lib.DTYPE_F16,
                  torch.bfloat16: _lib.DTYPE_BF16}


def ctc_greedy(logits: torch.Tensor) -> torch.Tensor:
    if logits.dim() != 2 or not logits.is_cuda:
        raise HfaError("ctc_greedy expects a CUDA tensor [T, V]")
    if logits.dtype not in TORCH_TO_DTYPE:
        logits = logits.float()
    T, V = int(logits.shape[0]), int(logits.shape[1])
    dev = logits.device
    scratch = torch.empty(max(T, 1), dtype=torch.int32, device=dev)
    out = torch.empty(max(T, 1), dtype=torch.int32, device=dev)
    n = torch.zeros(1, dtype=torch.int32, device=dev)
    with torch.cuda.device(dev):
        check(_lib.load().hfa_ctc_greedy(logits.data_ptr(), TORCH_TO_DTYPE[logits.dtype], T, V, logits.stride(0),
                                         logits.stride(1), scratch.data_ptr(), out.data_ptr(), n.data_ptr(),
                                         _stream_ptr()), "hfa_ctc_greedy")
    return out[: int(n.item())]
```

Baseline: 87.19 billion.

## Overlap emission kernel with skew DP via per-row-block ready flags and PDL

Adds an overlap mode in which the emission stream kernel processes row-block runs in a due-time order, computes edges inline, and publishes a release flag per row block. The skew DP kernel is launched as a programmatic dependent and polls these flags with acquire loads before issuing its bulk tile loads, so DP can begin while emission is still running. Backtrace clears the flags for the next call. This removes the serialization between the emission and DP phases but introduces spin-waiting, reduced emission occupancy, and ordering risks that depend on the proxy fence being correct.

```diff
diff --git a/hubertfa_b200/csrc/hfa_api.cu b/hubertfa_b200/csrc/hfa_api.cu
--- a/hubertfa_b200/csrc/hfa_api.cu
+++ b/hubertfa_b200/csrc/hfa_api.cu
@@ -25,9 +25,10 @@
 cudaError_t hfa_launch_dp_band(const HfaLaunchCtx &c, int k, int item_begin, int n_items, int32_t *ticket,
                                bool keep_dp, int64_t fused_row_stride, float *dp_dump);
 cudaError_t hfa_launch_dp_skew(const HfaLaunchCtx &c, int d, int item_begin, int n_items, int32_t *ticket,
-                               bool keep_dp, float *dp_dump);
+                               bool keep_dp, float *dp_dump, const uint32_t *ready);
 cudaError_t hfa_launch_emission(const HfaLaunchCtx &c, int total_row_blocks, int max_sp, int dtype,
-                                int64_t max_row_stride, int *n_launched);
+                                int64_t max_row_stride, int n_runs, int run_len, int ovl_per_sm, int *n_launched);
+bool hfa_emission_streams(int vocab, int dtype, int64_t max_row_stride);
 cudaError_t hfa_launch_edge(const HfaLaunchCtx &c, int total_row_blocks, int dtype);
 cudaError_t hfa_launch_pack(const HfaLaunchCtx &c, int total_row_blocks, const float *prob_log,
                             const float *edge_log, const float *not_edge_log,
@@ -146,6 +147,9 @@
     int32_t band_begin[2] = {0, 0}, band_count[2] = {0, 0}, band_k[2] = {2, 4};
     int32_t band_skew[2] = {0, 0};
     int64_t band_xchg_elems = 0, dp_store_elems = 0;
+    bool overlap = false;
+    int32_t emis_run_len = 2;
+    std::vector<int32_t> emis_runs;
     std::vector<int32_t> jblk_utt, jblk_first;
     int32_t n_valid = 0, n_kept = 0;
     int32_t bt_begin = 0;
@@ -157,6 +161,7 @@
     int64_t o_utt = 0, o_ids = 0, o_order = 0, o_rowblk = 0, o_blkutt = 0, o_inputs = 0, head_bytes = 0;
     int64_t o_emis = 0, o_edge2 = 0, o_edgep = 0, o_bp = 0, o_path = 0, o_revi = 0, o_revt = 0,
             o_last = 0, o_dpst = 0, o_jump = 0, o_moves = 0, o_rowent = 0, o_band_items = 0, o_jblk_utt = 0, o_jblk_first = 0, o_band_ticket = 0, o_band_xchg = 0, band_bytes = 0, o_tmaps = 0, ws_bytes = 0;
+    int64_t o_eruns = 0, o_ready = 0;
     int32_t n_tmaps = 0;
     std::vector<unsigned char> head;
     HfaResultLayout res{};
@@ -208,6 +213,8 @@
     w.band_items = reinterpret_cast<const HfaBandItem *>(b + p->o_band_items);
     w.band_ticket = reinterpret_cast<int32_t *>(b + p->o_band_ticket);
     w.band_xchg = reinterpret_cast<uint4 *>(b + p->o_band_xchg);
+    w.row_ready = p->overlap ? reinterpret_cast<uint32_t *>(b + p->o_ready) : nullptr;
+    w.emis_runs = reinterpret_cast<const int32_t *>(b + p->o_eruns);
     return w;
 }
 
@@ -452,6 +459,25 @@
         };
         add_bands(lat_band, 0);
         add_bands(big_band, 1);
+        p->overlap = p->warp_all_count == 0 && p->class_count[HFA_NUM_CLASSES] == 0 &&
+                     (p->band_count[0] > 0) != (p->band_count[1] > 0) &&
+                     p->band_skew[p->band_count[0] > 0 ? 0 : 1] > 0;
+        if (const char *e = std::getenv("HFA_EMIS_RUN")) p->emis_run_len = std::max(1, std::atoi(e));
+        if (p->overlap) {
+            int32_t t_max = 0;
+            for (const HfaUtt &m : p->utt) t_max = std::max(t_max, m.T);
+            struct Run { int64_t due; int32_t T, first; };
+            std::vector<Run> runs;
+            for (int32_t b = 0; b < n_utt; ++b)
+                for (int32_t j = 0; p->row_blocks[b] + j < p->row_blocks[b + 1]; j += p->emis_run_len)
+                    runs.push_back({(int64_t)(t_max - p->utt[b].T) + (int64_t)HFA_EMIS_ROWS * j, p->utt[b].T,
+                                    p->row_blocks[b] + j});
+            std::sort(runs.begin(), runs.end(), [](const Run &x, const Run &y) {
+                if (x.due != y.due) return x.due < y.due;
+                return x.T != y.T ? x.T > y.T : x.first < y.first;
+            });
+            for (const Run &r : runs) p->emis_runs.push_back(r.first);
+        }
         p->n_valid = (int32_t)all.size();
         for (const HfaUtt &m : p->utt) p->n_kept += (m.status == 0 && m.dp_off >= 0);
         p->jblk_first.assign((size_t)n_utt + 1, 0);
@@ -547,6 +573,7 @@
         p->o_jblk_first = region((int64_t)p->jblk_first.size() * 4);
         p->o_colids = region(p->n_compact > 0 ? (int64_t)p->col_ids.size() * 4 : 0);
         p->o_colmap = region(p->n_compact > 0 ? (int64_t)p->colmap.size() : 0);
+        p->o_eruns = region((int64_t)p->emis_runs.size() * 4);
         p->head_bytes = o;
         p->o_inputs = region((int64_t)n_utt * sizeof(HfaInput));
         p->o_emis = region(emis * 4);
@@ -567,6 +594,7 @@
         p->o_tmaps = region((int64_t)p->n_tmaps * 128);
         p->o_band_ticket = region(p->band_items.empty() ? 0 : 8);
         p->o_band_xchg = region(p->band_xchg_elems * 16);
+        p->o_ready = region(p->overlap ? (int64_t)p->row_blocks[n_utt] * 4 : 0);
         p->band_bytes = o - p->o_band_ticket;
         p->ws_bytes = std::max<int64_t>(o, 256);
 
@@ -590,6 +618,8 @@
         std::memcpy(p->head.data() + p->o_rowblk, p->row_blocks.data(), (size_t)(n_utt + 1) * 4);
         if (!p->block_utt.empty())
             std::memcpy(p->head.data() + p->o_blkutt, p->block_utt.data(), p->block_utt.size() * 4);
+        if (!p->emis_runs.empty())
+            std::memcpy(p->head.data() + p->o_eruns, p->emis_runs.data(), p->emis_runs.size() * 4);
 
         int64_t r = 0;
         auto rreg = [&](int64_t bytes) { const int64_t at = r; r = align_up(r + bytes, 16); return at; };
@@ -672,6 +702,7 @@
         case 1: off = p->o_edge2; n = p->total_edge * 8; break;
         case 2: off = p->o_edgep; n = p->total_edge * 4; break;
         case 3: off = p->o_bp; n = p->total_words * 4; break;
+        case 4: off = p->o_ready; n = p->overlap ? (int64_t)p->row_blocks[p->n_utt] * 4 : 0; break;
         default: break;
     }
     if (n_bytes) *n_bytes = n;
@@ -792,24 +823,38 @@
     side_pool().clear();
 }
 
-int hfa_emission(const hfa_plan *p, void *workspace, int32_t dtype, void *stream)
+static int64_t emission_row_stride(const hfa_plan *p, const void *workspace)
+{
+    static const bool no_tma = [] { const char *v = std::getenv("HFA_EMISSION_NO_TMA"); return v && v[0] == '1'; }();
+    return no_tma ? 0 : p->row_stride_of(workspace);
+}
+
+static int overlap_emission_ctas()
+{
+    int k = 1;
+    if (const char *e = std::getenv("HFA_OVERLAP_CTAS")) k = std::max(1, std::atoi(e));
+    return k;
+}
+
+static int emission_impl(const hfa_plan *p, void *workspace, int32_t dtype, void *stream, bool overlap)
 {
     if (!p || !workspace) return fail(HFA_ERR_ARG, "hfa_emission: NULL plan/workspace");
     if (p->n_utt == 0 || p->total_frames == 0) return HFA_OK;
     if (dtype < 0 || dtype > 2) return fail(HFA_ERR_ARG, "hfa_emission: bad dtype %d", dtype);
     HfaLaunchCtx c = make_ctx(p, workspace, stream);
-    static const bool no_tma = [] { const char *v = std::getenv("HFA_EMISSION_NO_TMA"); return v && v[0] == '1'; }();
-    const int64_t row_stride = no_tma ? 0 : p->row_stride_of(workspace);
+    const int64_t row_stride = emission_row_stride(p, workspace);
     HfaSideStreams *ss = nullptr;
     cudaError_t e = cudaSuccess;
-    if (row_stride > 0) {
+    if (row_stride > 0 && !overlap) {
         ss = side_streams();
         if (!ss) return fail(HFA_ERR_CUDA, "hfa_emission: cannot create side streams");
         e = cudaEventRecord(ss->fork, c.stream);
         if (e != cudaSuccess) return cuda_fail(e, "hfa_emission: fork");
     }
     int n_launched = 0;
-    e = hfa_launch_emission(c, p->row_blocks[p->n_utt], p->max_sp, dtype, row_stride, &n_launched);
+    e = hfa_launch_emission(c, p->row_blocks[p->n_utt], p->max_sp, dtype, row_stride,
+                            overlap ? (int)p->emis_runs.size() : 0, p->emis_run_len, overlap_emission_ctas(),
+                            &n_launched);
     if (e != cudaSuccess) return cuda_fail(e, "hfa_emission: launch");
     if (n_launched == 2) {
         HfaLaunchCtx cs = c;
@@ -824,6 +869,11 @@
     return HFA_OK;
 }
 
+int hfa_emission(const hfa_plan *p, void *workspace, int32_t dtype, void *stream)
+{
+    return emission_impl(p, workspace, dtype, stream, false);
+}
+
 int hfa_pack_emissions(const hfa_plan *p, void *workspace, const float *prob_log,
                        const float *edge_log, const float *not_edge_log, const float *edge_pred,
                        void *stream)
@@ -841,7 +891,7 @@
 }
 
 static int viterbi_forward_impl(const hfa_plan *p, void *workspace, float *dp_dump, void *stream,
-                                int64_t fused_row_stride)
+                                int64_t fused_row_stride, bool overlap = false)
 {
     if (!p || !workspace) return fail(HFA_ERR_ARG, "hfa_viterbi_forward: NULL plan/workspace");
     HfaLaunchCtx c = make_ctx(p, workspace, stream);
@@ -878,7 +928,8 @@
             const int wh = items[it].k == -3 ? 0 : 1;
             if (p->band_skew[wh] > 0)
                 e = hfa_launch_dp_skew(c, p->band_skew[wh], p->band_begin[wh], p->band_count[wh],
-                                       c.ws.band_ticket + wh, p->dp_store_elems > 0, dp_dump);
+                                       c.ws.band_ticket + wh, p->dp_store_elems > 0, dp_dump,
+                                       overlap ? c.ws.row_ready : nullptr);
             else
                 e = hfa_launch_dp_band(c, p->band_k[wh], p->band_begin[wh], p->band_count[wh],
                                        c.ws.band_ticket + wh, p->dp_store_elems > 0, fused_row_stride, dp_dump);
@@ -958,6 +1009,13 @@
            p->total_cells * 4;
 }
 
+static bool overlap_ok(const hfa_plan *p, void *workspace, int32_t dtype)
+{
+    static const bool off = [] { const char *v = std::getenv("HFA_OVERLAP"); return v && v[0] == '0'; }();
+    return !off && p->overlap && make_ws(p, workspace).tmaps != nullptr &&
+           hfa_emission_streams(p->vocab, dtype, emission_row_stride(p, workspace));
+}
+
 int hfa_align_batch(const hfa_plan *p, void *workspace, int32_t dtype, void *result,
                     float *frame_conf, void *stream)
 {
@@ -969,6 +1027,10 @@
     int rc;
     if ((fused_mode == 1 || (fused_mode == -1 && unsplit)) && fused_ok(p, workspace, dtype)) {
         rc = hfa_forward_fused(p, workspace, dtype, stream);
+    } else if (overlap_ok(p, workspace, dtype)) {
+        rc = emission_impl(p, workspace, dtype, stream, true);
+        if (rc != HFA_OK) return rc;
+        rc = viterbi_forward_impl(p, workspace, nullptr, stream, 0, true);
     } else {
         rc = hfa_emission(p, workspace, dtype, stream);
         if (rc != HFA_OK) return rc;
diff --git a/hubertfa_b200/csrc/hfa_backtrace.cu b/hubertfa_b200/csrc/hfa_backtrace.cu
--- a/hubertfa_b200/csrc/hfa_backtrace.cu
+++ b/hubertfa_b200/csrc/hfa_backtrace.cu
@@ -40,6 +40,8 @@
     const HfaUtt m = ws.utt[u];
     const int n_rows = (m.T + 15) >> 4;
     const int64_t idx = (int64_t)(blockIdx.x - ws.jblk_first[u]) * blockDim.x + threadIdx.x;
+    if (ws.row_ready != nullptr && idx < ws.row_blocks[u + 1] - ws.row_blocks[u])
+        ws.row_ready[ws.row_blocks[u] + idx] = 0u;
     if (idx >= (int64_t)n_rows * m.Sp) return;
     const int w = (int)(idx / m.Sp), s = (int)(idx - (int64_t)w * m.Sp);
     const int tt = (w == n_rows - 1) ? ((m.T - 1) & 15) : 15;
@@ -73,6 +75,8 @@
         return;
     }
     if (m.dp_off >= 0) return;
+    if (ws.row_ready != nullptr)
+        for (int j = ws.row_blocks[u] + lane; j < ws.row_blocks[u + 1]; j += 32) ws.row_ready[j] = 0u;
     const int T = m.T, S = m.S, Sp = m.Sp;
     const int32_t *ids = ws.ids + m.seg_off;
     const uint32_t *bp = ws.bp + m.bp_off;
diff --git a/hubertfa_b200/csrc/hfa_common.cuh b/hubertfa_b200/csrc/hfa_common.cuh
--- a/hubertfa_b200/csrc/hfa_common.cuh
+++ b/hubertfa_b200/csrc/hfa_common.cuh
@@ -68,6 +68,8 @@
     const HfaBandItem *band_items;
     int32_t *band_ticket;
     uint4 *band_xchg;
+    uint32_t *row_ready;
+    const int32_t *emis_runs;
 };
 
 #define HFA_NEG_INF __uint_as_float(0xff800000u)
diff --git a/hubertfa_b200/csrc/hfa_dp_skew.cu b/hubertfa_b200/csrc/hfa_dp_skew.cu
--- a/hubertfa_b200/csrc/hfa_dp_skew.cu
+++ b/hubertfa_b200/csrc/hfa_dp_skew.cu
@@ -120,6 +120,13 @@
 {
     asm volatile("st.relaxed.gpu.global.u64 [%0], %1;" ::"l"(p), "l"(a) : "memory");
 }
+__device__ __forceinline__ uint32_t sk_ld_ready(const uint32_t *p)
+{
+    uint32_t v;
+    asm volatile("ld.acquire.gpu.global.u32 %0, [%1];" : "=r"(v) : "l"(p) : "memory");
+    return v;
+}
+__device__ __forceinline__ void sk_fence_proxy_async_global() { asm volatile("fence.proxy.async.global;" ::: "memory"); }
 __device__ __forceinline__ unsigned long long sk_pack(float v, uint32_t tag)
 {
     return (unsigned long long)__float_as_uint(v) | ((unsigned long long)tag << 32);
@@ -203,7 +210,8 @@
 
 template <int D, int NSTG, bool KEEP, bool DUMP>
 __global__ void __launch_bounds__(64)
-hfa_dp_skew_kernel(HfaWs ws, int item_begin, int32_t *ticket, float *__restrict__ dp_dump, int force_slow)
+hfa_dp_skew_kernel(HfaWs ws, int item_begin, int32_t *ticket, float *__restrict__ dp_dump, int force_slow,
+                   const uint32_t *__restrict__ ready, int idle_ns)
 {
     using SM = SkSmem<NSTG>;
     constexpr int R = NSTG * BLK;
@@ -266,9 +274,8 @@
                 sk_bulk_load(sm0 + SM::EDGE + (uint32_t)NSTG * SK_EDGE_B, g_edge + t0, ebytes, bar);
             }
         };
-        static_assert(PF + 1 <= NSTG, "prologue fills distinct stages");
-        if (sk_elect_one())
-            for (int i = 0; i <= PF && i < NB; ++i) issue(i, i);
+        static_assert(PF + 1 <= NSTG, "tiles 0 .. PF fill distinct stages");
+        const uint32_t *my_ready = ready != nullptr ? ready + ws.row_blocks[u] : nullptr;
 
         const ulonglong2 *left_x = reinterpret_cast<const ulonglong2 *>(ws.band_xchg) +
                                    (has_left ? ws.band_items[item - 1].xoff : 0);
@@ -281,7 +288,7 @@
         uint32_t par_a = 0;
         int b = 0, st_b = 0;
         uint32_t par_b = 0;
-        int st_issue = (PF + 1) % NSTG;
+        int f = 0, st_issue = 0;
         uint32_t spins = 0;
         while (b < NB) {
             if (b < a && __all_sync(0xffffffffu, sk_mbar_test(sm0 + SM::DONE + 8u * (uint32_t)st_b, par_b))) {
@@ -296,15 +303,11 @@
                                                (uint32_t)t + 1u));
                     }
                 }
-                if (sk_elect_one()) {
-                    if (KEEP && g_dp != nullptr) {
-                        sk_bulk_store(g_dp + (int64_t)b * (BLK * 32), sm0 + SM::DPST + (uint32_t)buf_b * SK_DPST_B,
-                                      SK_DPST_B);
-                        hfa_bulk_commit();
-                    }
-                    if (b + PF + 1 < NB) issue(b + PF + 1, st_issue);
-                }
-                if (++st_issue == NSTG) st_issue = 0;
+                if (KEEP && g_dp != nullptr && sk_elect_one()) {
+                    sk_bulk_store(g_dp + (int64_t)b * (BLK * 32), sm0 + SM::DPST + (uint32_t)buf_b * SK_DPST_B,
+                                  SK_DPST_B);
+                    hfa_bulk_commit();
+                }
                 if (++st_b == NSTG) {
                     st_b = 0;
                     par_b ^= 1u;
@@ -313,6 +316,22 @@
                 ++b;
                 spins = 0;
                 continue;
+            }
+            if (f < NB && f <= b + PF) {
+                uint32_t go = 0;
+                if (sk_elect_one()) {
+                    go = (my_ready == nullptr || BLK * f >= T) ? 1u : sk_ld_ready(my_ready + (BLK * f) / 64);
+                    if (go) {
+                        if (my_ready != nullptr) sk_fence_proxy_async_global();
+                        issue(f, st_issue);
+                    }
+                }
+                if (__any_sync(0xffffffffu, go != 0)) {
+                    ++f;
+                    if (++st_issue == NSTG) st_issue = 0;
+                    spins = 0;
+                    continue;
+                }
             }
             if (a < NB && a <= b + SK_NBUF - 1 &&
                 __all_sync(0xffffffffu, sk_mbar_test(sm0 + SM::FULL + 8u * (uint32_t)st_a, par_a))) {
@@ -361,8 +380,10 @@
                 }
             }
             if (++spins > (1u << 26)) __trap();
+            if (idle_ns > 0) __nanosleep((unsigned)idle_ns);
         }
         if (KEEP && sk_elect_one()) hfa_bulk_wait_all();
+        asm volatile("griddepcontrol.wait;" ::: "memory");
         return;
     }
 
@@ -564,43 +585,66 @@
         if (s == S - 1) ws.dp_last[2 * u] = dp;
         if (s == S - 2) ws.dp_last[2 * u + 1] = dp;
     }
-}
+    asm volatile("griddepcontrol.wait;" ::: "memory");
+}
+
+struct SkLaunch {
+    int item_begin, n_items;
+    int32_t *ticket;
+    float *dp_dump;
+    int force_slow;
+    const uint32_t *ready;
+    int idle_ns;
+};
 
 template <int D, int NSTG, bool KEEP, bool DUMP>
-cudaError_t launch_skew(const HfaLaunchCtx &c, int item_begin, int n_items, int32_t *ticket, float *dp_dump,
-                        int force_slow)
+cudaError_t launch_skew(const HfaLaunchCtx &c, const SkLaunch &l)
 {
     const size_t smem = SkSmem<NSTG>::BYTES;
     cudaError_t e = cudaFuncSetAttribute(hfa_dp_skew_kernel<D, NSTG, KEEP, DUMP>,
                                          cudaFuncAttributeMaxDynamicSharedMemorySize, (int)smem);
     if (e != cudaSuccess) return e;
-    hfa_dp_skew_kernel<D, NSTG, KEEP, DUMP><<<n_items, 64, smem, c.stream>>>(c.ws, item_begin, ticket, dp_dump,
-                                                                            force_slow);
-    return cudaGetLastError();
+    if (l.ready != nullptr) {
+        e = cudaFuncSetAttribute(hfa_dp_skew_kernel<D, NSTG, KEEP, DUMP>, cudaFuncAttributePreferredSharedMemoryCarveout,
+                                 cudaSharedmemCarveoutMaxShared);
+        if (e != cudaSuccess) return e;
+    }
+    cudaLaunchConfig_t cfg = {};
+    cfg.gridDim = dim3((unsigned)l.n_items);
+    cfg.blockDim = dim3(64);
+    cfg.dynamicSmemBytes = smem;
+    cfg.stream = c.stream;
+    cudaLaunchAttribute attr[1];
+    attr[0].id = cudaLaunchAttributeProgrammaticStreamSerialization;
+    attr[0].val.programmaticStreamSerializationAllowed = 1;
+    cfg.attrs = attr;
+    cfg.numAttrs = l.ready != nullptr ? 1 : 0;
+    return cudaLaunchKernelEx(&cfg, hfa_dp_skew_kernel<D, NSTG, KEEP, DUMP>, c.ws, l.item_begin, l.ticket, l.dp_dump,
+                              l.force_slow, l.ready, l.idle_ns);
 }
 
 template <int D, int NSTG>
-cudaError_t launch_skew_d(const HfaLaunchCtx &c, int item_begin, int n_items, int32_t *ticket, bool keep_dp,
-                          float *dp_dump, int force_slow)
-{
-    if (dp_dump != nullptr)
-        return keep_dp ? launch_skew<D, NSTG, true, true>(c, item_begin, n_items, ticket, dp_dump, force_slow)
-                       : launch_skew<D, NSTG, false, true>(c, item_begin, n_items, ticket, dp_dump, force_slow);
-    return keep_dp ? launch_skew<D, NSTG, true, false>(c, item_begin, n_items, ticket, dp_dump, force_slow)
-                   : launch_skew<D, NSTG, false, false>(c, item_begin, n_items, ticket, dp_dump, force_slow);
+cudaError_t launch_skew_d(const HfaLaunchCtx &c, bool keep_dp, const SkLaunch &l)
+{
+    if (l.dp_dump != nullptr)
+        return keep_dp ? launch_skew<D, NSTG, true, true>(c, l) : launch_skew<D, NSTG, false, true>(c, l);
+    return keep_dp ? launch_skew<D, NSTG, true, false>(c, l) : launch_skew<D, NSTG, false, false>(c, l);
 }
 
 }
 
 cudaError_t hfa_launch_dp_skew(const HfaLaunchCtx &c, int d, int item_begin, int n_items, int32_t *ticket,
-                               bool keep_dp, float *dp_dump)
+                               bool keep_dp, float *dp_dump, const uint32_t *ready)
 {
     if (n_items <= 0) return cudaSuccess;
     if (c.ws.tmaps == nullptr) return cudaErrorNotSupported;
     const char *sl = getenv("HFA_SKEW_SLOW");
     const int force_slow = (sl && sl[0] == '1') ? 1 : 0;
+    int idle_ns = 0;
+    if (const char *e = getenv("HFA_SKEW_IDLE_NS")) idle_ns = atoi(e);
+    const SkLaunch l{item_begin, n_items, ticket, dp_dump, force_slow, ready, idle_ns};
     constexpr int NS = HFA_SKEW_BLK == 32 ? 5 : 12;
-    if (d == 2) return launch_skew_d<2, NS>(c, item_begin, n_items, ticket, keep_dp, dp_dump, force_slow);
-    if (d == 3) return launch_skew_d<3, NS>(c, item_begin, n_items, ticket, keep_dp, dp_dump, force_slow);
+    if (d == 2) return launch_skew_d<2, NS>(c, keep_dp, l);
+    if (d == 3) return launch_skew_d<3, NS>(c, keep_dp, l);
     return cudaErrorInvalidValue;
 }
diff --git a/hubertfa_b200/csrc/hfa_emission.cu b/hubertfa_b200/csrc/hfa_emission.cu
--- a/hubertfa_b200/csrc/hfa_emission.cu
+++ b/hubertfa_b200/csrc/hfa_emission.cu
@@ -260,9 +260,14 @@
         sum = __fadd_rn(sum, hfa_exp_neg(__fsub_rn(xv[j], mx)));
 }
 
-template <typename TIn>
+__device__ __forceinline__ void hfa_st_release_u32(uint32_t *p, uint32_t v)
+{
+    asm volatile("st.release.gpu.global.u32 [%0], %1;" ::"l"(p), "r"(v) : "memory");
+}
+
+template <typename TIn, bool OVL>
 __global__ void __launch_bounds__(HFA_EMIS_WARPS * 32)
-hfa_emission_stream_kernel(HfaWs ws, int n_blocks, int V, int sp_cap, int stage_bytes)
+hfa_emission_stream_kernel(HfaWs ws, int n_blocks, int V, int sp_cap, int stage_bytes, int n_runs, int run_len)
 {
     constexpr int RPW = HFA_EMIS_ROWS / HFA_EMIS_WARPS;
     extern __shared__ __align__(128) unsigned char smem_raw[];
@@ -275,9 +280,27 @@
     int32_t *shift_sm = reinterpret_cast<int32_t *>(bar + 2);
 
     const int tid = threadIdx.x, lane = tid & 31, warp = tid >> 5;
-    const int blk0 = (int)(((int64_t)blockIdx.x * n_blocks) / gridDim.x);
-    const int blk1 = (int)(((int64_t)(blockIdx.x + 1) * n_blocks) / gridDim.x);
-    if (blk0 >= blk1) return;
+    if (OVL) asm volatile("griddepcontrol.launch_dependents;" ::: "memory");
+    int r = blockIdx.x, blk, end;
+    auto run_end = [&](int first) { return min(first + run_len, ws.row_blocks[ws.block_utt[first] + 1]); };
+    if (OVL) {
+        if (r >= n_runs) return;
+        blk = ws.emis_runs[r];
+        end = run_end(blk);
+    } else {
+        blk = (int)(((int64_t)blockIdx.x * n_blocks) / gridDim.x);
+        end = (int)(((int64_t)(blockIdx.x + 1) * n_blocks) / gridDim.x);
+        if (blk >= end) return;
+    }
+    auto advance = [&](int &b, int &rr, int &e) {
+        if (++b < e) return;
+        if (OVL && (rr += gridDim.x) < n_runs) {
+            b = ws.emis_runs[rr];
+            e = run_end(b);
+            return;
+        }
+        b = -1;
+    };
 
     auto issue = [&](int blk, int s) {
         const int u = ws.block_utt[blk];
@@ -298,7 +321,7 @@
         hfa_mbar_init(&bar[0], 1);
         hfa_mbar_init(&bar[1], 1);
         hfa_fence_mbar_init();
-        issue(blk0, 0);
+        issue(blk, 0);
     }
     __syncthreads();
 
@@ -311,9 +334,11 @@
     for (int j = 0; j < 16; ++j) kreg[j] = 0;
     HfaUtt m;
     HfaInput in;
-    for (int blk = blk0; blk < blk1; ++blk) {
-        const int s = (blk - blk0) & 1;
-        if (tid == 0 && blk + 1 < blk1) issue(blk + 1, s ^ 1);
+    for (int it = 0; blk >= 0; ++it) {
+        const int s = it & 1;
+        int nxt = blk, r_nxt = r, end_nxt = end;
+        advance(nxt, r_nxt, end_nxt);
+        if (tid == 0 && nxt >= 0) issue(nxt, s ^ 1);
         const int u = ws.block_utt[blk];
         if (u != cur_u) {
             cur_u = u;
@@ -358,7 +383,7 @@
         const int t_base = (blk - ws.row_blocks[u]) * HFA_EMIS_ROWS;
         const int row_st = (int)in.frame_st;
 
-        hfa_mbar_wait(&bar[s], (uint32_t)(((blk - blk0) >> 1) & 1));
+        hfa_mbar_wait(&bar[s], (uint32_t)((it >> 1) & 1));
         const TIn *xs = reinterpret_cast<const TIn *>(stage0 + (size_t)s * stage_bytes + shift_sm[s]);
 
         {
@@ -459,7 +484,12 @@
                 }
             }
         }
+        if (OVL) edge_block<TIn>(ws, m, in, t_base, tid);
         __syncthreads();
+        if (OVL && tid == 0) hfa_st_release_u32(ws.row_ready + blk, 1u);
+        blk = nxt;
+        r = r_nxt;
+        end = end_nxt;
     }
 }
 
@@ -582,35 +612,47 @@
     return cudaGetLastError();
 }
 
+template <typename TIn> static int64_t stream_stage_bytes(int V, int64_t max_row_stride)
+{
+    const int64_t stage = max_row_stride > 0
+        ? ((HFA_EMIS_ROWS * max_row_stride * (int64_t)sizeof(TIn) + 32 + 127) & ~(int64_t)127) : 0;
+    return (V <= HFA_EMIS_BLOCK_MAX_V && stage <= 48 * 1024) ? stage : 0;
+}
+
 template <typename TIn>
 static cudaError_t launch_emission_t(const HfaLaunchCtx &c, int blocks, int max_sp, int64_t max_row_stride,
-                                     int *n_launched)
+                                     int n_runs, int run_len, int ovl_per_sm, int *n_launched)
 {
     *n_launched = 1;
     const int V = c.vocab;
     max_sp = max_sp < HFA_EMIS_ID_CAP ? max_sp : HFA_EMIS_ID_CAP;
     cudaError_t e;
-    const int64_t stage = max_row_stride > 0
-        ? ((HFA_EMIS_ROWS * max_row_stride * (int64_t)sizeof(TIn) + 32 + 127) & ~(int64_t)127) : 0;
-    if (V <= HFA_EMIS_BLOCK_MAX_V && stage > 0 && stage <= 48 * 1024) {
+    const int64_t stage = stream_stage_bytes<TIn>(V, max_row_stride);
+    if (stage > 0) {
         const size_t smem = 2 * (size_t)stage + (size_t)max_sp * 4 + 8 * 4 + 256 * 4 + HFA_EMIS_ROWS * 8 +
                             2 * 8 + 2 * 4 + 16;
-        e = cudaFuncSetAttribute(hfa_emission_stream_kernel<TIn>,
-                                 cudaFuncAttributeMaxDynamicSharedMemorySize, (int)smem);
+        const bool ovl = n_runs > 0;
+        const auto kern = ovl ? hfa_emission_stream_kernel<TIn, true> : hfa_emission_stream_kernel<TIn, false>;
+        e = cudaFuncSetAttribute(kern, cudaFuncAttributeMaxDynamicSharedMemorySize, (int)smem);
         if (e != cudaSuccess) return e;
+        if (ovl) {
+            e = cudaFuncSetAttribute(kern, cudaFuncAttributePreferredSharedMemoryCarveout, cudaSharedmemCarveoutMaxShared);
+            if (e != cudaSuccess) return e;
+        }
         int per_sm = 0;
-        e = cudaOccupancyMaxActiveBlocksPerMultiprocessor(&per_sm, hfa_emission_stream_kernel<TIn>,
-                                                          HFA_EMIS_WARPS * 32, smem);
+        e = cudaOccupancyMaxActiveBlocksPerMultiprocessor(&per_sm, kern, HFA_EMIS_WARPS * 32, smem);
         if (e != cudaSuccess) return e;
         per_sm = per_sm < 1 ? 1 : (per_sm > 4 ? 4 : per_sm);
+        if (ovl && per_sm > ovl_per_sm) per_sm = ovl_per_sm;
         int dev = 0, n_sm = 148;
         if (cudaGetDevice(&dev) == cudaSuccess) cudaDeviceGetAttribute(&n_sm, cudaDevAttrMultiProcessorCount, dev);
-        const int grid = blocks < n_sm * per_sm ? blocks : n_sm * per_sm;
-        *n_launched = 2;
-        hfa_emission_stream_kernel<TIn><<<grid, HFA_EMIS_WARPS * 32, smem, c.stream>>>(
-            c.ws, blocks, V, max_sp, (int)stage);
+        const int work = ovl ? n_runs : blocks;
+        const int grid = work < n_sm * per_sm ? work : n_sm * per_sm;
+        *n_launched = ovl ? 1 : 2;
+        kern<<<grid, HFA_EMIS_WARPS * 32, smem, c.stream>>>(c.ws, blocks, V, max_sp, (int)stage, n_runs, run_len);
         return cudaGetLastError();
     }
+    if (n_runs > 0) return cudaErrorNotSupported;
     if (V <= HFA_EMIS_BLOCK_MAX_V) {
         const int VP = (V + 1) | 1;
         const size_t smem = (size_t)max_sp * 4 + 8 * 4 + 256 * 4 + HFA_EMIS_ROWS * 8 +
@@ -633,15 +675,28 @@
     return cudaGetLastError();
 }
 
+bool hfa_emission_streams(int vocab, int dtype, int64_t max_row_stride)
+{
+    if (dtype == 0) return stream_stage_bytes<float>(vocab, max_row_stride) > 0;
+    if (dtype == 1) return stream_stage_bytes<__half>(vocab, max_row_stride) > 0;
+    if (dtype == 2) return stream_stage_bytes<__nv_bfloat16>(vocab, max_row_stride) > 0;
+    return false;
+}
+
 cudaError_t hfa_launch_emission(const HfaLaunchCtx &c, int total_row_blocks, int max_sp, int dtype,
-                                int64_t max_row_stride, int *n_launched)
+                                int64_t max_row_stride, int n_runs, int run_len, int ovl_per_sm, int *n_launched)
 {
     *n_launched = 0;
     if (total_row_blocks <= 0) return cudaSuccess;
-    if (dtype == 0) return launch_emission_t<float>(c, total_row_blocks, max_sp, max_row_stride, n_launched);
-    if (dtype == 1) return launch_emission_t<__half>(c, total_row_blocks, max_sp, max_row_stride, n_launched);
+    if (dtype == 0)
+        return launch_emission_t<float>(c, total_row_blocks, max_sp, max_row_stride, n_runs, run_len, ovl_per_sm,
+                                        n_launched);
+    if (dtype == 1)
+        return launch_emission_t<__half>(c, total_row_blocks, max_sp, max_row_stride, n_runs, run_len, ovl_per_sm,
+                                         n_launched);
     if (dtype == 2)
-        return launch_emission_t<__nv_bfloat16>(c, total_row_blocks, max_sp, max_row_stride, n_launched);
+        return launch_emission_t<__nv_bfloat16>(c, total_row_blocks, max_sp, max_row_stride, n_runs, run_len,
+                                                ovl_per_sm, n_launched);
     return cudaErrorInvalidValue;
 }
 
diff --git a/hubertfa_b200/ops.py b/hubertfa_b200/ops.py
--- a/hubertfa_b200/ops.py
+++ b/hubertfa_b200/ops.py
@@ -129,11 +129,11 @@
                     intervals=v(L.intervals, np.float64, 2 * ns).reshape(ns, 2))
 
     def debug_region(self, workspace: torch.Tensor, which: str) -> torch.Tensor:
-        code = {"emis": 0, "edge2": 1, "edge_p": 2, "bp": 3}[which]
+        code = {"emis": 0, "edge2": 1, "edge_p": 2, "bp": 3, "ready": 4}[which]
         nb = C.c_int64()
         off = int(self._lib.hfa_plan_debug_region(self._h, code, C.byref(nb)))
         raw = workspace[off:off + int(nb.value)]
-        if which == "bp":
+        if which in ("bp", "ready"):
             return raw.view(torch.int32)
         v = raw.view(torch.float32)
         return v.view(-1, 2) if which == "edge2" else v
```

Result: slower. 68.21 billion (median of 6 runs) (-21.8%).
